# leighghunt/kart

Measured on AMD Instinct MI355X. Metric: feature deltas classified+field-diffed/sec (M/s) at 1/2/4/8 GPUs; % HBM peak, higher is better.
Workload: dtype u8/u64 (integer + fp64 compare); 1 GPU; C3: ONE 100000000-polygon int-PK layer, 10% edits (4% geometry + 4% attribute updates, 1% del, 1% ins), two-commit diff + field diff; features=100000000, delta_order=walk (= key) order, then pk order (kd_delta_pk_order), side_order=git tree (walk) order as listed, no side sort, parallelism=bucket-range shards x1

## Files before the change

include/kartdiff.h:

```cpp
#ifndef KARTDIFF_H
#define KARTDIFF_H

#include <stddef.h>
#include <stdint.h>

#ifdef __cplusplus
extern "C" {
#endif

#define KD_ABI_VERSION 1

#define KD_OK 0
#define KD_EINVAL (-1)
#define KD_EHIP (-2)
#define KD_EUNSUPPORTED (-3)

#define KD_NONE 0xFFFFFFFFu

#define KD_MEM_HOST 0u
#define KD_MEM_DEVICE 1u

#define KD_KEY_INT 0u
#define KD_KEY_HASH 1u

// ... 3 lines not shown
    uint64_t n;
    const uint64_t* key;
    const uint8_t* oid;
    const uint8_t* name;
    const uint64_t* name_off;
    uint32_t mem;
    uint32_t key_mode;
} kd_side;

typedef struct kd_blobs {
    uint64_t n;
    const uint8_t* data;
    const uint64_t* off;
    uint32_t mem;
    uint32_t size_hint;
} kd_blobs;

typedef struct kd_legend_maps {
    int32_t n_keys;
    int32_t words;
    int32_t n_leg_old;
    int32_t n_leg_new;
    const uint8_t* leg_old_hex;
    const int16_t* map_old;
    const uint8_t* leg_new_hex;
    const int16_t* map_new;
    const uint64_t* cmp_mask;
} kd_legend_maps;

typedef struct kd_diff_result {
    uint64_t n_insert, n_update, n_delete, n_delta;
    uint32_t* delta;
    uint32_t* upd;
} kd_diff_result;

typedef struct kd_merge_result {
    uint64_t n_clean;
    uint64_t n_conflict;
    uint64_t n_mdelta;
    uint32_t* conflict;
    uint32_t* mdelta;
} kd_merge_result;

int kd_abi_version(void);
const char* kd_last_error(void);
int kd_init(int device_ordinal, kd_ctx** out);
int kd_fini(kd_ctx* ctx);
int kd_set_stream(kd_ctx* ctx, void* hip_stream);
int kd_set_option(kd_ctx* ctx, const char* name, int64_t value);
int kd_get_option(kd_ctx* ctx, const char* name, int64_t* value);
int kd_sync(kd_ctx* ctx);
int kd_reserve(kd_ctx* ctx, uint64_t max_entries_per_side, uint64_t max_updates);
void kd_free(void* p);

int kd_diff2(kd_ctx* ctx, const kd_side* base, const kd_side* target, uint32_t flags,
             kd_diff_result** out);
#define KD_DIFF_UNORDERED 0x1u

int kd_diff2_device(kd_ctx* ctx, const kd_side* base, const kd_side* target, uint32_t flags,
                    uint32_t* d_delta, uint32_t* d_upd, uint64_t* d_counts, uint32_t* d_err);

int kd_diff2_device_perm(kd_ctx* ctx, const kd_side* base, const kd_side* target, const uint32_t* base_order,
                         const uint32_t* target_order, uint32_t flags, uint32_t* d_delta, uint32_t* d_upd,
                         uint64_t* d_counts, uint32_t* d_err);

int kd_diff2_device_ex(kd_ctx* ctx, const kd_side* base, const kd_side* target, const uint32_t* base_order,
                       const uint32_t* target_order, uint32_t flags, uint32_t* d_delta, uint32_t* d_upd,
                       uint64_t* d_delta_key, uint64_t* d_upd_key, uint64_t* d_counts, uint32_t* d_err);

int kd_fielddiff(kd_ctx* ctx, const kd_blobs* old_blobs, const kd_blobs* new_blobs,
                 const uint32_t* pu, uint64_t n_upd, const uint64_t* d_n_upd, uint32_t pairs_mem,
                 const kd_legend_maps* maps, uint64_t* masks, uint8_t* status, uint32_t out_mem);

int kd_merge3(kd_ctx* ctx, const kd_side* ancestor, const kd_side* ours, const kd_side* theirs,
              uint32_t flags, kd_merge_result** out);
int kd_merge3_device(kd_ctx* ctx, const kd_side* ancestor, const kd_side* ours, const kd_side* theirs,
                     uint32_t flags, uint32_t* d_conflict, uint32_t* d_mdelta, uint64_t* d_counts,
                     uint32_t* d_err);

int kd_merge3_device_perm(kd_ctx* ctx, const kd_side* ancestor, const kd_side* ours, const kd_side* theirs,
                          const uint32_t* ancestor_order, const uint32_t* ours_order, const uint32_t* theirs_order,
                          uint32_t flags, uint32_t* d_conflict, uint32_t* d_mdelta, uint64_t* d_counts,
                          uint32_t* d_err);

int kd_envelopes(kd_ctx* ctx, const kd_blobs* geoms, const double filt_env[4], int bits,
                 uint8_t* match, uint8_t* enc, uint8_t* enc_ok, uint32_t out_mem,
                 uint64_t* n_candidates);
int kd_env_overlap(kd_ctx* ctx, const uint8_t* enc, uint64_t n, int bits, const double q[4],
                   uint8_t* out, uint32_t mem);

typedef struct kd_sf_index kd_sf_index;
int kd_sf_index_build(kd_ctx* ctx, const uint8_t* oid, const uint8_t* env, uint64_t n, int bits, uint32_t mem,
                      kd_sf_index** out);
int kd_sf_filter(kd_ctx* ctx, const kd_sf_index* index, const uint8_t* oid, const uint8_t* is_feature, uint64_t m,
                 const double q[4], uint8_t* result, uint32_t mem);
int kd_sf_index_free(kd_sf_index* index);

#define KD_GF_RECT 0x1u
#define KD_GF_DELTA_HEADS 0x2u
typedef struct kd_geom_cols {
    int32_t n_leg_old, n_leg_new;
    const uint8_t* leg_old_hex;
    const int16_t* gidx_old;
    const uint8_t* leg_new_hex;
    const int16_t* gidx_new;
} kd_geom_cols;
int kd_geom_filter(kd_ctx* ctx, const kd_blobs* old_blobs, const kd_blobs* new_blobs, const uint32_t* pairs,
                   uint64_t n, const uint64_t* d_n, uint32_t pairs_mem, const kd_geom_cols* cols,
                   const double filt_env[4], uint32_t flags, int bits, uint8_t* match, uint32_t* keep,
                   uint64_t* n_keep, uint8_t* enc, uint8_t* enc_ok, uint32_t out_mem);

#define KD_GH_GEOM 0u
#define KD_GH_NULL 2u
#define KD_GH_FALLBACK 3u
typedef struct kd_geom_head {
    uint8_t gpkg[40];
    uint32_t glen;
    uint32_t goff_status;
} kd_geom_head;
int kd_geom_heads(const uint8_t* data, const uint64_t* off, uint64_t n, int n_leg, const uint8_t* leg_hex,
                  const int16_t* gidx, int threads, kd_geom_head* out);
int kd_geom_filter_heads(kd_ctx* ctx, const kd_geom_head* heads_old, uint64_t n_old, const kd_geom_head* heads_new,
                         uint64_t n_new, uint32_t heads_mem, const kd_blobs* old_blobs, const kd_blobs* new_blobs,
                         const uint32_t* pairs, uint64_t n, const uint64_t* d_n, uint32_t pairs_mem,
                         const double filt_env[4], uint32_t flags, int bits, uint8_t* match, uint32_t* keep,
                         uint64_t* n_keep, uint8_t* enc, uint8_t* enc_ok, uint32_t out_mem);

int kd_geom_filter_deltas(kd_ctx* ctx, const kd_geom_head* heads_old, uint64_t n_old, const kd_geom_head* heads_new,
                          uint64_t n_new, const kd_blobs* old_blobs, const kd_blobs* new_blobs, const uint32_t* pairs,
                          uint64_t cap, const uint64_t* d_n, const double filt_env[4], uint32_t flags, int bits,
                          uint8_t* match, uint32_t* keep, uint64_t* n_keep, uint8_t* enc, uint8_t* enc_ok);

#define KD_HEX_BYTES 0u
#define KD_HEX_GPKG_WKB 1u
int kd_hex_encode(kd_ctx* ctx, const kd_blobs* blobs, uint32_t mode, uint8_t* hex, uint32_t* start,
                  uint8_t* status, uint32_t out_mem);

int kd_sort_side(kd_ctx* ctx, uint64_t* d_key, uint8_t* d_oid, uint32_t* d_order, uint64_t n, uint32_t* h_dup);
typedef struct kd_keys_info {
    uint64_t vary;
    uint64_t key0;
    int64_t pk_min, pk_max;
    int32_t ascending;
    int32_t seg_max;
} kd_keys_info;
int kd_keys_scan(const uint64_t* keys, uint64_t n, uint32_t key_mode, kd_keys_info* out);
int kd_sort_side_into(kd_ctx* ctx, const uint64_t* d_key_in, const uint8_t* d_oid_in, uint64_t* d_key_out,
                      uint8_t* d_oid_out, uint32_t* d_order, uint64_t n, uint32_t* d_dup, const kd_keys_info* info);
int kd_sort_segmented_into(kd_ctx* ctx, const uint64_t* d_key_in, uint64_t* d_key_out, uint32_t* d_order,
                           uint64_t n, int seg_bits, int max_seg, uint32_t* d_err);
int kd_delta_pk_order(kd_ctx* ctx, const kd_side* base, const kd_side* target, const uint32_t* d_delta,
                      const uint64_t* d_keys, uint64_t cap, const uint64_t* d_n, int64_t pk_lo, int64_t pk_hi,
                      int64_t* d_pk, uint32_t* d_perm);

#define KD_COPY_H2D 1u
#define KD_COPY_D2H 2u
#define KD_COPY_D2D 3u
int kd_malloc(kd_ctx* ctx, uint64_t bytes, void** dptr);
int kd_mfree(kd_ctx* ctx, void* dptr);
int kd_host_alloc(uint64_t bytes, void** hptr);
int kd_host_free(void* hptr);
int kd_memcpy(kd_ctx* ctx, void* dst, const void* src, uint64_t bytes, uint32_t kind);
int kd_memset(kd_ctx* ctx, void* dst, int value, uint64_t bytes);
int kd_device_sync(kd_ctx* ctx);

#define KD_COMM_ID_BYTES 128
int kd_comm_unique_id(uint8_t id[KD_COMM_ID_BYTES]);
int kd_comm_init(kd_ctx* ctx, int nranks, int rank, const uint8_t id[KD_COMM_ID_BYTES]);
int kd_comm_fini(kd_ctx* ctx);
int kd_comm_info(kd_ctx* ctx, int32_t out[3]);
int kd_allgather_u64(kd_ctx* ctx, const uint64_t* d_send, uint64_t* d_recv, uint64_t n);
int kd_diff2_gather(kd_ctx* ctx, const kd_side* base, const kd_side* target, uint64_t base_off,
                    uint64_t target_off, uint32_t flags, uint32_t* d_delta, uint32_t* d_upd,
                    uint64_t* d_counts, uint32_t* d_err, uint32_t* d_all_delta, uint64_t all_cap,
                    uint64_t* d_all_counts, uint64_t* h_all_counts);
int kd_diff2_gather_begin(kd_ctx* ctx, const kd_side* base, const kd_side* target, uint64_t base_off,
                          uint64_t target_off, uint32_t flags, uint32_t* d_delta, uint32_t* d_upd,
                          uint64_t* d_counts, uint32_t* d_err, uint64_t* d_all_counts);
int kd_diff2_gather_end(kd_ctx* ctx, const uint32_t* d_delta, uint32_t* d_all_delta, uint64_t all_cap,
                        uint64_t* h_all_counts);
int kd_diff2_sharded(kd_ctx** ctxs, int g, const kd_side* base, const kd_side* target, int bucket_bits,
                     uint32_t flags, kd_diff_result** out);
int kd_shard_cuts(const uint64_t* key_a, uint64_t n_a, const uint64_t* key_b, uint64_t n_b, int g, int bucket_bits,
                  uint64_t* cut, uint64_t* a_lo, uint64_t* b_lo);

int64_t kd_pack_int_keys(const uint8_t* names, const uint64_t* name_off, uint64_t n,
                         uint64_t* keys, uint8_t* status);
int64_t kd_pack_hash_keys(const uint8_t* paths, const uint64_t* path_off, uint64_t n, int levels,
                          int hex, uint64_t* keys, uint8_t* status);
int kd_int_keys_to_pks(const uint64_t* keys, uint64_t n, int64_t* pks);

#define KD_ENOTFOUND (-4)
typedef struct kd_odb kd_odb;
int kd_odb_open(const char* gitdir, kd_odb** out);
int kd_odb_set_option(kd_odb* odb, const char* name, int64_t value);
int kd_odb_get_option(kd_odb* odb, const char* name, int64_t* value);
int kd_odb_close(kd_odb* odb);
int kd_odb_read(kd_odb* odb, const uint8_t oid[20], int* type, uint8_t** data, uint64_t* len);
int kd_odb_read_batch(kd_odb* odb, const uint8_t* oids, uint64_t n, int threads, uint8_t** data,
                      uint64_t* off, uint8_t* status);
typedef struct kd_leaves {
    uint64_t n;
    uint64_t* path_off;
    uint32_t* mode;
    uint8_t* oid;
    uint8_t* path;
    int32_t present;
} kd_leaves;
#define KD_WALK_ALL (-1)
int kd_walk(kd_odb* odb, const uint8_t* roots, int k, const char* subpath, int cmp0, int cmp1,
            int threads, kd_leaves** out);

int kd_prof_enable(kd_ctx* ctx, int on);
int kd_prof_select(kd_ctx* ctx, const char* names);
int kd_prof_get(kd_ctx* ctx, const char* name, uint64_t* launches, double* total_ms);
int kd_prof_reset(kd_ctx* ctx);

#ifdef __cplusplus
}
#endif
#endif
```

kart_amd/_native.py:

```python
import ctypes
import os

HERE = os.path.dirname(os.path.abspath(__file__))
LIB_PATH = os.environ.get("KART_AMD_LIB", os.path.join(HERE, "libkartdiff.so"))

KD_OK = 0
KD_EINVAL = -1
KD_EHIP = -2
KD_EUNSUPPORTED = -3
KD_ENOTFOUND = -4
KD_WALK_ALL = -1
KD_NONE = 0xFFFFFFFF
KD_MEM_HOST = 0
KD_MEM_DEVICE = 1
KD_KEY_INT = 0
KD_KEY_HASH = 1
KD_DIFF_UNORDERED = 0x1
KD_HEX_BYTES = 0
KD_HEX_GPKG_WKB = 1
KD_COPY_H2D = 1
KD_COPY_D2H = 2
KD_COPY_D2D = 3
KD_COMM_ID_BYTES = 128
KD_GH_GEOM, KD_GH_NULL, KD_GH_FALLBACK = 0, 2, 3
KD_GF_RECT = 0x1
KD_GF_DELTA_HEADS = 0x2

c_u8p = ctypes.POINTER(ctypes.c_uint8)
c_u32p = ctypes.POINTER(ctypes.c_uint32)
c_u64p = ctypes.POINTER(ctypes.c_uint64)
c_i16p = ctypes.POINTER(ctypes.c_int16)
c_i64p = ctypes.POINTER(ctypes.c_int64)
c_dblp = ctypes.POINTER(ctypes.c_double)


class NativeUnavailable(RuntimeError):
    pass


class KdError(RuntimeError):
    def __init__(self, code, msg):
        super().__init__(f"libkartdiff error {code}: {msg}")
        self.code = code


class Unsupported(KdError):
    """KD_EUNSUPPORTED: this input needs the reference CPU path."""


class NotFound(KdError):
    """KD_ENOTFOUND: a git object is not in the object database."""


class KdLeaves(ctypes.Structure):
    _fields_ = [
        ("n", ctypes.c_uint64),
        ("path_off", c_u64p),
        ("mode", c_u32p),
        ("oid", c_u8p),
        ("path", c_u8p),
        ("present", ctypes.c_int32),
    ]


class KdSide(ctypes.Structure):
    _fields_ = [
        ("n", ctypes.c_uint64),
        ("key", ctypes.c_void_p),
        ("oid", ctypes.c_void_p),
        ("name", ctypes.c_void_p),
        ("name_off", ctypes.c_void_p),
        ("mem", ctypes.c_uint32),
        ("key_mode", ctypes.c_uint32),
    ]


class KdBlobs(ctypes.Structure):
    _fields_ = [
        ("n", ctypes.c_uint64),
        ("data", ctypes.c_void_p),
        ("off", ctypes.c_void_p),
        ("mem", ctypes.c_uint32),
        ("size_hint", ctypes.c_uint32),
    ]


class KdLegendMaps(ctypes.Structure):
    _fields_ = [
        ("n_keys", ctypes.c_int32),
        ("words", ctypes.c_int32),
        ("n_leg_old", ctypes.c_int32),
        ("n_leg_new", ctypes.c_int32),
        ("leg_old_hex", ctypes.c_void_p),
        ("map_old", ctypes.c_void_p),
        ("leg_new_hex", ctypes.c_void_p),
        ("map_new", ctypes.c_void_p),
        ("cmp_mask", ctypes.c_void_p),
    ]


class KdGeomCols(ctypes.Structure):
    _fields_ = [
        ("n_leg_old", ctypes.c_int32),
        ("n_leg_new", ctypes.c_int32),
        ("leg_old_hex", ctypes.c_void_p),
        ("gidx_old", ctypes.c_void_p),
        ("leg_new_hex", ctypes.c_void_p),
        ("gidx_new", ctypes.c_void_p),
    ]


class KdKeysInfo(ctypes.Structure):
    _fields_ = [
        ("vary", ctypes.c_uint64),
        ("key0", ctypes.c_uint64),
        ("pk_min", ctypes.c_int64),
        ("pk_max", ctypes.c_int64),
        ("ascending", ctypes.c_int32),
        ("seg_max", ctypes.c_int32),
    ]


class KdDiffResult(ctypes.Structure):
    _fields_ = [
        ("n_insert", ctypes.c_uint64),
        ("n_update", ctypes.c_uint64),
        ("n_delete", ctypes.c_uint64),
        ("n_delta", ctypes.c_uint64),
        ("delta", c_u32p),
        ("upd", c_u32p),
    ]


class KdMergeResult(ctypes.Structure):
    _fields_ = [
        ("n_clean", ctypes.c_uint64),
        ("n_conflict", ctypes.c_uint64),
        ("n_mdelta", ctypes.c_uint64),
        ("conflict", c_u32p),
        ("mdelta", c_u32p),
    ]


SIGNATURES = {
    "kd_abi_version": (ctypes.c_int, []),
    "kd_last_error": (ctypes.c_char_p, []),
    "kd_init": (ctypes.c_int, [ctypes.c_int, ctypes.POINTER(ctypes.c_void_p)]),
    "kd_fini": (ctypes.c_int, [ctypes.c_void_p]),
    "kd_set_stream": (ctypes.c_int, [ctypes.c_void_p, ctypes.c_void_p]),
    "kd_set_option": (ctypes.c_int, [ctypes.c_void_p, ctypes.c_char_p, ctypes.c_int64]),
    "kd_get_option": (ctypes.c_int, [ctypes.c_void_p, ctypes.c_char_p, ctypes.POINTER(ctypes.c_int64)]),
    "kd_sync": (ctypes.c_int, [ctypes.c_void_p]),
    "kd_reserve": (ctypes.c_int, [ctypes.c_void_p, ctypes.c_uint64, ctypes.c_uint64]),
    "kd_free": (None, [ctypes.c_void_p]),
    "kd_diff2": (
        ctypes.c_int,
        [ctypes.c_void_p, ctypes.POINTER(KdSide), ctypes.POINTER(KdSide), ctypes.c_uint32,
         ctypes.POINTER(ctypes.POINTER(KdDiffResult))],
    ),
    "kd_diff2_device": (
        ctypes.c_int,
        [ctypes.c_void_p, ctypes.POINTER(KdSide), ctypes.POINTER(KdSide), ctypes.c_uint32,
         ctypes.c_void_p, ctypes.c_void_p, ctypes.c_void_p, ctypes.c_void_p],
    ),
    "kd_fielddiff": (
        ctypes.c_int,
        [ctypes.c_void_p, ctypes.POINTER(KdBlobs), ctypes.POINTER(KdBlobs), ctypes.c_void_p,
         ctypes.c_uint64, ctypes.c_void_p, ctypes.c_uint32, ctypes.POINTER(KdLegendMaps),
         ctypes.c_void_p, ctypes.c_void_p, ctypes.c_uint32],
    ),
    "kd_merge3": (
        ctypes.c_int,
        [ctypes.c_void_p, ctypes.POINTER(KdSide), ctypes.POINTER(KdSide), ctypes.POINTER(KdSide),
         ctypes.c_uint32, ctypes.POINTER(ctypes.POINTER(KdMergeResult))],
    ),
    "kd_merge3_device": (
        ctypes.c_int,
        [ctypes.c_void_p, ctypes.POINTER(KdSide), ctypes.POINTER(KdSide), ctypes.POINTER(KdSide),
         ctypes.c_uint32, ctypes.c_void_p, ctypes.c_void_p, ctypes.c_void_p, ctypes.c_void_p],
    ),
    "kd_merge3_device_perm": (
        ctypes.c_int,
        [ctypes.c_void_p, ctypes.POINTER(KdSide), ctypes.POINTER(KdSide), ctypes.POINTER(KdSide), ctypes.c_void_p,
         ctypes.c_void_p, ctypes.c_void_p, ctypes.c_uint32, ctypes.c_void_p, ctypes.c_void_p, ctypes.c_void_p,
         ctypes.c_void_p],
    ),
    "kd_envelopes": (
        ctypes.c_int,
        [ctypes.c_void_p, ctypes.POINTER(KdBlobs), c_dblp, ctypes.c_int, ctypes.c_void_p,
         ctypes.c_void_p, ctypes.c_void_p, ctypes.c_uint32, c_u64p],
    ),
    "kd_env_overlap": (
        ctypes.c_int,
        [ctypes.c_void_p, ctypes.c_void_p, ctypes.c_uint64, ctypes.c_int, c_dblp, ctypes.c_void_p,
         ctypes.c_uint32],
    ),
    "kd_geom_heads": (ctypes.c_int, [ctypes.c_void_p, ctypes.c_void_p, ctypes.c_uint64, ctypes.c_int, ctypes.c_void_p,
                                      ctypes.c_void_p, ctypes.c_int, ctypes.c_void_p]),
    "kd_geom_filter_heads": (
        ctypes.c_int,
        [ctypes.c_void_p, ctypes.c_void_p, ctypes.c_uint64, ctypes.c_void_p, ctypes.c_uint64, ctypes.c_uint32,
         ctypes.c_void_p, ctypes.c_void_p, ctypes.c_void_p, ctypes.c_uint64, ctypes.c_void_p, ctypes.c_uint32, c_dblp,
         ctypes.c_uint32, ctypes.c_int, ctypes.c_void_p, ctypes.c_void_p, c_u64p, ctypes.c_void_p, ctypes.c_void_p,
         ctypes.c_uint32],
    ),
    "kd_geom_filter_deltas": (
        ctypes.c_int,
        [ctypes.c_void_p, ctypes.c_void_p, ctypes.c_uint64, ctypes.c_void_p, ctypes.c_uint64, ctypes.POINTER(KdBlobs),
         ctypes.POINTER(KdBlobs), ctypes.c_void_p, ctypes.c_uint64, ctypes.c_void_p, c_dblp, ctypes.c_uint32, ctypes.c_int,
         ctypes.c_void_p, ctypes.c_void_p, c_u64p, ctypes.c_void_p, ctypes.c_void_p],
    ),
    "kd_shard_cuts": (ctypes.c_int, [ctypes.c_void_p, ctypes.c_uint64, ctypes.c_void_p, ctypes.c_uint64, ctypes.c_int,
                                      ctypes.c_int, ctypes.c_void_p, ctypes.c_void_p, ctypes.c_void_p]),
    "kd_sf_index_build": (ctypes.c_int, [ctypes.c_void_p, ctypes.c_void_p, ctypes.c_void_p, ctypes.c_uint64, ctypes.c_int,
                                          ctypes.c_uint32, ctypes.POINTER(ctypes.c_void_p)]),
    "kd_sf_filter": (ctypes.c_int, [ctypes.c_void_p, ctypes.c_void_p, ctypes.c_void_p, ctypes.c_void_p, ctypes.c_uint64,
                                     c_dblp, ctypes.c_void_p, ctypes.c_uint32]),
    "kd_sf_index_free": (ctypes.c_int, [ctypes.c_void_p]),
    "kd_geom_filter": (
        ctypes.c_int,
        [ctypes.c_void_p, ctypes.POINTER(KdBlobs), ctypes.POINTER(KdBlobs), ctypes.c_void_p, ctypes.c_uint64,
         ctypes.c_void_p, ctypes.c_uint32, ctypes.POINTER(KdGeomCols), c_dblp, ctypes.c_uint32, ctypes.c_int,
         ctypes.c_void_p, ctypes.c_void_p, c_u64p, ctypes.c_void_p, ctypes.c_void_p, ctypes.c_uint32],
    ),
    "kd_hex_encode": (
        ctypes.c_int,
        [ctypes.c_void_p, ctypes.POINTER(KdBlobs), ctypes.c_uint32, ctypes.c_void_p, ctypes.c_void_p,
         ctypes.c_void_p, ctypes.c_uint32],
    ),
    "kd_sort_side": (ctypes.c_int, [ctypes.c_void_p, ctypes.c_void_p, ctypes.c_void_p, ctypes.c_void_p, ctypes.c_uint64,
                                     ctypes.c_void_p]),
    "kd_diff2_device_perm": (ctypes.c_int, [ctypes.c_void_p, ctypes.c_void_p, ctypes.c_void_p, ctypes.c_void_p,
                                             ctypes.c_void_p, ctypes.c_uint32, ctypes.c_void_p, ctypes.c_void_p,
                                             ctypes.c_void_p, ctypes.c_void_p]),
    "kd_sort_side_into": (ctypes.c_int, [ctypes.c_void_p, ctypes.c_void_p, ctypes.c_void_p, ctypes.c_void_p,
                                          ctypes.c_void_p, ctypes.c_void_p, ctypes.c_uint64, ctypes.c_void_p,
                                          ctypes.POINTER(KdKeysInfo)]),
    "kd_keys_scan": (ctypes.c_int, [ctypes.c_void_p, ctypes.c_uint64, ctypes.c_uint32, ctypes.POINTER(KdKeysInfo)]),
    "kd_sort_segmented_into": (ctypes.c_int, [ctypes.c_void_p, ctypes.c_void_p, ctypes.c_void_p, ctypes.c_void_p,
                                               ctypes.c_uint64, ctypes.c_int, ctypes.c_int, ctypes.c_void_p]),
    "kd_delta_pk_order": (ctypes.c_int, [ctypes.c_void_p, ctypes.POINTER(KdSide), ctypes.POINTER(KdSide),
                                          ctypes.c_void_p, ctypes.c_void_p, ctypes.c_uint64, ctypes.c_void_p,
                                          ctypes.c_int64, ctypes.c_int64, ctypes.c_void_p, ctypes.c_void_p]),
    "kd_diff2_device_ex": (ctypes.c_int, [ctypes.c_void_p, ctypes.POINTER(KdSide), ctypes.POINTER(KdSide),
                                           ctypes.c_void_p, ctypes.c_void_p, ctypes.c_uint32, ctypes.c_void_p,
                                           ctypes.c_void_p, ctypes.c_void_p, ctypes.c_void_p, ctypes.c_void_p,
                                           ctypes.c_void_p]),
    "kd_malloc": (ctypes.c_int, [ctypes.c_void_p, ctypes.c_uint64, ctypes.POINTER(ctypes.c_void_p)]),
    "kd_mfree": (ctypes.c_int, [ctypes.c_void_p, ctypes.c_void_p]),
    "kd_host_alloc": (ctypes.c_int, [ctypes.c_uint64, ctypes.POINTER(ctypes.c_void_p)]),
    "kd_host_free": (ctypes.c_int, [ctypes.c_void_p]),
    "kd_memcpy": (ctypes.c_int, [ctypes.c_void_p, ctypes.c_void_p, ctypes.c_void_p, ctypes.c_uint64, ctypes.c_uint32]),
    "kd_memset": (ctypes.c_int, [ctypes.c_void_p, ctypes.c_void_p, ctypes.c_int, ctypes.c_uint64]),
    "kd_device_sync": (ctypes.c_int, [ctypes.c_void_p]),
    "kd_comm_unique_id": (ctypes.c_int, [ctypes.c_void_p]),
    "kd_comm_init": (ctypes.c_int, [ctypes.c_void_p, ctypes.c_int, ctypes.c_int, ctypes.c_void_p]),
    "kd_comm_fini": (ctypes.c_int, [ctypes.c_void_p]),
    "kd_comm_info": (ctypes.c_int, [ctypes.c_void_p, ctypes.c_void_p]),
    "kd_allgather_u64": (ctypes.c_int, [ctypes.c_void_p, ctypes.c_void_p, ctypes.c_void_p, ctypes.c_uint64]),
    "kd_diff2_gather": (
        ctypes.c_int,
        [ctypes.c_void_p, ctypes.POINTER(KdSide), ctypes.POINTER(KdSide), ctypes.c_uint64, ctypes.c_uint64,
         ctypes.c_uint32, ctypes.c_void_p, ctypes.c_void_p, ctypes.c_void_p, ctypes.c_void_p, ctypes.c_void_p,
         ctypes.c_uint64, ctypes.c_void_p, ctypes.c_void_p],
    ),
    "kd_diff2_gather_begin": (
        ctypes.c_int,
        [ctypes.c_void_p, ctypes.POINTER(KdSide), ctypes.POINTER(KdSide), ctypes.c_uint64, ctypes.c_uint64,
         ctypes.c_uint32, ctypes.c_void_p, ctypes.c_void_p, ctypes.c_void_p, ctypes.c_void_p, ctypes.c_void_p],
    ),
    "kd_diff2_gather_end": (
        ctypes.c_int, [ctypes.c_void_p, ctypes.c_void_p, ctypes.c_void_p, ctypes.c_uint64, ctypes.c_void_p],
    ),
    "kd_diff2_sharded": (
        ctypes.c_int,
        [ctypes.POINTER(ctypes.c_void_p), ctypes.c_int, ctypes.POINTER(KdSide), ctypes.POINTER(KdSide), ctypes.c_int,
         ctypes.c_uint32, ctypes.POINTER(ctypes.POINTER(KdDiffResult))],
    ),
    "kd_pack_int_keys": (
        ctypes.c_int64,
        [ctypes.c_void_p, ctypes.c_void_p, ctypes.c_uint64, ctypes.c_void_p, ctypes.c_void_p],
    ),
    "kd_pack_hash_keys": (
        ctypes.c_int64,
        [ctypes.c_void_p, ctypes.c_void_p, ctypes.c_uint64, ctypes.c_int, ctypes.c_int,
         ctypes.c_void_p, ctypes.c_void_p],
    ),
    "kd_int_keys_to_pks": (ctypes.c_int, [ctypes.c_void_p, ctypes.c_uint64, ctypes.c_void_p]),
    "kd_odb_open": (ctypes.c_int, [ctypes.c_char_p, ctypes.POINTER(ctypes.c_void_p)]),
    "kd_odb_close": (ctypes.c_int, [ctypes.c_void_p]),
    "kd_odb_set_option": (ctypes.c_int, [ctypes.c_void_p, ctypes.c_char_p, ctypes.c_int64]),
    "kd_odb_get_option": (ctypes.c_int, [ctypes.c_void_p, ctypes.c_char_p, ctypes.POINTER(ctypes.c_int64)]),
    "kd_odb_read": (
        ctypes.c_int,
        [ctypes.c_void_p, ctypes.c_void_p, ctypes.POINTER(ctypes.c_int), ctypes.POINTER(c_u8p), c_u64p],
    ),
    "kd_odb_read_batch": (
        ctypes.c_int,
        [ctypes.c_void_p, ctypes.c_void_p, ctypes.c_uint64, ctypes.c_int, ctypes.POINTER(c_u8p), ctypes.c_void_p,
         ctypes.c_void_p],
    ),
    "kd_walk": (
        ctypes.c_int,
        [ctypes.c_void_p, ctypes.c_void_p, ctypes.c_int, ctypes.c_char_p, ctypes.c_int, ctypes.c_int, ctypes.c_int,
         ctypes.POINTER(ctypes.POINTER(KdLeaves))],
    ),
    "kd_prof_enable": (ctypes.c_int, [ctypes.c_void_p, ctypes.c_int]),
    "kd_prof_select": (ctypes.c_int, [ctypes.c_void_p, ctypes.c_char_p]),
    "kd_prof_get": (
        ctypes.c_int,
        [ctypes.c_void_p, ctypes.c_char_p, c_u64p, c_dblp],
    ),
    "kd_prof_reset": (ctypes.c_int, [ctypes.c_void_p]),
}

_lib = None


def lib():
    global _lib
    if _lib is None:
        if not os.path.exists(LIB_PATH):
            raise NativeUnavailable(
                f"{LIB_PATH} not built: run `python -c 'import __graft_entry__ as g; g.build()'`"
            )
        try:
            L = ctypes.CDLL(LIB_PATH)
        except OSError as e:
            raise NativeUnavailable(f"cannot load {LIB_PATH}: {e}") from e
        for name, (res, args) in SIGNATURES.items():
            fn = getattr(L, name)
            fn.restype = res
            fn.argtypes = args
        _lib = L
    return _lib


def check(rc, what=""):
    if rc == KD_OK:
        return
    msg = lib().kd_last_error().decode(errors="replace")
    if rc == KD_EUNSUPPORTED:
        raise Unsupported(rc, f"{what}: {msg}")
    if rc == KD_ENOTFOUND:
        raise NotFound(rc, f"{what}: {msg}")
    raise KdError(rc, f"{what}: {msg}")


def ptr(a):
    if a is None:
        return None
    return a.ctypes.data
```

kart_amd/csrc/kd_classify.hip:

```cpp
#include <cstdlib>

#include "kd_join.h"

namespace kd {

#ifndef KD_RS3_PROBE_NOSEARCH
#define KD_RS3_PROBE_NOSEARCH 0
#endif
#ifndef KD_RS3_PROBE_NOOID
#define KD_RS3_PROBE_NOOID 0
#endif
#ifndef KD_RS3_PROBE_NONAMES
#define KD_RS3_PROBE_NONAMES 0
#endif
constexpr int C3_NT = 256;
constexpr int C3_CH = 1024;
#ifndef KD_C3_SAMPLE_BITS
#define KD_C3_SAMPLE_BITS 11
#endif
constexpr int C3_SAMPLE_BITS = KD_C3_SAMPLE_BITS;
constexpr int C3_SAMPLES = 1 << C3_SAMPLE_BITS;

struct Resolve3Args {
    const u64 *A, *O, *T;
// ... 281 lines not shown
    g.A = (const u64*)dz; g.O = (const u64*)ptr(O.key, nO); g.T = (const u64*)ptr(T.key, nT);
    g.oA = (const u32*)ptr(A.oid, nA); g.oO = (const u32*)ptr(O.oid, nO); g.oT = (const u32*)ptr(T.oid, nT);
    g.nA = nA; g.nO = nO;
    g.nmA = (const u8*)ptr(A.name, nA); g.nmO = (const u8*)ptr(O.name, nO); g.nmT = (const u8*)ptr(T.name, nT);
    g.noA = (const u64*)ptr(A.name_off, nA); g.noO = (const u64*)ptr(O.name_off, nO); g.noT = (const u64*)ptr(T.name_off, nT);
    g.hash_mode = A.key_mode == KD_KEY_HASH;
    g.cand = nullptr; g.cand3 = cand3; g.c2 = c2;
    g.pA = (const u32*)ptr(pA, nA); g.pO = (const u32*)ptr(pO, nO); g.pT = (const u32*)ptr(pT, nT);
    g.desc = (u64*)desc; g.nchunk = nchunk; g.aux = (u32*)aux;
    g.out_conf = d_conf; g.out_md = d_md; g.counts = counts; g.err = derr;
    const u64 grid = std::min<u64>((nO + nT) / C3_CH + 1, (u64)ctx->n_cu * (u64)occ_r3a);
    return launch(ctx, "k_resolve3", [&] {
        if (perm) hipLaunchKernelGGL((k_resolve3<C3_NT, true, true>), dim3((unsigned)grid), dim3(C3_NT), 0, ctx->stream, g);
        else hipLaunchKernelGGL((k_resolve3<C3_NT, false, true>), dim3((unsigned)grid), dim3(C3_NT), 0, ctx->stream, g);
    });
}

int kd::stage_side(kd_ctx* ctx, const kd_side* s, const char* tag, kd_side* dev) {
    *dev = *s;
    dev->mem = KD_MEM_DEVICE;
    std::string p(tag);
    int rc;
    if ((rc = stage_in(ctx, (p + ".key").c_str(), s->key, s->n * 8, s->mem, (const void**)&dev->key))) return rc;
    if ((rc = stage_in(ctx, (p + ".oid").c_str(), s->oid, s->n * 20, s->mem, (const void**)&dev->oid))) return rc;
    if (s->key_mode == KD_KEY_HASH && s->n) {
        KD_CHECK(s->name_off && s->name, "KD_KEY_HASH side without filenames");
        u64 nbytes = s->mem == KD_MEM_HOST ? s->name_off[s->n] : 0;
        if (s->mem == KD_MEM_DEVICE) {
            KD_HIP(hipMemcpy(&nbytes, s->name_off + s->n, 8, hipMemcpyDeviceToHost));
        }
        if ((rc = stage_in(ctx, (p + ".noff").c_str(), s->name_off, (s->n + 1) * 8, s->mem, (const void**)&dev->name_off))) return rc;
        if ((rc = stage_in(ctx, (p + ".name").c_str(), s->name, nbytes ? nbytes : 1, s->mem, (const void**)&dev->name))) return rc;
    }
    return KD_OK;
}

int kd::check_side(const kd_side* s, const char* which) {
    KD_CHECK(s, "%s side is NULL", which);
    KD_CHECK(s->n == 0 || (s->key && s->oid), "%s side: key/oid NULL", which);
    KD_CHECK(s->mem == KD_MEM_HOST || s->mem == KD_MEM_DEVICE, "%s side: bad mem", which);
    KD_CHECK(s->key_mode == KD_KEY_INT || s->key_mode == KD_KEY_HASH, "%s side: bad key_mode", which);
    return KD_OK;
}

static int merge3_device(kd_ctx* ctx, const kd_side& A, const kd_side& O, const kd_side& T, u32* d_conf, uint2* d_md,
                         u64* counts, u32* derr, const u32* pA = nullptr, const u32* pO = nullptr,
                         const u32* pT = nullptr) {
    const bool perm = pA || pO || pT;
    int rc;
    const u64 nA = A.n, nO = O.n, nT = T.n;
    if (nO + nT > 0 && ctx->opt.merge3_join)
        return merge3_join_device(ctx, A, O, T, d_conf, d_md, counts, derr, pA, pO, pT);
    const u64 nchunk = (nO + nT) / C3_CH + 2;
    void *cand, *c2, *desc, *aux, *dz;
    if ((rc = ensure(ctx, "c3.cand", (nO + nT + 1) * 8, &cand))) return rc;
    if ((rc = ensure(ctx, "c3.c2", 64, &c2))) return rc;
    if ((rc = ensure(ctx, "c3.desc", 2 * nchunk * 8, &desc))) return rc;
    const bool fresh_aux = ctx->bufs["c3.aux"].p == nullptr;
    if ((rc = ensure(ctx, "c3.aux", 64, &aux))) return rc;
    if (fresh_aux) KD_HIP(hipMemsetAsync(aux, 0, 64, ctx->stream));
    if ((rc = device_zeros(ctx, &dz))) return rc;
    const u64* kA = nA ? A.key : (const u64*)dz;
    rc = launch(ctx, "k_sorted3", [&] {
        const u64 work = std::max<u64>(nA / 2, 2 * nchunk);
        const u64 blocks = std::min<u64>((work + 255) / 256, (u64)ctx->n_cu * 8);
        hipLaunchKernelGGL(k_sorted3, dim3((unsigned)std::max<u64>(blocks, 1)), dim3(256), 0, ctx->stream, kA, nA,
                           (u64*)desc, 2 * nchunk, (u32*)aux, counts);
    });
    if (rc) return rc;
    if ((rc = diff2_device(ctx, &O, &T, 0, (u32*)cand, nullptr, (u64*)c2, derr, perm ? pO : nullptr,
                           perm ? pT : nullptr)))
        return rc;
    ctx->occ_resolve3 = occupancy(ctx, perm ? (const void*)k_resolve3<C3_NT, true, false> : (const void*)k_resolve3<C3_NT, false, false>,
                                  C3_NT, 0);
    auto ptr = [&](const void* p, u64 n) { return n && p ? p : (const void*)dz; };
    Resolve3Args g;
    g.A = kA; g.O = (const u64*)ptr(O.key, nO); g.T = (const u64*)ptr(T.key, nT);
    g.oA = (const u32*)ptr(A.oid, nA); g.oO = (const u32*)ptr(O.oid, nO); g.oT = (const u32*)ptr(T.oid, nT);
    g.nA = nA; g.nO = nO;
    g.nmA = (const u8*)ptr(A.name, nA); g.nmO = (const u8*)ptr(O.name, nO); g.nmT = (const u8*)ptr(T.name, nT);
    g.noA = (const u64*)ptr(A.name_off, nA); g.noO = (const u64*)ptr(O.name_off, nO); g.noT = (const u64*)ptr(T.name_off, nT);
    g.hash_mode = A.key_mode == KD_KEY_HASH;
    g.cand = (const uint2*)cand; g.c2 = (const u64*)c2;
    g.pA = (const u32*)ptr(pA, nA); g.pO = (const u32*)ptr(pO, nO); g.pT = (const u32*)ptr(pT, nT);
    g.desc = (u64*)desc; g.nchunk = nchunk; g.aux = (u32*)aux;
    g.out_conf = d_conf; g.out_md = d_md; g.counts = counts; g.err = derr;
    const u64 grid = std::min<u64>((nO + nT) / C3_CH + 1, (u64)ctx->n_cu * (u64)ctx->occ_resolve3);
    return launch(ctx, "k_resolve3", [&] {
        if (perm) hipLaunchKernelGGL((k_resolve3<C3_NT, true, false>), dim3((unsigned)grid), dim3(C3_NT), 0, ctx->stream, g);
        else hipLaunchKernelGGL((k_resolve3<C3_NT, false, false>), dim3((unsigned)grid), dim3(C3_NT), 0, ctx->stream, g);
    });
}

extern "C" {

int kd_reserve(kd_ctx* ctx, uint64_t max_entries_per_side, uint64_t max_updates) {
    KD_CHECK(ctx, "kd_reserve: ctx NULL");
    KD_HIP(hipSetDevice(ctx->device));
    u64 total = 2 * max_entries_per_side;
    u64 ntiles = (total + C2_TILE - 1) / C2_TILE + 1;
    void* p;
    int rc;
    if ((rc = ensure(ctx, "c2.part", (ntiles + 1) * 8, &p))) return rc;
    if ((rc = ensure(ctx, "c2.tcnt", ntiles * 16, &p))) return rc;
    if ((rc = ensure(ctx, "c2.gsum", 2 * (ntiles / 64 + 1) * 8, &p))) return rc;
    if ((rc = ensure(ctx, "c2.sdel", ntiles * (C2_TILE + 64) * 8, &p))) return rc;
    (void)max_updates;
    return KD_OK;
}

int kd_diff2_device(kd_ctx* ctx, const kd_side* base, const kd_side* target, uint32_t flags, uint32_t* d_delta,
                    uint32_t* d_upd, uint64_t* d_counts, uint32_t* d_err) {
    KD_CHECK(ctx, "kd_diff2_device: ctx NULL");
    int rc;
    if ((rc = check_side(base, "base")) || (rc = check_side(target, "target"))) return rc;
    KD_CHECK(base->mem == KD_MEM_DEVICE && target->mem == KD_MEM_DEVICE, "kd_diff2_device: sides must be device memory");
    KD_CHECK(d_delta && d_counts && d_err, "kd_diff2_device: NULL output");
    KD_HIP(hipSetDevice(ctx->device));
    return diff2_device(ctx, base, target, flags, d_delta, d_upd, d_counts, d_err);
}

int kd_diff2_device_perm(kd_ctx* ctx, const kd_side* base, const kd_side* target, const uint32_t* base_order,
                         const uint32_t* target_order, uint32_t flags, uint32_t* d_delta, uint32_t* d_upd,
                         uint64_t* d_counts, uint32_t* d_err) {
    KD_CHECK(ctx, "kd_diff2_device_perm: ctx NULL");
    int rc;
    if ((rc = check_side(base, "base")) || (rc = check_side(target, "target"))) return rc;
    KD_CHECK(base->mem == KD_MEM_DEVICE && target->mem == KD_MEM_DEVICE, "kd_diff2_device_perm: sides must be device memory");
    KD_CHECK(d_delta && d_counts && d_err, "kd_diff2_device_perm: NULL output");
    KD_CHECK((base->n == 0 || base_order) && (target->n == 0 || target_order), "kd_diff2_device_perm: NULL order");
    KD_HIP(hipSetDevice(ctx->device));
    return diff2_device(ctx, base, target, flags, d_delta, d_upd, d_counts, d_err,
                        base_order ? base_order : (const u32*)nullptr, target_order);
}

int kd_diff2_device_ex(kd_ctx* ctx, const kd_side* base, const kd_side* target, const uint32_t* base_order,
                       const uint32_t* target_order, uint32_t flags, uint32_t* d_delta, uint32_t* d_upd,
                       uint64_t* d_delta_key, uint64_t* d_upd_key, uint64_t* d_counts, uint32_t* d_err) {
    KD_CHECK(ctx, "kd_diff2_device_ex: ctx NULL");
    int rc;
    if ((rc = check_side(base, "base")) || (rc = check_side(target, "target"))) return rc;
    KD_CHECK(base->mem == KD_MEM_DEVICE && target->mem == KD_MEM_DEVICE, "kd_diff2_device_ex: sides must be device memory");
    KD_CHECK(d_delta && d_counts && d_err, "kd_diff2_device_ex: NULL output");
    KD_CHECK(!base_order == !target_order, "kd_diff2_device_ex: both orders or neither");
    KD_CHECK(!d_upd_key || (d_upd && d_delta_key), "kd_diff2_device_ex: update keys need the update list and delta keys");
    KD_HIP(hipSetDevice(ctx->device));
    void* dz = nullptr;
    if (base_order && (rc = device_zeros(ctx, &dz))) return rc;
    const u32* oa = base_order ? (base->n ? base_order : (const u32*)dz) : nullptr;
    const u32* ob = target_order ? (target->n ? target_order : (const u32*)dz) : nullptr;
    return diff2_device(ctx, base, target, flags, d_delta, d_upd, d_counts, d_err, oa, ob, d_delta_key, d_upd_key);
}

int kd_diff2(kd_ctx* ctx, const kd_side* base, const kd_side* target, uint32_t flags, kd_diff_result** out) {
    KD_CHECK(ctx && out, "kd_diff2: NULL");
    int rc;
    if ((rc = check_side(base, "base")) || (rc = check_side(target, "target"))) return rc;
    KD_HIP(hipSetDevice(ctx->device));
    host_mark(ctx, nullptr);
    kd_side A, B;
    if ((rc = stage_side(ctx, base, "in.a", &A)) || (rc = stage_side(ctx, target, "in.b", &B))) return rc;
    host_mark(ctx, "kd_diff2 stage");
    u64 total = base->n + target->n;
    void *dd, *du, *dc;
    if ((rc = ensure(ctx, "out.delta", (total + 1) * 8, &dd))) return rc;
    if ((rc = ensure(ctx, "out.upd", (total + 1) * 8, &du))) return rc;
    if ((rc = ensure(ctx, "out.counts", 64, &dc))) return rc;
    host_mark(ctx, "kd_diff2 ensure");
    u64* counts = (u64*)dc;
    u32* derr = (u32*)(counts + 4);
    if ((rc = diff2_device(ctx, &A, &B, flags, (u32*)dd, (u32*)du, counts, derr))) return rc;
    host_mark(ctx, "kd_diff2 kernels");
    u64 hc[5];
    KD_HIP(hipMemcpyAsync(hc, dc, 40, hipMemcpyDeviceToHost, ctx->stream));
    KD_HIP(hipStreamSynchronize(ctx->stream));
    u32 err = (u32)(hc[4] & 0xFFFFFFFFu);
    if (err) {
        set_error("kd_diff2: %s", (err & 1) ? "side keys not strictly ascending" : "hash key collision between different filenames");
        return KD_EUNSUPPORTED;
    }
    u64 nd = hc[3], nu = hc[1];
    host_mark(ctx, "kd_diff2 counts");
    size_t bytes = sizeof(kd_diff_result) + (nd + nu) * 8 + 16;
    kd_diff_result* r = (kd_diff_result*)std::malloc(bytes);
    KD_CHECK(r, "kd_diff2: out of host memory");
    host_mark(ctx, "kd_diff2 malloc");
    r->n_insert = hc[0]; r->n_update = hc[1]; r->n_delete = hc[2]; r->n_delta = nd;
    r->delta = (u32*)(r + 1);
    r->upd = r->delta + 2 * nd;
    if (nd) {
        if ((rc = stage_d2h(ctx, r->delta, dd, nd * 8)) || (nu && (rc = stage_d2h(ctx, r->upd, du, nu * 8)))) {
            std::free(r);
            return rc;
        }
    }
    host_mark(ctx, "kd_diff2 results");
    prof_flush(ctx);
    *out = r;
    return KD_OK;
}

int kd_merge3(kd_ctx* ctx, const kd_side* anc, const kd_side* ours, const kd_side* theirs, uint32_t flags,
              kd_merge_result** out) {
    (void)flags;
    KD_CHECK(ctx && out, "kd_merge3: NULL");
    int rc;
    if ((rc = check_side(anc, "ancestor")) || (rc = check_side(ours, "ours")) || (rc = check_side(theirs, "theirs"))) return rc;
    KD_CHECK(anc->key_mode == ours->key_mode && ours->key_mode == theirs->key_mode, "kd_merge3: key modes differ");
    KD_CHECK(anc->n < 0xFFFFFFFFull && ours->n < 0xFFFFFFFFull && theirs->n < 0xFFFFFFFFull, "kd_merge3: side too large");
    KD_HIP(hipSetDevice(ctx->device));
    kd_side A, O, T;
    if ((rc = stage_side(ctx, anc, "in.a", &A)) || (rc = stage_side(ctx, ours, "in.b", &O)) ||
        (rc = stage_side(ctx, theirs, "in.c", &T)))
        return rc;
    const u64 nA = A.n, nO = O.n, nT = T.n;
    void *oc, *om, *dc;
    if ((rc = ensure(ctx, "c3.oc", (nA + nO + nT + 1) * 12, &oc))) return rc;
    if ((rc = ensure(ctx, "c3.om", (nO + nT + 1) * 8, &om))) return rc;
    if ((rc = ensure(ctx, "c3.counts", 64, &dc))) return rc;
    u64* counts = (u64*)dc;
    u32* derr = (u32*)(counts + 4);
    if ((rc = merge3_device(ctx, A, O, T, (u32*)oc, (uint2*)om, counts, derr))) return rc;
    u64 hc[5];
    KD_HIP(hipMemcpyAsync(hc, dc, 40, hipMemcpyDeviceToHost, ctx->stream));
    KD_HIP(hipStreamSynchronize(ctx->stream));
    u32 err = (u32)(hc[4] & 0xFFFFFFFFu);
    if (err) {
        set_error("kd_merge3: err=0x%x (%s)", err,
                  (err & 1) ? "keys not strictly ascending" : (err & 2) ? "hash key collision" : "tile overflow");
        return KD_EUNSUPPORTED;
    }
    u64 nc = hc[1], nm = hc[2];
    kd_merge_result* r = (kd_merge_result*)std::malloc(sizeof(kd_merge_result) + nc * 12 + nm * 8 + 16);
    KD_CHECK(r, "kd_merge3: out of host memory");
    r->n_clean = hc[0]; r->n_conflict = nc; r->n_mdelta = nm;
    r->conflict = (u32*)(r + 1);
    r->mdelta = r->conflict + 3 * nc;
    if ((nc && (rc = stage_d2h(ctx, r->conflict, oc, nc * 12))) || (nm && (rc = stage_d2h(ctx, r->mdelta, om, nm * 8)))) {
        std::free(r);
        return rc;
    }
    prof_flush(ctx);
    *out = r;
    return KD_OK;
}

int kd_merge3_device(kd_ctx* ctx, const kd_side* anc, const kd_side* ours, const kd_side* theirs, uint32_t flags,
                     uint32_t* d_conflict, uint32_t* d_mdelta, uint64_t* d_counts, uint32_t* d_err) {
    (void)flags;
    KD_CHECK(ctx && d_conflict && d_mdelta && d_counts && d_err, "kd_merge3_device: NULL");
    int rc;
    if ((rc = check_side(anc, "ancestor")) || (rc = check_side(ours, "ours")) || (rc = check_side(theirs, "theirs"))) return rc;
    KD_CHECK(anc->mem == KD_MEM_DEVICE && ours->mem == KD_MEM_DEVICE && theirs->mem == KD_MEM_DEVICE,
             "kd_merge3_device: sides must be device memory");
    KD_CHECK(anc->key_mode == ours->key_mode && ours->key_mode == theirs->key_mode, "kd_merge3_device: key modes differ");
    KD_CHECK(anc->n < 0xFFFFFFFFull && ours->n < 0xFFFFFFFFull && theirs->n < 0xFFFFFFFFull,
             "kd_merge3_device: side too large");
    KD_HIP(hipSetDevice(ctx->device));
    return merge3_device(ctx, *anc, *ours, *theirs, d_conflict, (uint2*)d_mdelta, d_counts, d_err);
}

int kd_merge3_device_perm(kd_ctx* ctx, const kd_side* anc, const kd_side* ours, const kd_side* theirs,
                          const uint32_t* anc_order, const uint32_t* ours_order, const uint32_t* theirs_order,
                          uint32_t flags, uint32_t* d_conflict, uint32_t* d_mdelta, uint64_t* d_counts, uint32_t* d_err) {
    (void)flags;
    KD_CHECK(ctx && d_conflict && d_mdelta && d_counts && d_err, "kd_merge3_device_perm: NULL");
    int rc;
    if ((rc = check_side(anc, "ancestor")) || (rc = check_side(ours, "ours")) || (rc = check_side(theirs, "theirs"))) return rc;
    KD_CHECK(anc->mem == KD_MEM_DEVICE && ours->mem == KD_MEM_DEVICE && theirs->mem == KD_MEM_DEVICE,
             "kd_merge3_device_perm: sides must be device memory");
    KD_CHECK(anc->key_mode == ours->key_mode && ours->key_mode == theirs->key_mode, "kd_merge3_device_perm: key modes differ");
    KD_CHECK(anc->n < 0xFFFFFFFFull && ours->n < 0xFFFFFFFFull && theirs->n < 0xFFFFFFFFull,
             "kd_merge3_device_perm: side too large");
    KD_CHECK((anc->n == 0 || anc_order) && (ours->n == 0 || ours_order) && (theirs->n == 0 || theirs_order),
             "kd_merge3_device_perm: NULL order");
    KD_HIP(hipSetDevice(ctx->device));
    void* dz;
    if ((rc = device_zeros(ctx, &dz))) return rc;
    auto ord = [&](const uint32_t* p) { return p ? p : (const u32*)dz; };
    return merge3_device(ctx, *anc, *ours, *theirs, d_conflict, (uint2*)d_mdelta, d_counts, d_err, ord(anc_order),
                         ord(ours_order), ord(theirs_order));
}

}
```

kart_amd/csrc/kd_classify2.hip:

```cpp
#include <cstdlib>

#include "kd_join.h"

namespace kd {

constexpr u64 C2_GROUP = 64;
#ifndef KD_C2_STAGE_PAD
#define KD_C2_STAGE_PAD 32
#endif
constexpr u64 C2_STAGE = C2_TILE + KD_C2_STAGE_PAD;
#ifndef KD_J2_NAME_HALO
#define KD_J2_NAME_HALO 64
#endif
constexpr u64 J2_NAME_HALO = KD_J2_NAME_HALO;
#ifndef KD_PLACE_NT
#define KD_PLACE_NT 64
#endif


template <int PW>
__device__ __forceinline__ u64 mp_search(const u64* __restrict__ A, const u64* __restrict__ B, u64 d, u64 lo, u64 hi) {
    const int lane = threadIdx.x & 63, sub = lane % PW, grp = lane / PW;
    while (hi > lo) {
        const u64 step = (hi - lo + PW - 1) / PW;
// ... 1492 lines not shown
        }
        __syncthreads();
        if (cf) {
            u32* o = sc + 3 * (tc + pc + __builtin_amdgcn_mbcnt_hi((u32)(bc >> 32), __builtin_amdgcn_mbcnt_lo((u32)bc, 0)));
            o[0] = ik; o[1] = io; o[2] = itt;
        }
        if (md) sm[tm + pm + __builtin_amdgcn_mbcnt_hi((u32)(bm >> 32), __builtin_amdgcn_mbcnt_lo((u32)bm, 0))] = make_uint2(io, itt);
        tc += nc;
        tm += nm;
    }
    if (ne) err |= 2u;
    static_assert(2 * IPT < 16, "k_join3b: the clean count's ballot slices");
    {
        const u32 wcl = (u32)__popcll(__ballot(clean & 1)) + 2u * (u32)__popcll(__ballot((clean >> 1) & 1)) +
                        4u * (u32)__popcll(__ballot((clean >> 2) & 1)) + 8u * (u32)__popcll(__ballot((clean >> 3) & 1));
        if (lane == 0) s_wave[2 * (NT / 64) + wid] = wcl;
    }
    __syncthreads();
    u32 tcl = 0;
#pragma unroll
    for (int w = 0; w < NT / 64; w++) tcl += s_wave[2 * (NT / 64) + w];
    if (tid == 0) {
        u32* cc = g.tile_cnt + 4 * tile;
        cc[0] = tcl; cc[1] = tm; cc[2] = 0; cc[3] = tc;
        u64* gs = g.gsum + 2 * (tile / C2_GROUP);
        atomicAdd((unsigned long long*)gs, (unsigned long long)(tc | (u64)tm << 32));
        atomicAdd((unsigned long long*)gs + 1, (unsigned long long)tcl);
    }
    if (!more) break;
    tile = tnext;
    nmA0 = xA0; nmA1 = xA1; nmB0 = xB0; nmB1 = xB1;
    }
    if (err) atomicOr(g.err, err);
}

int merge3_join_device(kd_ctx* ctx, const kd_side& K, const kd_side& O, const kd_side& T, u32* d_conf, uint2* d_md,
                       u64* d_counts, u32* d_err, const u32* ordK, const u32* ordO, const u32* ordT) {
    const u64 nK = K.n, nO = O.n, nT = T.n, total = nO + nT;
    const bool hash = K.key_mode == KD_KEY_HASH;
    const bool perm = ordK || ordO || ordT;
    const bool split = ctx->opt.merge3_split == 1;
    const bool j3_ol = ctx->opt.j3_ol == 1;
    const bool v2 = ctx->opt.j3_v != 0 && !(j3_ol && !perm);
    const int TILE = v2 ? J3B_TILE : J3_TILE;
    if (hash) KD_CHECK((nK == 0 || (K.name && K.name_off)) && (nO == 0 || (O.name && O.name_off)) &&
                       (nT == 0 || (T.name && T.name_off)), "merge3: KD_KEY_HASH needs filenames");
    const u64 ntiles = (total + TILE - 1) / TILE;
    const u64 n_zero = 2 * ((ntiles + C2_GROUP - 1) / C2_GROUP);
    void *part, *apart, *tcnt, *gsum, *gpre, *sconf, *smd, *dz;
    int rc;
    if ((rc = ensure(ctx, "c2.part", (ntiles + 1) * sizeof(u64), &part))) return rc;
    if ((rc = ensure(ctx, "c3.apart", (ntiles + 1) * sizeof(u64), &apart))) return rc;
    if ((rc = ensure(ctx, "c2.tcnt", ntiles * 4 * sizeof(u32), &tcnt))) return rc;
    if ((rc = ensure(ctx, "c2.gsum", n_zero * sizeof(u64), &gsum))) return rc;
    if ((rc = ensure(ctx, "c2.gpre", n_zero * sizeof(u64), &gpre))) return rc;
    if ((rc = ensure(ctx, "c3.sconf", ntiles * C2_STAGE * 12, &sconf))) return rc;
    if ((rc = ensure(ctx, "c3.smd", ntiles * C2_STAGE * sizeof(uint2), &smd))) return rc;
    if ((rc = device_zeros(ctx, &dz))) return rc;
    auto P = [&](const void* p, u64 n) { return n && p ? p : (const void*)dz; };
    const u64* kO = (const u64*)P(O.key, nO);
    const u64* kT = (const u64*)P(T.key, nT);
    const u64* kK = (const u64*)P(K.key, nK);
    rc = launch(ctx, "k_partition2", [&] {
        unsigned nb = (unsigned)((ntiles + C2_PG - 1) / C2_PG);
        if (v2) hipLaunchKernelGGL(k_partition2<J3B_TILE>, dim3(nb), dim3(C2_PNT), 0, ctx->stream, kO, nO, kT, nT, ntiles,
                                   (u64*)part, d_counts, d_err, (u64*)gsum, n_zero);
        else hipLaunchKernelGGL(k_partition2<J3_TILE>, dim3(nb), dim3(C2_PNT), 0, ctx->stream, kO, nO, kT, nT, ntiles,
                                (u64*)part, d_counts, d_err, (u64*)gsum, n_zero);
    });
    if (rc) return rc;
    void* nsplit = nullptr;
    if (v2 && hash && (rc = ensure(ctx, "c3.nsplit", 4 * (ntiles + 1) * sizeof(u64), &nsplit))) return rc;
    rc = launch(ctx, "k_apart3", [&] {
        const u64 lanes = 8 * (ntiles + 1);
        if (v2)
            hipLaunchKernelGGL(k_apart3b, dim3((unsigned)((lanes + 255) / 256)), dim3(256), 0, ctx->stream, kO, nO, kT, nT,
                               (const u64*)part, ntiles, TILE, kK, nK, (u64*)apart, (const u64*)P(O.name_off, nO),
                               (const u64*)P(T.name_off, nT), perm ? J3B_HALO : (u64)0, (u64*)nsplit);
        else
            hipLaunchKernelGGL(k_apart3, dim3((unsigned)((lanes + 255) / 256)), dim3(256), 0, ctx->stream, kO, nO, kT, nT,
                               (const u64*)part, ntiles, TILE, kK, nK, (u64*)apart);
    });
    if (rc) return rc;
    Join3Args a;
    Join2Args& g = a.j;
    g.A = kO; g.oidA = (const u8*)P(O.oid, nO); g.nA = nO;
    g.B = kT; g.oidB = (const u8*)P(T.oid, nT); g.nB = nT;
    g.part = (const u64*)part;
    g.nameA = (const u8*)P(O.name, nO); g.nameOffA = (const u64*)P(O.name_off, nO);
    g.nameB = (const u8*)P(T.name, nT); g.nameOffB = (const u64*)P(T.name_off, nT);
    g.hash_mode = hash ? 1 : 0;
    g.dummy = (const u8*)dz;
    g.ordA = (const u32*)P(ordO, nO); g.ordB = (const u32*)P(ordT, nT);
    g.stage_delta = nullptr;
    g.tile_cnt = (u32*)tcnt; g.gsum = (u64*)gsum; g.err = d_err;
    g.out_delta = g.out_upd = nullptr; g.counts = d_counts;
    g.stage_dkey = g.out_dkey = g.out_ukey = nullptr;
    g.ntiles = ntiles;
    a.K = kK; a.oidK = (const u8*)P(K.oid, nK); a.nameK = (const u8*)P(K.name, nK);
    a.nameOffK = (const u64*)P(K.name_off, nK); a.ordK = (const u32*)P(ordK, nK); a.nK = nK;
    a.apart = (const u64*)apart; a.stage_conf = (u32*)sconf; a.stage_md = (uint2*)smd;
    a.nsplit = (const u64*)nsplit;
    void *cand3 = nullptr, *c2 = nullptr;
    if (split) {
        if ((rc = ensure(ctx, "c3.cand3", (total + 1) * 12, &cand3))) return rc;
        if ((rc = ensure(ctx, "c3.c2j", 64, &c2))) return rc;
    }
    auto j3b_grid = [&](const void* kern) {
        if (!J3B_PERSIST) return (unsigned)ntiles;
        return (unsigned)std::max<u64>(1, std::min<u64>(ntiles, (u64)ctx->n_cu * (u64)occupancy(ctx, kern, J3B_NT, 0)));
    };
    rc = launch(ctx, "k_join3", [&] {
#define KD_J3(H, PM, S) hipLaunchKernelGGL((k_join3<C2_NT, J3_IPT, H, PM, S>), dim3((unsigned)ntiles), dim3(C2_NT), 0, ctx->stream, a)
        if (v2) {
#define KD_J3B(H, PM, S) hipLaunchKernelGGL((k_join3b<J3B_NT, J3B_IPT, H, PM, S>), dim3(j3b_grid((const void*)k_join3b<J3B_NT, J3B_IPT, H, PM, S>)), dim3(J3B_NT), 0, ctx->stream, a)
            if (split) {
                if (hash) { if (perm) KD_J3B(true, true, true); else KD_J3B(true, false, true); }
                else { if (perm) KD_J3B(false, true, true); else KD_J3B(false, false, true); }
            } else {
                if (hash) { if (perm) KD_J3B(true, true, false); else KD_J3B(true, false, false); }
                else { if (perm) KD_J3B(false, true, false); else KD_J3B(false, false, false); }
            }
#undef KD_J3B
        } else if (split) {
            if (hash) { if (perm) KD_J3(true, true, true); else KD_J3(true, false, true); }
            else { if (perm) KD_J3(false, true, true); else KD_J3(false, false, true); }
        } else if (j3_ol && !perm) {
            if (hash) hipLaunchKernelGGL((k_join3<C2_NT, J3_IPT, true, false, false, true>), dim3((unsigned)ntiles), dim3(C2_NT), 0, ctx->stream, a);
            else hipLaunchKernelGGL((k_join3<C2_NT, J3_IPT, false, false, false, true>), dim3((unsigned)ntiles), dim3(C2_NT), 0, ctx->stream, a);
        } else {
            if (hash) { if (perm) KD_J3(true, true, false); else KD_J3(true, false, false); }
            else { if (perm) KD_J3(false, true, false); else KD_J3(false, false, false); }
        }
#undef KD_J3
    });
    if (rc) return rc;
    u64* jcounts = split ? (u64*)c2 : d_counts;
    rc = launch(ctx, "k_gscan2", [&] {
        hipLaunchKernelGGL(k_gscan2, dim3(1), dim3(1024), 0, ctx->stream, (const u64*)gsum, (u64)(n_zero / 2),
                           (u64*)gpre, jcounts, 1);
    });
    if (rc) return rc;
    rc = launch(ctx, "k_place3", [&] {
        hipLaunchKernelGGL(k_place3, dim3((unsigned)ntiles), dim3(64), 0, ctx->stream, (const u32*)sconf,
                           (const uint2*)smd, (const u32*)tcnt, (const u64*)gpre, split ? (u32*)cand3 : d_conf, d_md);
    });
    if (rc || !split) return rc;
    return resolve3_have_a(ctx, K, O, T, (const u32*)cand3, (const u64*)c2, d_conf, d_md, d_counts, d_err, ordK, ordO,
                           ordT);
}

int diff2_device(kd_ctx* ctx, const kd_side* A, const kd_side* B, u32 flags, u32* d_delta, u32* d_upd,
                 u64* d_counts, u32* d_err, const u32* ordA, const u32* ordB, u64* d_dkey, u64* d_ukey) {
    const bool unord = (flags & KD_DIFF_UNORDERED) != 0;
    const u64 nA = A->n, nB = B->n, total = nA + nB;
    KD_CHECK(nA < 0xFFFFFFFFull && nB < 0xFFFFFFFFull, "diff2: side too large for uint32 indices");
    const bool hash = A->key_mode == KD_KEY_HASH || B->key_mode == KD_KEY_HASH;
    KD_CHECK(A->key_mode == B->key_mode, "diff2: key modes differ");
    if (hash) KD_CHECK((nA == 0 || (A->name && A->name_off)) && (nB == 0 || (B->name && B->name_off)),
                       "diff2: KD_KEY_HASH needs filenames");
    const u64 ntiles = (total + C2_TILE - 1) / C2_TILE;
    if (ntiles == 0) {
        KD_HIP(hipMemsetAsync(d_err, 0, sizeof(u32), ctx->stream));
        KD_HIP(hipMemsetAsync(d_counts, 0, 4 * sizeof(u64), ctx->stream));
        return KD_OK;
    }
    void *part, *tcnt = nullptr, *sdel = nullptr, *gsum = nullptr, *gpre = nullptr;
    int rc;
    if ((rc = ensure(ctx, "c2.part", (ntiles + 1) * sizeof(u64), &part))) return rc;
    u64* zero = nullptr;
    u64 n_zero = 0;
    if (!unord) {
        n_zero = 2 * ((ntiles + C2_GROUP - 1) / C2_GROUP);
        if ((rc = ensure(ctx, "c2.tcnt", ntiles * 4 * sizeof(u32), &tcnt))) return rc;
        if ((rc = ensure(ctx, "c2.gsum", n_zero * sizeof(u64), &gsum))) return rc;
        if ((rc = ensure(ctx, "c2.gpre", n_zero * sizeof(u64), &gpre))) return rc;
        if ((rc = ensure(ctx, "c2.sdel", ntiles * C2_STAGE * sizeof(uint2), &sdel))) return rc;
        zero = (u64*)gsum;
    }
    void* skd = nullptr;
    if (d_dkey && !unord && (rc = ensure(ctx, "c2.skd", ntiles * C2_STAGE * sizeof(u64), &skd))) return rc;
    void* dz;
    if ((rc = device_zeros(ctx, &dz))) return rc;
    const u64* kA = nA ? A->key : (const u64*)dz;
    const u64* kB = nB ? B->key : (const u64*)dz;
    const u8* empty_oid = (const u8*)dz;
    rc = launch(ctx, "k_partition2", [&] {
        unsigned nb = (unsigned)((ntiles + C2_PG - 1) / C2_PG);
        hipLaunchKernelGGL(k_partition2<C2_TILE>, dim3(nb), dim3(C2_PNT), 0, ctx->stream, kA, nA, kB, nB, ntiles,
                           (u64*)part, d_counts, d_err, zero, n_zero);
    });
    if (rc) return rc;
    Join2Args g;
    g.A = kA; g.oidA = nA ? A->oid : empty_oid; g.nA = nA;
    g.B = kB; g.oidB = nB ? B->oid : empty_oid; g.nB = nB;
    g.part = (const u64*)part;
    g.nameA = nA && A->name ? A->name : (const u8*)dz;
    g.nameOffA = nA && A->name_off ? A->name_off : (const u64*)dz;
    g.nameB = nB && B->name ? B->name : (const u8*)dz;
    g.nameOffB = nB && B->name_off ? B->name_off : (const u64*)dz;
    g.hash_mode = hash ? 1 : 0;
    g.dummy = (const u8*)dz;
    const bool perm = ordA != nullptr || ordB != nullptr;
    const bool oid_lds = nA + nB >= ctx->opt.j2_oidlds_min;
    const bool j2r = ctx->opt.j2r == 1;
    const int j2r_occ = j2r ? occupancy(ctx, (const void*)k_join2r<C2_NT, C2_IPT>, C2_NT, 0) : 1;
    g.ordA = nA && ordA ? ordA : (const u32*)dz;
    g.ordB = nB && ordB ? ordB : (const u32*)dz;
    g.stage_delta = (uint2*)sdel;
    g.tile_cnt = (u32*)tcnt; g.gsum = (u64*)gsum; g.err = d_err;
    g.out_delta = (uint2*)d_delta; g.out_upd = (uint2*)d_upd; g.counts = d_counts;
    g.stage_dkey = (u64*)skd;
    g.out_dkey = d_dkey; g.out_ukey = d_upd ? d_ukey : nullptr;
    g.ntiles = ntiles;
    rc = launch(ctx, "k_join2", [&] {
#define KD_J2(U, H, P) hipLaunchKernelGGL((k_join2<C2_NT, C2_IPT, U, H, P>), dim3((unsigned)ntiles), dim3(C2_NT), 0, ctx->stream, g)
#define KD_J2OL(U) hipLaunchKernelGGL((k_join2<C2_NT, C2_IPT, U, false, false, true>), dim3((unsigned)ntiles), dim3(C2_NT), 0, ctx->stream, g)
#define KD_J2R() hipLaunchKernelGGL((k_join2r<C2_NT, C2_IPT>), dim3((unsigned)std::min<u64>(ntiles, (u64)ctx->n_cu * j2r_occ)), dim3(C2_NT), 0, ctx->stream, g)
        if (perm) {
            if (unord) { if (hash) KD_J2(true, true, true); else KD_J2(true, false, true); }
            else { if (hash) KD_J2(false, true, true); else KD_J2(false, false, true); }
        } else if (!hash && oid_lds) {
            if (unord) KD_J2OL(true);
            else if (j2r) KD_J2R();
            else KD_J2OL(false);
        } else {
            if (unord) { if (hash) KD_J2(true, true, false); else KD_J2(true, false, false); }
            else { if (hash) KD_J2(false, true, false); else KD_J2(false, false, false); }
        }
#undef KD_J2
#undef KD_J2OL
#undef KD_J2R
    });
    if (rc || unord) return rc;
    rc = launch(ctx, "k_gscan2", [&] {
        hipLaunchKernelGGL(k_gscan2, dim3(1), dim3(1024), 0, ctx->stream, (const u64*)gsum, (u64)(n_zero / 2),
                           (u64*)gpre, d_counts, 0);
    });
    if (rc) return rc;
    return launch(ctx, "k_place2", [&] {
        hipLaunchKernelGGL((k_place2<KD_PLACE_NT>), dim3((unsigned)ntiles), dim3(KD_PLACE_NT), 0, ctx->stream,
                           (const uint2*)sdel, (const u32*)tcnt, (const u64*)gpre, (int)C2_STAGE, (uint2*)d_delta,
                           (uint2*)d_upd, (const u64*)skd, d_dkey, d_upd ? d_ukey : nullptr);
    });
}

}
```

kart_amd/csrc/kd_ctx.hip:

```cpp
#include <cstdarg>
#include <cstdio>
#include <cstdlib>
#include <cstring>
#include <algorithm>
#include <chrono>
#include <thread>

#include "kd_internal.h"
#include "kd_walkkey.h"

namespace kd {

static thread_local char g_err[1024] = "";

void set_error(const char* fmt, ...) {
    va_list ap;
    va_start(ap, fmt);
    vsnprintf(g_err, sizeof g_err, fmt, ap);
    va_end(ap);
}

constexpr size_t SLAB_BYTES = (size_t)64 << 20, SLAB_PIECE_MAX = (size_t)8 << 20;

int ensure(kd_ctx* ctx, const char* slot, size_t bytes, void** out) {
    DevBuf& b = ctx->bufs[slot];
    if (bytes == 0) bytes = 16;
    if (b.bytes < bytes) {
        if (b.p) {
            hipError_t e = hipStreamSynchronize(ctx->stream);
            if (e != hipSuccess) { set_error("sync before realloc: %s", hipGetErrorString(e)); return KD_EHIP; }
            if (!b.slab) KD_HIP(hipFree(b.p));
            b.p = nullptr;
            b.bytes = 0;
            b.slab = false;
        }
        const size_t want = (bytes + bytes / 8 + 255) & ~(size_t)255;
        if (want <= SLAB_PIECE_MAX) {
            if (!ctx->slab) {
                void* s = nullptr;
                if (hipMalloc(&s, SLAB_BYTES) == hipSuccess) ctx->slab = (char*)s;
                ctx->slab_used = 0;
            }
            if (ctx->slab && ctx->slab_used + want <= SLAB_BYTES) {
                b.p = ctx->slab + ctx->slab_used;
                ctx->slab_used += want;
                b.bytes = want;
                b.slab = true;
            }
        }
        if (!b.p) {
            KD_HIP(hipMalloc(&b.p, want));
            b.bytes = want;
        }
    }
    *out = b.p;
    return KD_OK;
}

int device_zeros(kd_ctx* ctx, void** out) {
    kd::DevBuf& b = ctx->bufs["zeros"];
    const bool fresh = b.p == nullptr;
    int rc = ensure(ctx, "zeros", 256, out);
    if (rc) return rc;
    if (fresh) KD_HIP(hipMemsetAsync(*out, 0, 256, ctx->stream));
    return KD_OK;
}

int stage_in(kd_ctx* ctx, const char* slot, const void* p, size_t bytes, u32 mem, const void** dev) {
    if (p == nullptr || bytes == 0 || mem == KD_MEM_DEVICE) {
        *dev = p;
        return KD_OK;
    }
    void* d = nullptr;
    int rc = ensure(ctx, slot, bytes, &d);
    if (rc) return rc;
    if ((rc = stage_h2d(ctx, d, p, bytes))) return rc;
    *dev = d;
    return KD_OK;
}

constexpr size_t PIN_CHUNK = (size_t)4 << 20, PIN_MIN = (size_t)64 << 10, PIN_MAX = (size_t)32 << 20;

int stage_h2d(kd_ctx* ctx, void* dst, const void* src, size_t bytes) {
    if (bytes < PIN_MIN || bytes >= PIN_MAX || !ctx->pin[1]) {
        KD_HIP(hipMemcpyAsync(dst, src, bytes, hipMemcpyHostToDevice, ctx->stream));
        return KD_OK;
    }
    for (size_t o = 0; o < bytes; o += PIN_CHUNK) {
        const int j = ctx->pin_next;
        ctx->pin_next ^= 1;
        const size_t c = std::min(PIN_CHUNK, bytes - o);
        KD_HIP(hipEventSynchronize(ctx->pin_ev[j]));
        std::memcpy(ctx->pin[j], (const char*)src + o, c);
        KD_HIP(hipMemcpyAsync((char*)dst + o, ctx->pin[j], c, hipMemcpyHostToDevice, ctx->stream));
        KD_HIP(hipEventRecord(ctx->pin_ev[j], ctx->stream));
    }
    return KD_OK;
}

__global__ __launch_bounds__(256) void k_to_host(const u8* __restrict__ src, u8* __restrict__ dst, u64 bytes) {
    const u64 n16 = bytes / 16;
    for (u64 i = (u64)blockIdx.x * 256 + threadIdx.x; i < n16; i += (u64)gridDim.x * 256)
        ((uint4*)dst)[i] = ((const uint4*)src)[i];
    const u64 t = 16 * n16 + (u64)blockIdx.x * 256 + threadIdx.x;
    if (blockIdx.x == 0 && t < bytes) dst[t] = src[t];
}

int stage_d2h(kd_ctx* ctx, void* dst, const void* src, size_t bytes) {
    if (bytes < PIN_MIN || bytes >= PIN_MAX || !ctx->pin[1]) {
        KD_HIP(hipMemcpyAsync(dst, src, bytes, hipMemcpyDeviceToHost, ctx->stream));
        KD_HIP(hipStreamSynchronize(ctx->stream));
        return KD_OK;
    }
    const size_t n = (bytes + PIN_CHUNK - 1) / PIN_CHUNK;
    const bool aligned = ((uintptr_t)src & 15) == 0 && ctx->pin_dev[1];
    auto issue = [&](size_t i) -> hipError_t {
        const size_t o = i * PIN_CHUNK, c = std::min(PIN_CHUNK, bytes - o);
        hipError_t e;
        if (aligned) {
            const unsigned grid = (unsigned)std::min<size_t>((c / 16 + 255) / 256 + 1, 1024);
            hipLaunchKernelGGL(k_to_host, dim3(grid), dim3(256), 0, ctx->stream, (const u8*)src + o,
                               (u8*)ctx->pin_dev[i & 1], (u64)c);
            e = hipGetLastError();
        } else {
            e = hipMemcpyAsync(ctx->pin[i & 1], (const char*)src + o, c, hipMemcpyDeviceToHost, ctx->stream);
        }
        return e == hipSuccess ? hipEventRecord(ctx->pin_ev[i & 1], ctx->stream) : e;
    };
    KD_HIP(issue(0));
    for (size_t i = 0; i < n; i++) {
        if (i + 1 < n) KD_HIP(issue(i + 1));
        KD_HIP(hipEventSynchronize(ctx->pin_ev[i & 1]));
        host_mark(ctx, "d2h chunk wait");
        const size_t o = i * PIN_CHUNK;
        std::memcpy((char*)dst + o, ctx->pin[i & 1], std::min(PIN_CHUNK, bytes - o));
        host_mark(ctx, "d2h chunk copy-out");
    }
    ctx->pin_next = 0;
    return KD_OK;
}

void host_mark(kd_ctx* ctx, const char* name) {
    static thread_local std::chrono::steady_clock::time_point t0;
    if (!ctx->opt.trace_host) return;
    (void)hipStreamSynchronize(ctx->stream);
    const auto t = std::chrono::steady_clock::now();
    if (name) std::fprintf(stderr, "[kd] %-22s %9.3f ms\n", name, std::chrono::duration<double, std::milli>(t - t0).count());
    t0 = t;
}

void prof_begin(kd_ctx* ctx, const char* name, hipEvent_t* a) {
    (void)name;
    if (ctx->ev_pool.empty()) {
        hipEvent_t e;
        if (hipEventCreateWithFlags(&e, hipEventDisableSystemFence) != hipSuccess) { *a = nullptr; return; }
        ctx->ev_pool.push_back(e);
    }
    *a = ctx->ev_pool.back();
    ctx->ev_pool.pop_back();
    (void)hipEventRecord(*a, ctx->stream);
}

void prof_end(kd_ctx* ctx, const char* name, hipEvent_t a) {
    if (!a) return;
    hipEvent_t b;
    if (ctx->ev_pool.empty()) {
        if (hipEventCreateWithFlags(&b, hipEventDisableSystemFence) != hipSuccess) return;
    } else {
        b = ctx->ev_pool.back();
        ctx->ev_pool.pop_back();
    }
    (void)hipEventRecord(b, ctx->stream);
    ctx->pending.push_back({name, a, b});
}

int prof_flush(kd_ctx* ctx) {
    for (auto& p : ctx->pending) {
        KD_HIP(hipEventSynchronize(p.b));
        float ms = 0;
        KD_HIP(hipEventElapsedTime(&ms, p.a, p.b));
        ProfStat& s = ctx->stats[p.name];
        s.launches++;
        s.ms += ms;
        ctx->ev_pool.push_back(p.a);
        ctx->ev_pool.push_back(p.b);
    }
    ctx->pending.clear();
    return KD_OK;
}

static inline int b64v(u8 c) {
    if (c >= 'A' && c <= 'Z') return c - 'A';
    if (c >= 'a' && c <= 'z') return c - 'a' + 26;
    if (c >= '0' && c <= '9') return c - '0' + 52;
    if (c == '-') return 62;
    if (c == '_') return 63;
    return -1;
}

static inline int int_key(bool neg, u64 mag, u64* key) {
    if (neg ? mag > (1ull << 63) : mag >= (1ull << 63)) return 2;
    *key = wk::int_key(neg ? (i64)(0 - mag) : (i64)mag);
    return 0;
}

static int decode_int_name(const u8* s, int n, u64* key) {
    u8 buf[16];
    int o = 0, acc = 0, bits = 0;
    for (int i = 0; i < n; i++) {
        if (s[i] == '=') break;
        int v = b64v(s[i]);
        if (v < 0) return 1;
        acc = (acc << 6) | v;
        bits += 6;
        if (bits >= 8) {
            bits -= 8;
            if (o >= 16) return 1;
            buf[o++] = (u8)((acc >> bits) & 0xFF);
        }
    }
    if (o < 2 || buf[0] != 0x91) return 1;
    u8 t = buf[1];
    int w = 0;
    bool sgn = false;
    u64 u = 0;
    if (t <= 0x7f) { u = t; }
    else if (t >= 0xe0) { sgn = true; u = (u64)(i64)(int8_t)t; }
    else if (t >= 0xcc && t <= 0xcf) { w = 1 << (t - 0xcc); }
    else if (t >= 0xd0 && t <= 0xd3) { w = 1 << (t - 0xd0); sgn = true; }
    else return 1;
    if (o != 2 + w) return 1;
    if (w) {
        for (int i = 0; i < w; i++) u = (u << 8) | buf[2 + i];
        if (sgn) { int sh = 64 - 8 * w; u = (u64)(((i64)(u << sh)) >> sh); }
    }
    if (sgn) {
        i64 v = (i64)u;
        return int_key(v < 0, v < 0 ? (u64)(-(__int128)v) : (u64)v, key);
    }
    return int_key(false, u, key);
}

template <typename F>
static void par_for(u64 n, F&& f) {
    unsigned nt = std::thread::hardware_concurrency();
    if (nt == 0) nt = 1;
    if (nt > 32) nt = 32;
    if (n < 65536) nt = 1;
    std::vector<std::thread> th;
    u64 chunk = (n + nt - 1) / nt;
    for (unsigned t = 0; t < nt; t++) {
        u64 a = t * chunk, b = std::min<u64>(n, a + chunk);
        if (a >= b) break;
        th.emplace_back([&f, a, b] { for (u64 i = a; i < b; i++) f(i); });
    }
    for (auto& t : th) t.join();
}

static inline u64 fnv1a64(const u8* p, u64 n) {
    u64 h = 1469598103934665603ull;
    for (u64 i = 0; i < n; i++) { h ^= p[i]; h *= 1099511628211ull; }
    return h;
}

}

using namespace kd;

namespace kd {
int occupancy(kd_ctx* ctx, const void* kernel, int block, size_t lds) {
    const auto key = std::make_tuple(kernel, block, lds);
    auto it = ctx->occ.find(key);
    if (it != ctx->occ.end()) return it->second;
    int nb = 0;
    if (hipSetDevice(ctx->device) != hipSuccess ||
        hipOccupancyMaxActiveBlocksPerMultiprocessor(&nb, kernel, block, lds) != hipSuccess || nb <= 0)
        nb = 1;
    ctx->occ[key] = nb;
    return nb;
}
}

extern "C" {

int kd_abi_version(void) { return KD_ABI_VERSION; }

const char* kd_last_error(void) { return kd::g_err; }

__global__ void k_load_probe() {}

namespace {
struct OptDef {
    const char* name;
    const char* env;
    int64_t kd_opts::*i64;
    int kd_opts::*i32;
    uint64_t kd_opts::*u64;
};
const OptDef OPTS[] = {
    {"merge3_join", "KD_MERGE3_JOIN", nullptr, &kd_opts::merge3_join, nullptr},
    {"merge3_split", "KD_MERGE3_SPLIT", nullptr, &kd_opts::merge3_split, nullptr},
    {"j3_ol", "KD_J3_OL", nullptr, &kd_opts::j3_ol, nullptr},
    {"j3_v", "KD_J3_V", nullptr, &kd_opts::j3_v, nullptr},
    {"j2_oidlds_min", "KD_J2_OIDLDS_MIN", nullptr, nullptr, &kd_opts::j2_oidlds_min},
    {"j2r", "KD_J2R", nullptr, &kd_opts::j2r, nullptr},
    {"fd_stream", "KD_FD_STREAM", nullptr, &kd_opts::fd_stream, nullptr},
    {"fd_walk", "KD_FD_WALK", nullptr, &kd_opts::fd_walk, nullptr},
    {"pkm_max_blocks", "KD_PKM_MAX_BLOCKS", nullptr, nullptr, &kd_opts::pkm_max_blocks},
    {"trace_host", "KD_TRACE_HOST", nullptr, &kd_opts::trace_host, nullptr},
};
void opt_set(kd_opts& o, const OptDef& d, int64_t v) {
    if (d.i32) o.*(d.i32) = (int)v;
    else if (d.u64) o.*(d.u64) = (uint64_t)v;
}
}

int kd_set_option(kd_ctx* ctx, const char* name, int64_t value) {
    KD_CHECK(ctx && name, "kd_set_option: NULL");
    for (const OptDef& d : OPTS)
        if (!strcmp(d.name, name)) {
            opt_set(ctx->opt, d, value);
            return KD_OK;
        }
    KD_CHECK(false, "kd_set_option: unknown option '%s'", name);
}

int kd_get_option(kd_ctx* ctx, const char* name, int64_t* value) {
    KD_CHECK(ctx && name && value, "kd_get_option: NULL");
    for (const OptDef& d : OPTS)
        if (!strcmp(d.name, name)) {
            *value = d.i32 ? (int64_t)(ctx->opt.*(d.i32)) : (int64_t)(ctx->opt.*(d.u64));
            return KD_OK;
        }
    KD_CHECK(false, "kd_get_option: unknown option '%s'", name);
}

int kd_init(int device_ordinal, kd_ctx** out) {
    KD_CHECK(out != nullptr, "kd_init: out is NULL");
    int n = 0;
    KD_HIP(hipGetDeviceCount(&n));
    KD_CHECK(device_ordinal >= 0 && device_ordinal < n, "kd_init: device %d of %d", device_ordinal, n);
    KD_HIP(hipSetDevice(device_ordinal));
    kd_ctx* c = new kd_ctx();
    c->device = device_ordinal;
    for (const OptDef& d : OPTS)
        if (const char* v = std::getenv(d.env)) opt_set(c->opt, d, strtoll(v, nullptr, 10));
    hipError_t e = hipStreamCreateWithFlags(&c->own_stream, hipStreamNonBlocking);
    if (e != hipSuccess) {
        delete c;
        set_error("hipStreamCreate: %s", hipGetErrorString(e));
        return KD_EHIP;
    }
    c->stream = c->own_stream;
    int cu = 0;
    if (hipDeviceGetAttribute(&cu, hipDeviceAttributeMultiprocessorCount, device_ordinal) == hipSuccess && cu > 0)
        c->n_cu = cu;
    {
        void* s = nullptr;
        if (hipMalloc(&s, SLAB_BYTES) == hipSuccess) c->slab = (char*)s;
        c->slab_used = 0;
    }
    for (int j = 0; j < 2; j++) {
        void* h = nullptr;
        if (hipHostMalloc(&h, PIN_CHUNK, hipHostMallocMapped) != hipSuccess) break;
        if (hipEventCreateWithFlags(&c->pin_ev[j], hipEventDisableTiming) != hipSuccess) {
            (void)hipHostFree(h);
            break;
        }
        c->pin[j] = (char*)h;
        void* dp = nullptr;
        if (hipHostGetDevicePointer(&dp, h, 0) == hipSuccess) c->pin_dev[j] = dp;
    }
    hipLaunchKernelGGL(k_load_probe, dim3(1), dim3(64), 0, c->stream);
    if (c->slab) {
        (void)hipMemsetAsync(c->slab, 0, 1024, c->stream);
        (void)hipMemcpyAsync(c->slab + 512, c->slab, 256, hipMemcpyDeviceToDevice, c->stream);
        for (int j = 0; j < 2; j++)
            if (c->pin[j]) {
                std::memset(c->pin[j], 0, PIN_CHUNK);
                (void)hipMemcpyAsync(c->slab + 4096, c->pin[j], PIN_CHUNK, hipMemcpyHostToDevice, c->stream);
                if (c->pin_dev[j])
                    hipLaunchKernelGGL(k_to_host, dim3(64), dim3(256), 0, c->stream, (const u8*)(c->slab + 4096),
                                       (u8*)c->pin_dev[j], (u64)PIN_CHUNK);
                (void)hipEventRecord(c->pin_ev[j], c->stream);
                (void)hipEventSynchronize(c->pin_ev[j]);
            }
        kd_side A{};
        A.n = 1;
        A.key = (const u64*)c->slab;
        A.oid = (const u8*)c->slab;
        A.mem = KD_MEM_DEVICE;
        A.key_mode = KD_KEY_INT;
        u32* out = (u32*)(c->slab + 512);
        c->slab_used = (size_t)8 << 20;
        (void)diff2_device(c, &A, &A, 0, out, out + 8, (u64*)(c->slab + 768), (u32*)(c->slab + 800));
        c->slab_used = 0;
        for (auto& kv : c->bufs)
            if (!kv.second.slab && kv.second.p) (void)hipFree(kv.second.p);
        c->bufs.clear();
    }
    if ((e = hipStreamSynchronize(c->stream)) != hipSuccess) {
        if (c->slab) (void)hipFree(c->slab);
        for (int j = 0; j < 2; j++) {
            if (c->pin[j]) (void)hipHostFree(c->pin[j]);
            if (c->pin_ev[j]) (void)hipEventDestroy(c->pin_ev[j]);
        }
        (void)hipStreamDestroy(c->own_stream);
        delete c;
        set_error("kd_init: %s", hipGetErrorString(e));
        return KD_EHIP;
    }
    *out = c;
    return KD_OK;
}

int kd_fini(kd_ctx* ctx) {
    if (!ctx) return KD_OK;
    (void)hipSetDevice(ctx->device);
    (void)hipStreamSynchronize(ctx->stream);
    prof_flush(ctx);
    comm_release(ctx);
    gather_release(ctx);
    for (auto& kv : ctx->bufs)
        if (kv.second.p && !kv.second.slab) (void)hipFree(kv.second.p);
    if (ctx->slab) (void)hipFree(ctx->slab);
    for (int j = 0; j < 2; j++) {
        if (ctx->pin[j]) (void)hipHostFree(ctx->pin[j]);
        if (ctx->pin_ev[j]) (void)hipEventDestroy(ctx->pin_ev[j]);
    }
    for (auto e : ctx->ev_pool) (void)hipEventDestroy(e);
    if (ctx->own_stream) (void)hipStreamDestroy(ctx->own_stream);
    delete ctx;
    return KD_OK;
}

int kd_set_stream(kd_ctx* ctx, void* hip_stream) {
    KD_CHECK(ctx, "kd_set_stream: ctx is NULL");
    ctx->stream = hip_stream ? (hipStream_t)hip_stream : ctx->own_stream;
    return KD_OK;
}

int kd_sync(kd_ctx* ctx) {
    KD_CHECK(ctx, "kd_sync: ctx is NULL");
    KD_HIP(hipSetDevice(ctx->device));
    KD_HIP(hipStreamSynchronize(ctx->stream));
    return prof_flush(ctx);
}

void kd_free(void* p) {
    if (!p) return;
    std::free(p);
}

int kd_prof_enable(kd_ctx* ctx, int on) {
    KD_CHECK(ctx, "kd_prof_enable: ctx is NULL");
    ctx->prof = on != 0;
    return KD_OK;
}

int kd_prof_select(kd_ctx* ctx, const char* names) {
    KD_CHECK(ctx, "kd_prof_select: ctx is NULL");
    ctx->prof_only = names && *names ? "," + std::string(names) + "," : std::string();
    return KD_OK;
}

int kd_prof_get(kd_ctx* ctx, const char* name, uint64_t* launches, double* total_ms) {
    KD_CHECK(ctx && name, "kd_prof_get: bad args");
    int rc = prof_flush(ctx);
    if (rc) return rc;
    auto it = ctx->stats.find(name);
    if (launches) *launches = it == ctx->stats.end() ? 0 : it->second.launches;
    if (total_ms) *total_ms = it == ctx->stats.end() ? 0 : it->second.ms;
    return KD_OK;
}

int kd_prof_reset(kd_ctx* ctx) {
    KD_CHECK(ctx, "kd_prof_reset: ctx is NULL");
    int rc = prof_flush(ctx);
    ctx->stats.clear();
    return rc;
}


int64_t kd_pack_int_keys(const uint8_t* names, const uint64_t* name_off, uint64_t n, uint64_t* keys,
                         uint8_t* status) {
    if (!names || !name_off || !keys || !status) { set_error("kd_pack_int_keys: NULL"); return KD_EINVAL; }
    std::vector<u64> badc(1, 0);
    std::mutex m;
    u64 bad = 0;
    par_for(n, [&](u64 i) {
        u64 a = name_off[i], b = name_off[i + 1];
        for (u64 j = b; j > a; j--)
            if (names[j - 1] == '/') { a = j; break; }
        u64 k = 0;
        int st = (b - a > 24) ? 1 : decode_int_name(names + a, (int)(b - a), &k);
        keys[i] = k;
        status[i] = (u8)st;
        if (st) { std::lock_guard<std::mutex> g(m); bad++; }
    });
    return (int64_t)bad;
}

int64_t kd_pack_hash_keys(const uint8_t* paths, const uint64_t* path_off, uint64_t n, int levels, int hex,
                          uint64_t* keys, uint8_t* status) {
    if (!paths || !path_off || !keys || !status || levels <= 0) { set_error("kd_pack_hash_keys: bad args"); return KD_EINVAL; }
    std::mutex m;
    u64 bad = 0;
    par_for(n, [&](u64 i) {
        const u8* s = paths + path_off[i];
        u64 len = path_off[i + 1] - path_off[i];
        u64 bucket = 0, pos = 0;
        int bits = 0, st = 0;
        for (int l = 0; l < levels && !st; l++) {
            int seg = hex ? 2 : 1;
            for (int c = 0; c < seg && !st; c++) {
                if (pos >= len) { st = 1; break; }
                u8 ch = s[pos++];
                int v;
                if (hex) {
                    v = (ch >= '0' && ch <= '9') ? ch - '0' : (ch >= 'a' && ch <= 'f') ? ch - 'a' + 10 : -1;
                    if (v < 0) { st = 1; break; }
                    bucket = (bucket << 4) | (u64)v; bits += 4;
                } else {
                    v = b64v(ch);
                    if (v < 0) { st = 1; break; }
                    bucket = (bucket << 6) | (u64)wk::T.rank[v]; bits += 6;
                }
            }
            if (!st && (pos >= len || s[pos] != '/')) st = 1;
            pos++;
        }
        u64 k = 0;
        if (!st) {
            int low = 64 - bits;
            u64 h = fnv1a64(s + pos, len - pos);
            k = (bucket << low) | (h >> (64 - low));
        }
        keys[i] = k;
        status[i] = (u8)st;
        if (st) { std::lock_guard<std::mutex> g(m); bad++; }
    });
    return (int64_t)bad;
}

int kd_keys_scan(const uint64_t* keys, uint64_t n, uint32_t key_mode, kd_keys_info* out) {
    KD_CHECK(out && (n == 0 || keys), "kd_keys_scan: NULL");
    KD_CHECK(key_mode == KD_KEY_INT || key_mode == KD_KEY_HASH, "kd_keys_scan: bad key_mode");
    *out = kd_keys_info{};
    out->ascending = 1;
    if (n == 0) return KD_OK;
    const u64 k0 = keys[0];
    unsigned nt = std::thread::hardware_concurrency();
    nt = nt == 0 ? 1 : nt > 32 ? 32 : nt;
    if (n < 65536) nt = 1;
    struct Part {
        u64 vary = 0;
        i64 lo = INT64_MAX, hi = INT64_MIN;
        bool asc = true, basc = true;
        u64 b0 = 0, b1 = 0, pre = 0, suf = 0, mx = 0, len = 0;
    };
    std::vector<Part> part(nt);
    std::vector<std::thread> th;
    const u64 chunk = (n + nt - 1) / nt;
    for (unsigned t = 0; t < nt; t++) {
        const u64 a = t * chunk, b = std::min<u64>(n, a + chunk);
        if (a >= b) break;
        th.emplace_back([&, t, a, b] {
            Part p;
            p.len = b - a;
            p.b0 = keys[a] >> 40;
            u64 run = 0, prev = p.b0;
            bool first = true;
            for (u64 i = a; i < b; i++) {
                const u64 k = keys[i];
                p.vary |= k ^ k0;
// ... 66 lines not shown
```

kart_amd/csrc/kd_internal.h:

```cpp
#pragma once
#include <hip/hip_runtime.h>

#include <cstdint>
#include <cstring>
#include <map>
#include <utility>
#include <mutex>
#include <string>
#include <tuple>
#include <vector>

#include "kartdiff.h"

typedef uint8_t u8;
typedef uint16_t u16;
typedef uint32_t u32;
typedef uint64_t u64;
typedef int64_t i64;
typedef int16_t i16;
typedef int8_t i8;
typedef unsigned u32x4 __attribute__((ext_vector_type(4)));
typedef uint64_t u64x2 __attribute__((ext_vector_type(2)));

namespace kd {

void set_error(const char* fmt, ...);

#define KD_HIP(call)                                                                        \
    do {                                                                                    \
        hipError_t e_ = (call);                                                             \
        if (e_ != hipSuccess) {                                                             \
            ::kd::set_error("%s:%d %s: %s", __FILE__, __LINE__, #call, hipGetErrorString(e_)); \
            return KD_EHIP;                                                                 \
        }                                                                                   \
    } while (0)

#define KD_CHECK(cond, ...)            \
    do {                               \
        if (!(cond)) {                 \
            ::kd::set_error(__VA_ARGS__); \
            return KD_EINVAL;          \
        }                              \
    } while (0)

struct DevBuf {
    void* p = nullptr;
    size_t bytes = 0;
    bool slab = false;
};

struct ProfStat {
    u64 launches = 0;
    double ms = 0;
};

struct PendingEv {
    std::string name;
    hipEvent_t a, b;
};

}

struct kd_opts {
    int merge3_join = 1;
    int merge3_split = 0;
    int j3_ol = 0;
    int j3_v = 1;
    uint64_t j2_oidlds_min = 1ull << 26;
    int j2r = 0;
    int fd_stream = -1;
    int fd_walk = -1;
    uint64_t pkm_max_blocks = 1ull << 26;
    int trace_host = 0;
};

struct kd_ctx {
    int device = 0;
    kd_opts opt;
    hipStream_t own_stream = nullptr;
    hipStream_t stream = nullptr;
    std::map<std::string, kd::DevBuf> bufs;
    bool prof = false;
    std::string prof_only;
    std::vector<hipEvent_t> ev_pool;
    std::vector<kd::PendingEv> pending;
    std::map<std::string, kd::ProfStat> stats;
    std::vector<uint8_t> fd_tab;
    int n_cu = 256;
    void* comm = nullptr;
    int nranks = 1, rank = 0;
    std::vector<int> group_devs;
    std::vector<void*> group_comms;
    hipStream_t comm_stream = nullptr;
    hipEvent_t ev_counts = nullptr, ev_gathered = nullptr;
    uint64_t* h_counts_pin = nullptr;
    int h_counts_ranks = 0;
    uint64_t gather_send_cap = 0;
    int occ_resolve3 = 0;
    std::map<std::tuple<const void*, int, size_t>, int> occ;
    uint32_t rs_epoch = 0;
    int pkm_cur = 0;
    void* pkm_zero_ptr[2] = {nullptr, nullptr};
    uint64_t pkm_zero_nb[2] = {0, 0};
    char* slab = nullptr;
    size_t slab_used = 0;
    char* pin[2] = {nullptr, nullptr};
    void* pin_dev[2] = {nullptr, nullptr};
    hipEvent_t pin_ev[2] = {nullptr, nullptr};
    int pin_next = 0;
};

namespace kd {

void gather_release(kd_ctx* ctx);
int ensure(kd_ctx* ctx, const char* slot, size_t bytes, void** out);
int stage_h2d(kd_ctx* ctx, void* dst, const void* src, size_t bytes);
void host_mark(kd_ctx* ctx, const char* name);
int stage_d2h(kd_ctx* ctx, void* dst, const void* src, size_t bytes);

int device_zeros(kd_ctx* ctx, void** out);

int occupancy(kd_ctx* ctx, const void* kernel, int block, size_t lds);

void prof_begin(kd_ctx* ctx, const char* name, hipEvent_t* a);
void prof_end(kd_ctx* ctx, const char* name, hipEvent_t a);
int prof_flush(kd_ctx* ctx);

inline bool prof_on(const kd_ctx* ctx, const char* name) {
    return ctx->prof && (ctx->prof_only.empty() || ctx->prof_only.find("," + std::string(name) + ",") != std::string::npos);
}

template <typename F>
inline int launch(kd_ctx* ctx, const char* name, F&& f) {
    hipEvent_t a = nullptr;
    const bool prof = prof_on(ctx, name);
    if (prof) prof_begin(ctx, name, &a);
    f();
    hipError_t e = hipGetLastError();
    if (prof) prof_end(ctx, name, a);
    if (e != hipSuccess) {
        set_error("launch %s: %s", name, hipGetErrorString(e));
        return KD_EHIP;
    }
    return KD_OK;
}

int stage_in(kd_ctx* ctx, const char* slot, const void* p, size_t bytes, u32 mem, const void** dev);
int stage_side(kd_ctx* ctx, const kd_side* s, const char* tag, kd_side* dev);
int check_side(const kd_side* s, const char* which);
void comm_release(kd_ctx* ctx);

int resolve3_have_a(kd_ctx* ctx, const kd_side& K, const kd_side& O, const kd_side& T, const u32* cand3, const u64* c2,
                    u32* d_conf, uint2* d_md, u64* d_counts, u32* d_err, const u32* ordK, const u32* ordO,
                    const u32* ordT);
int merge3_join_device(kd_ctx* ctx, const kd_side& K, const kd_side& O, const kd_side& T, u32* d_conf, uint2* d_md,
                       u64* d_counts, u32* d_err, const u32* ordK = nullptr, const u32* ordO = nullptr,
                       const u32* ordT = nullptr);
int diff2_device(kd_ctx* ctx, const kd_side* A, const kd_side* B, u32 flags, u32* d_delta,
                 u32* d_upd, u64* d_counts, u32* d_err, const u32* ordA = nullptr, const u32* ordB = nullptr,
                 u64* d_dkey = nullptr, u64* d_ukey = nullptr);
#ifndef KD_C2_NT
#define KD_C2_NT 256
#endif
constexpr int C2_NT = KD_C2_NT;
#ifndef KD_C2_IPT
#define KD_C2_IPT 4
#endif
constexpr int C2_IPT = KD_C2_IPT;
constexpr int C2_TILE = C2_NT * C2_IPT;

}
```

kart_amd/csrc/kd_sort.hip:

```cpp
#include "kd_internal.h"
#include "kd_walkkey.h"

namespace kd {

#ifndef KD_RS_RB
#define KD_RS_RB 9
#endif
constexpr int RS_RB = KD_RS_RB;
constexpr int RS_RD = 1 << RS_RB;
constexpr int RS_MAXRUNS = 4;
constexpr int RS_HIST_NT = 256, RS_HIST_IPT = 16;
#ifndef KD_RS_NT
#define KD_RS_NT 512
#endif
#ifndef KD_RS_IPT32
#define KD_RS_IPT32 16
#endif
#ifndef KD_RS_IPT64
#define KD_RS_IPT64 8
#endif
constexpr int RS_NT = KD_RS_NT;

struct SortPlan {
    u64 kconst;
// ... 244 lines not shown
        u32 x[CPT], s = 0;
#pragma unroll
        for (int j = 0; j < CPT; j++) {
            const u32 L = (u32)(tid * CPT + j);
            x[j] = s_cnt[rs_ci<NW>(L / NW, L % NW)];
            s += x[j];
        }
        u32 inc = s;
#pragma unroll
        for (int o = 1; o < 64; o <<= 1) {
            const u32 y = __shfl_up(inc, o, 64);
            if (lane >= o) inc += y;
        }
        if (lane == 63) s_wsum[wv] = inc;
        __syncthreads();
        u32 ex = inc - s;
#pragma unroll
        for (int w = 0; w < NW; w++)
            if (w < wv) ex += s_wsum[w];
#pragma unroll
        for (int j = 0; j < CPT; j++) {
            const u32 L = (u32)(tid * CPT + j);
            s_cnt[rs_ci<NW>(L / NW, L % NW)] = (u16)ex;
            ex += x[j];
        }
    }
    __syncthreads();
    const u32 dstart = tid < RS_RD ? (u32)s_cnt[rs_ci<NW>(tid, 0)] : 0;
#pragma unroll
    for (int i = 0; i < IPT; i++) {
        if (wbase + (u64)i * 64 < n) {
            const u32 d = (u32)(c[i] >> shift) & dmask;
            const u32 p = s_cnt[rs_ci<NW>(d, wv)] + rk[i];
            s_key[p] = c[i];
            s_val[p] = v[i];
        }
    }
    if (tid < RS_RD) {
        u64 ex = 0;
#ifdef KD_RS_PROBE_NOLB
        if (false) {
#else
        if (tile > 0) {
#endif
            i64 t = (i64)tile - 1;
            while (true) {
                u64 w[RS_LBW];
#pragma unroll
                for (int k = 0; k < RS_LBW; k++) w[k] = t - k >= 0 ? rs_load(status + (u64)(t - k) * RS_RD + tid) : RS_INC;
                int used = 0;
                bool done = false;
#pragma unroll
                for (int k = 0; k < RS_LBW; k++) {
                    if (done || used < k) continue;
                    const u64 x = w[k];
                    const bool ready = (x >> 62) != 0 && ((u32)((x >> 40) & (RS_EPOCHS - 1)) == epoch || t - k < 0);
                    if (!ready) continue;
                    ex += x & RS_CNT;
                    used = k + 1;
                    done = (x >> 62) == 2;
                }
                if (done) break;
                t -= used;
                if (used < RS_LBW) __builtin_amdgcn_s_sleep(1);
            }
            rs_store(st, RS_INC | ((u64)epoch << 40) | (ex + dcnt));
        }
        s_goff[tid] = gbase[tid] + (u32)ex - dstart;
    }
    __syncthreads();
    for (u32 j = tid; j < valid; j += NT) {
        const CK k = s_key[j];
        const u32 x = s_val[j];
        const u32 dst = s_goff[(u32)(k >> shift) & dmask] + j;
        if (LAST) ((u64*)kout)[dst] = rs_expand((u64)k, plan) ^ plan.out_xor;
        else ((CK*)kout)[dst] = k;
        vout[dst] = x;
    }
    __syncthreads();
    }
}

__global__ __launch_bounds__(256) void k_gather_oid(const u8* __restrict__ in, const u32* __restrict__ order, u64 n,
                                                    u8* __restrict__ out) {
    typedef const __attribute__((address_space(1))) u32* gp32;
    __shared__ __attribute__((aligned(16))) u32 s_rows[4][64 * 5];
    const int lane = threadIdx.x & 63, wv = threadIdx.x >> 6;
    u32* R = s_rows[wv];
    const bool al16 = ((uintptr_t)out & 15) == 0;
    for (u64 r0 = ((u64)blockIdx.x * 4 + wv) * 64; r0 < n; r0 += (u64)gridDim.x * 256) {
        const u64 k = r0 + lane;
        const u32 m = (u32)min<u64>(64, n - r0);
        if (k < n) {
            const gp32 s = (gp32)(in + 20ull * order[k]);
            const u32 a = s[0], b = s[1], c = s[2], e = s[3], f = s[4];
            R[5 * lane] = a; R[5 * lane + 1] = b; R[5 * lane + 2] = c; R[5 * lane + 3] = e; R[5 * lane + 4] = f;
        }
        __builtin_amdgcn_wave_barrier();
        u32* d = (u32*)(out + 20ull * r0);
        if (m == 64 && al16) {
            const u32x4* S = (const u32x4*)R;
            ((u32x4*)d)[lane] = S[lane];
            if (lane < 16) ((u32x4*)d)[64 + lane] = S[64 + lane];
        } else {
            for (u32 j = lane; j < 5 * m; j += 64) d[j] = R[j];
        }
        __builtin_amdgcn_wave_barrier();
    }
}

__global__ __launch_bounds__(256) void k_iota_u32(u32* __restrict__ out, u64 n) {
    for (u64 i = (u64)blockIdx.x * 256 + threadIdx.x; i < n; i += (u64)gridDim.x * 256) out[i] = (u32)i;
}

__global__ __launch_bounds__(256) void k_check_sorted(const u64* __restrict__ key, u64 n, u32* __restrict__ dup) {
    bool bad = false;
    for (u64 i = (u64)blockIdx.x * 256 + threadIdx.x + 1; i < n; i += (u64)gridDim.x * 256) bad |= key[i - 1] >= key[i];
    if (__ballot(bad) && (threadIdx.x & 63) == 0) atomicOr(dup, 1u);
}

template <typename CK>
__global__ __launch_bounds__(RS_HIST_NT) void k_dpk_keys(const uint2* __restrict__ rec, u64 ncap, const u64* __restrict__ dn,
                                                          const u64* __restrict__ kA, const u64* __restrict__ kB,
                                                          const u64* __restrict__ rkey,
                                                          int npass, int width, SortPlan plan, CK* __restrict__ out,
                                                          u32* __restrict__ hist) {
    __shared__ u32 s_h[8 * RS_RD];
    const int tid = threadIdx.x;
    for (int i = tid; i < npass * RS_RD; i += RS_HIST_NT) s_h[i] = 0;
    __syncthreads();
    const u64 n = min(*dn, ncap);
    const u32 dmask = (1u << width) - 1;
    for (u64 r = (u64)blockIdx.x * RS_HIST_NT + tid; r < n; r += (u64)gridDim.x * RS_HIST_NT) {
        u64 key;
        if (rkey) key = rkey[r];
        else {
            const uint2 d = rec[r];
            key = d.x != KD_NONE ? kA[d.x] : kB[d.y];
        }
        const u64 sk = (u64)wk::int_key_pk(key) ^ (1ull << 63);
        const CK c = rs_compact<CK>(sk, plan);
        out[r] = c;
        for (int p = 0; p < npass; p++) atomicAdd(&s_h[p * RS_RD + ((u32)(c >> (p * width)) & dmask)], 1u);
    }
    __syncthreads();
    for (int i = tid; i < npass * RS_RD; i += RS_HIST_NT)
        if (s_h[i]) atomicAdd(&hist[i], s_h[i]);
}

#ifndef KD_PKM_IPT
#define KD_PKM_IPT 16
#endif
constexpr int PKM_NT = 256, PKM_IPT = KD_PKM_IPT, PKM_CH = PKM_NT * PKM_IPT;

__global__ __launch_bounds__(PKM_NT) void k_pkm_mark(const uint2* __restrict__ rec, u64 ncap, const u64* __restrict__ dn,
                                                     const u64* __restrict__ kA, const u64* __restrict__ kB,
                                                     const u64* __restrict__ rkey, i64 lo_block, u64 nb,
                                                     u64* __restrict__ masks, i64* __restrict__ pk_out) {
    const u64 n = min(*dn, ncap);
    const int lane = threadIdx.x & 63;
    const u64 stride = (u64)gridDim.x * PKM_NT;
    for (u64 base = (u64)blockIdx.x * PKM_NT + (threadIdx.x & ~63); base < n; base += stride) {
        const u64 r = base + lane;
        const bool ok = r < n;
        i64 pk = 0;
        if (ok) {
            u64 key;
            if (rkey) key = rkey[r];
            else {
                const uint2 d = rec[r];
                key = d.x != KD_NONE ? kA[d.x] : kB[d.y];
            }
            pk = wk::int_key_pk(key);
            if (!rkey) pk_out[r] = pk;
        }
        const u64 b = (u64)((pk >> 6) - lo_block);
        const bool inb = ok && b < nb;
        u64 bit = inb ? 1ull << (pk & 63) : 0;
        const u64 bprev = __shfl_up(b, 1, 64);
        const bool head = inb && (lane == 0 || bprev != b);
        const u64 heads = __ballot(head);
        const u64 later = lane == 63 ? 0 : heads & (~0ull << (lane + 1));
        const int seg_end = later ? __ffsll((long long)later) - 1 : 64;
#pragma unroll
        for (int o = 1; o < 64; o <<= 1) {
            const u64 v = __shfl_down(bit, o, 64);
            if (lane + o < seg_end) bit |= v;
        }
        if (head) atomicOr((unsigned long long*)(masks + b), (unsigned long long)bit);
    }
}

static_assert(PKM_IPT % 4 == 0, "k_pkm_scan: 16-B loads and stores");
__global__ __launch_bounds__(PKM_NT) void k_pkm_scan(const u64* __restrict__ masks, u64 nb, u32* __restrict__ local,
                                                     u32* __restrict__ chunk_tot, u64* __restrict__ zero) {
    __shared__ u32 s_wave[PKM_NT / 64];
    const int tid = threadIdx.x;
    const u64 c0 = (u64)blockIdx.x * PKM_CH + (u64)tid * PKM_IPT;
    u32 cnt[PKM_IPT], sum = 0;
    if (c0 + PKM_IPT <= nb) {
        const u32x4* m4 = (const u32x4*)(masks + c0);
#pragma unroll
        for (int j = 0; j < PKM_IPT / 2; j++) {
            const u32x4 v = m4[j];
            cnt[2 * j] = (u32)__popc(v.x) + (u32)__popc(v.y);
            cnt[2 * j + 1] = (u32)__popc(v.z) + (u32)__popc(v.w);
        }
        u32x4* z4 = (u32x4*)(zero + c0);
#pragma unroll
        for (int j = 0; j < PKM_IPT / 2; j++) z4[j] = u32x4{0u, 0u, 0u, 0u};
    } else {
#pragma unroll
        for (int j = 0; j < PKM_IPT; j++) {
            cnt[j] = c0 + j < nb ? (u32)__popcll(masks[c0 + j]) : 0u;
            if (c0 + j < nb) zero[c0 + j] = 0;
        }
    }
#pragma unroll
    for (int j = 0; j < PKM_IPT; j++) sum += cnt[j];
    u32 tot;
    u32 ex = block_scan_u32<PKM_NT>(sum, s_wave, &tot);
    if (c0 + PKM_IPT <= nb) {
        u32x4* l4 = (u32x4*)(local + c0);
#pragma unroll
        for (int j = 0; j < PKM_IPT / 4; j++) {
            u32x4 o;
            o.x = ex; ex += cnt[4 * j];
            o.y = ex; ex += cnt[4 * j + 1];
            o.z = ex; ex += cnt[4 * j + 2];
            o.w = ex; ex += cnt[4 * j + 3];
            l4[j] = o;
        }
    } else {
#pragma unroll
        for (int j = 0; j < PKM_IPT; j++) {
            if (c0 + j < nb) local[c0 + j] = ex;
            ex += cnt[j];
        }
    }
    if (tid == 0) chunk_tot[blockIdx.x] = tot;
}

constexpr int PKC_PT = 8;
__global__ __launch_bounds__(1024) void k_pkm_cscan(const u32* __restrict__ chunk_tot, u32 nch, u32* __restrict__ chunk_pre) {
    __shared__ u32 s_wave[1024 / 64];
    const int tid = threadIdx.x;
    u32 carry = 0;
    for (u32 base = 0; base < nch; base += 1024 * PKC_PT) {
        const u32 k0 = base + (u32)tid * PKC_PT;
        u32 v[PKC_PT], sum = 0;
#pragma unroll
        for (int j = 0; j < PKC_PT; j++) {
            v[j] = k0 + j < nch ? chunk_tot[k0 + j] : 0u;
            sum += v[j];
        }
        u32 t2;
        u32 e = block_scan_u32<1024>(sum, s_wave, &t2);
#pragma unroll
        for (int j = 0; j < PKC_PT; j++) {
            if (k0 + j < nch) chunk_pre[k0 + j] = carry + e;
            e += v[j];
        }
        carry += t2;
        __syncthreads();
    }
}

__global__ __launch_bounds__(PKM_NT) void k_pkm_place(const i64* __restrict__ pks, const u64* __restrict__ rkey, u64 ncap,
                                                      const u64* __restrict__ dn, i64 lo_block, u64 nb,
                                                      const u64* __restrict__ masks, const u32* __restrict__ local,
                                                      const u32* __restrict__ chunk_pre, i64* __restrict__ out_pk,
                                                      u32* __restrict__ out_perm) {
    const u64 n = min(*dn, ncap);
    for (u64 r = (u64)blockIdx.x * PKM_NT + threadIdx.x; r < n; r += (u64)gridDim.x * PKM_NT) {
        const i64 pk = rkey ? wk::int_key_pk(rkey[r]) : pks[r];
        const u64 b = (u64)((pk >> 6) - lo_block);
        if (b >= nb) continue;
        const u64 below = masks[b] & ((1ull << (pk & 63)) - 1);
        const u32 pos = chunk_pre[b / PKM_CH] + local[b] + (u32)__popcll(below);
        out_pk[pos] = pk;
        out_perm[pos] = (u32)r;
    }
}

constexpr int RS_SEG_MAX = 512;
#ifndef KD_SEG_IPT
#define KD_SEG_IPT 8
#endif
constexpr int SEG_NT = 256, SEG_IPT = KD_SEG_IPT, SEG_T = SEG_NT * SEG_IPT, SEG_HS = 128;

template <bool MAX>
__device__ __forceinline__ u32 seg_block_scan(u32 v, u32* s_w, bool reverse) {
    const int lane = threadIdx.x & 63, wv = threadIdx.x >> 6;
    constexpr int NW = SEG_NT / 64;
    u32 x = v;
#pragma unroll
    for (int o = 1; o < 64; o <<= 1) {
        const u32 y = reverse ? __shfl_down(x, o, 64) : __shfl_up(x, o, 64);
        const bool in = reverse ? lane + o < 64 : lane >= o;
        if (in) x = MAX ? (y > x ? y : x) : (y < x ? y : x);
    }
    if (lane == (reverse ? 0 : 63)) s_w[wv] = x;
    __syncthreads();
#pragma unroll
    for (int w = 0; w < NW; w++) {
        const u32 y = s_w[w];
        if (reverse ? w > wv : w < wv) x = MAX ? (y > x ? y : x) : (y < x ? y : x);
    }
    __syncthreads();
    return x;
}

template <int SEG_H, bool BM>
__global__ __launch_bounds__(SEG_NT) void k_seg_sort(const u64* __restrict__ key, u64 n, int shift, u64* __restrict__ kout,
                                                     u32* __restrict__ order, u32* __restrict__ err) {
    constexpr int SEG_E = SEG_T + 2 * SEG_H, SEG_EPT = SEG_E / SEG_NT;
    static_assert(SEG_E % SEG_NT == 0 && SEG_E < 65536, "segmented-sort tile shape");
    __shared__ u64 s_k[SEG_E];
    __shared__ u64 s_bm[BM ? SEG_E / 2 : 1];
    __shared__ u16 s_st[SEG_E];
    __shared__ u16 s_en[SEG_E];
    __shared__ u32 s_w[SEG_NT / 64];
    __shared__ u32 s_inc[SEG_NT];
    const int tid = threadIdx.x;
    const u64 ntiles = (n + SEG_T - 1) / SEG_T;
    auto geo = [&](u64 t, i64& g0, int& vlo, int& vhi) {
        g0 = (i64)(t * SEG_T) - SEG_H;
        vlo = g0 < 0 ? (int)(-g0) : 0;
        vhi = (int)min<i64>((i64)SEG_E, (i64)n - g0);
    };
    u64 v[SEG_EPT];
    auto fetch = [&](u64 t) {
        i64 g0;
        int vlo, vhi;
        geo(t, g0, vlo, vhi);
        const char* kt = (const char*)(key + g0);
#pragma unroll
        for (int j = 0; j < SEG_EPT; j++) {
            const int x = tid + j * SEG_NT;
            const u32 xc = (u32)(x < vlo ? vlo : (x >= vhi ? vhi - 1 : x));
            v[j] = *(const u64*)(kt + 8u * xc);
        }
    };
    u64 tile = blockIdx.x;
    if (tile < ntiles) fetch(tile);
    u32 bad = 0;
    for (; tile < ntiles; tile += gridDim.x) {
        i64 g0;
        int vlo, vhi;
        geo(tile, g0, vlo, vhi);
#pragma unroll
        for (int j = 0; j < SEG_EPT; j++) {
            const int x = tid + j * SEG_NT;
            s_k[x] = (x >= vlo && x < vhi) ? v[j] : 0;
        }
        __syncthreads();
        if (tile + gridDim.x < ntiles) fetch(tile + gridDim.x);
        static_assert(SEG_EPT <= 32, "head bits");
        const int x0 = tid * SEG_EPT;
        u64 kk[SEG_EPT + 1];
        kk[0] = x0 > 0 ? s_k[x0 - 1] : 0;
#pragma unroll
        for (int j = 0; j < SEG_EPT; j++) kk[j + 1] = s_k[x0 + j];
        u32 hm = 0;
#pragma unroll
        for (int j = 0; j < SEG_EPT; j++) {
            const int x = x0 + j;
            const bool valid = x >= vlo && x < vhi;
            const bool head = !valid || x == vlo || ((kk[j + 1] ^ kk[j]) >> shift) != 0;
            hm |= head ? 1u << j : 0u;
            if (head && valid && x > vlo && x >= SEG_H && x < SEG_H + SEG_T && (kk[j + 1] >> shift) < (kk[j] >> shift))
                bad |= 1u;
        }
        u32 st_loc[SEG_EPT], en_loc[SEG_EPT];
        u32 runp1 = 0;
#pragma unroll
        for (int j = 0; j < SEG_EPT; j++) {
            if ((hm >> j) & 1u) runp1 = (u32)(x0 + j) + 1;
            st_loc[j] = runp1;
        }
        u32 nxt = SEG_E;
#pragma unroll
        for (int j = SEG_EPT - 1; j >= 0; j--) {
            en_loc[j] = nxt;
            if ((hm >> j) & 1u) nxt = (u32)(x0 + j);
        }
        const u32 fwd = seg_block_scan<true>(runp1, s_w, false);
        s_inc[tid] = fwd;
        __syncthreads();
        const u32 before = tid ? s_inc[tid - 1] : 0u;
        __syncthreads();
        const u32 bwd = seg_block_scan<false>(nxt, s_w, true);
        s_inc[tid] = bwd;
        __syncthreads();
        const u32 after = tid + 1 < SEG_NT ? s_inc[tid + 1] : (u32)SEG_E;
#pragma unroll
        for (int j = 0; j < SEG_EPT; j++) {
            s_st[x0 + j] = (u16)((st_loc[j] ? st_loc[j] : before) - 1);
            s_en[x0 + j] = (u16)(en_loc[j] != (u32)SEG_E ? en_loc[j] : after);
        }
        __syncthreads();
        if (BM) {
#pragma unroll
            for (int j = 0; j < SEG_EPT; j++) {
                const int x = x0 + j;
                const u32 s0 = s_st[x], len = s_en[x] - s0;
                if (x >= vlo && x < vhi && (u32)x == s0 && len >= 2 && len <= 64) s_bm[x >> 1] = 0;
            }
            __syncthreads();
            u64 acc = 0;
            u32 cur = 0;
#pragma unroll
            for (int j = 0; j < SEG_EPT; j++) {
                const int x = x0 + j;
                const u32 s0 = s_st[x], len = s_en[x] - s0;
                if (s0 != cur) {
                    if (acc) atomicOr((unsigned long long*)&s_bm[cur >> 1], acc);
                    acc = 0;
                    cur = s0;
                }
                if (x >= vlo && x < vhi && len >= 2 && len <= 64) {
                    const u64 k = s_k[x], hk = s_k[s0];
                    if (((k ^ hk) >> 6) == 0) acc |= 1ull << (k & 63);
                }
            }
            if (acc) atomicOr((unsigned long long*)&s_bm[cur >> 1], acc);
            __syncthreads();
        }
        char* const ko = (char*)(kout + g0);
        char* const oo = (char*)(order + g0);
        const u32 og = (u32)g0;
        const bool lo_open = g0 > 0, hi_open = g0 + SEG_E < (i64)n;
// ... 184 lines not shown
    } else {
        void* bits;
        if ((rc = ensure(ctx, "rs.bits", 16, &bits))) return rc;
        KD_HIP(hipMemsetAsync(bits, 0, 16, ctx->stream));
        rc = launch(ctx, "k_rs_bits", [&] {
            hipLaunchKernelGGL(k_rs_bits, dim3(gs), dim3(256), 0, ctx->stream, key_in, n, (u64*)bits);
        });
        if (rc) return rc;
        u64 hv[2] = {0, 0};
        KD_HIP(hipMemcpyAsync(hv, bits, 8, hipMemcpyDeviceToHost, ctx->stream));
        KD_HIP(hipMemcpyAsync(hv + 1, key_in, 8, hipMemcpyDeviceToHost, ctx->stream));
        KD_HIP(hipStreamSynchronize(ctx->stream));
        vary = hv[0];
        k0 = hv[1];
    }
    if (vary == 0) {
        if (key_out != key_in) KD_HIP(hipMemcpyAsync(key_out, key_in, n * 8, hipMemcpyDeviceToDevice, ctx->stream));
        return launch(ctx, "k_iota", [&] {
            hipLaunchKernelGGL(k_iota_u32, dim3(gs), dim3(256), 0, ctx->stream, order, n);
        });
    }
    const SortPlan plan = make_plan(vary, k0);
    int npass, width;
    plan_passes(plan, &npass, &width);
    if (inplace && npass == 1) {
        void* tmp;
        if ((rc = ensure(ctx, "rs.kin", n * 8, &tmp))) return rc;
        KD_HIP(hipMemcpyAsync(tmp, key_in, n * 8, hipMemcpyDeviceToDevice, ctx->stream));
        key_in = (const u64*)tmp;
    }
    SortState S;
    if ((rc = rs_state(ctx, npass, S))) return rc;
    const bool narrow = plan.bits <= 32;
    constexpr u64 HCH = (u64)RS_HIST_NT * RS_HIST_IPT;
    const unsigned hg = (unsigned)std::max<u64>(1, std::min<u64>((n + HCH - 1) / HCH, (u64)ctx->n_cu * 2));
    rc = launch(ctx, "k_sort_hist", [&] {
        if (narrow)
            hipLaunchKernelGGL(k_sort_hist<u32>, dim3(hg), dim3(RS_HIST_NT), 0, ctx->stream, key_in, n, (const u64*)nullptr,
                               npass, width, plan, S.hist);
        else
            hipLaunchKernelGGL(k_sort_hist<u64>, dim3(hg), dim3(RS_HIST_NT), 0, ctx->stream, key_in, n, (const u64*)nullptr,
                               npass, width, plan, S.hist);
    });
    if (rc) return rc;
    rc = launch(ctx, "k_sort_scan", [&] {
        hipLaunchKernelGGL(k_sort_scan, dim3(1), dim3(RS_RD), 0, ctx->stream, (const u32*)S.hist, npass, S.gbase);
    });
    if (rc) return rc;
    return narrow ? rs_passes<u32>(ctx, S, key_in, true, key_out, order, n, nullptr, npass, width, plan)
                  : rs_passes<u64>(ctx, S, key_in, true, key_out, order, n, nullptr, npass, width, plan);
}

static int gather_and_check(kd_ctx* ctx, const u8* oid_in, u8* oid_out, const u32* order, const u64* key_sorted, u64 n,
                            u32* d_dup) {
    const unsigned gs = (unsigned)std::max<u64>(1, std::min<u64>((n + 255) / 256, (u64)ctx->n_cu * 8));
    int rc;
    if (oid_in) {
        if ((rc = launch(ctx, "k_gather_oid", [&] {
                 hipLaunchKernelGGL(k_gather_oid, dim3(gs), dim3(256), 0, ctx->stream, oid_in, order, n, oid_out);
             })))
            return rc;
    }
    if (d_dup) {
        KD_HIP(hipMemsetAsync(d_dup, 0, 4, ctx->stream));
        if ((rc = launch(ctx, "k_check_sorted", [&] {
                 hipLaunchKernelGGL(k_check_sorted, dim3(gs), dim3(256), 0, ctx->stream, key_sorted, n, d_dup);
             })))
            return rc;
    }
    return KD_OK;
}

static SortPlan pk_plan(i64 lo, i64 hi) {
    const u64 a = (u64)lo ^ (1ull << 63), b = (u64)hi ^ (1ull << 63);
    const u64 d = a ^ b;
    const u64 vary = d ? (d >> 63 ? ~0ull : ((1ull << (64 - __builtin_clzll(d))) - 1)) : 0;
    SortPlan p = make_plan(vary, a);
    p.out_xor = 1ull << 63;
    return p;
}

}

using namespace kd;

extern "C" int kd_sort_side_into(kd_ctx* ctx, const uint64_t* d_key_in, const uint8_t* d_oid_in, uint64_t* d_key_out,
                                 uint8_t* d_oid_out, uint32_t* d_order, uint64_t n, uint32_t* d_dup,
                                 const kd_keys_info* info) {
    KD_CHECK(ctx && (n == 0 || (d_key_in && d_key_out && d_order)), "kd_sort_side_into: NULL");
    KD_CHECK(!d_oid_in == !d_oid_out, "kd_sort_side_into: OID input and output go together");
    KD_CHECK(n < 0xFFFFFFFFull, "kd_sort_side_into: side too large for uint32 indices");
    KD_CHECK(n == 0 || ((const void*)d_key_in != (const void*)d_key_out &&
                        (!d_oid_in || (const void*)d_oid_in != (const void*)d_oid_out)),
             "kd_sort_side_into: outputs must not alias the inputs (kd_sort_side sorts in place)");
    KD_HIP(hipSetDevice(ctx->device));
    if (n == 0) {
        if (d_dup) KD_HIP(hipMemsetAsync(d_dup, 0, 4, ctx->stream));
        return KD_OK;
    }
    int rc = sort_keys(ctx, d_key_in, d_key_out, d_order, n, false, info);
    if (rc) return rc;
    return gather_and_check(ctx, d_oid_in, d_oid_out, d_order, d_key_out, n, d_dup);
}

extern "C" int kd_sort_side(kd_ctx* ctx, uint64_t* d_key, uint8_t* d_oid, uint32_t* d_order, uint64_t n,
                            uint32_t* h_dup) {
    KD_CHECK(ctx && (n == 0 || (d_key && d_order)), "kd_sort_side: NULL");
    KD_CHECK(n < 0xFFFFFFFFull, "kd_sort_side: side too large for uint32 indices");
    KD_HIP(hipSetDevice(ctx->device));
    if (h_dup) *h_dup = 0;
    if (n == 0) return KD_OK;
    int rc = sort_keys(ctx, d_key, d_key, d_order, n, true, nullptr);
    if (rc) return rc;
    void *o2 = nullptr, *dup = nullptr;
    if (d_oid && (rc = ensure(ctx, "rs.oid", n * 20, &o2))) return rc;
    if (h_dup && (rc = ensure(ctx, "rs.dup", 16, &dup))) return rc;
    if ((rc = gather_and_check(ctx, d_oid, (u8*)o2, d_order, d_key, n, (u32*)dup))) return rc;
    if (d_oid) KD_HIP(hipMemcpyAsync(d_oid, o2, n * 20, hipMemcpyDeviceToDevice, ctx->stream));
    if (h_dup) {
        KD_HIP(hipMemcpyAsync(h_dup, dup, 4, hipMemcpyDeviceToHost, ctx->stream));
        KD_HIP(hipStreamSynchronize(ctx->stream));
    }
    return KD_OK;
}

extern "C" int kd_sort_segmented_into(kd_ctx* ctx, const uint64_t* d_key_in, uint64_t* d_key_out, uint32_t* d_order,
                                      uint64_t n, int seg_bits, int max_seg, uint32_t* d_err) {
    KD_CHECK(ctx && d_err && (n == 0 || (d_key_in && d_key_out && d_order)), "kd_sort_segmented_into: NULL");
    KD_CHECK(n < 0xFFFFFFFFull, "kd_sort_segmented_into: side too large for uint32 indices");
    KD_CHECK(seg_bits > 0 && seg_bits < 64, "kd_sort_segmented_into: seg_bits %d", seg_bits);
    KD_CHECK(n == 0 || (const void*)d_key_in != (const void*)d_key_out, "kd_sort_segmented_into: output aliases input");
    KD_HIP(hipSetDevice(ctx->device));
    if (n == 0) return KD_OK;
    const u64 ntiles = (n + SEG_T - 1) / SEG_T;
    const bool small = max_seg > 0 && max_seg <= SEG_HS;
    const bool bm = small && max_seg > 16;
    const unsigned grid = (unsigned)ntiles;
    return launch(ctx, "k_seg_sort", [&] {
        if (small && bm)
            hipLaunchKernelGGL((k_seg_sort<SEG_HS, true>), dim3(grid), dim3(SEG_NT), 0, ctx->stream, d_key_in, n,
                               64 - seg_bits, d_key_out, d_order, d_err);
        else if (small)
            hipLaunchKernelGGL((k_seg_sort<SEG_HS, false>), dim3(grid), dim3(SEG_NT), 0, ctx->stream, d_key_in, n,
                               64 - seg_bits, d_key_out, d_order, d_err);
        else
            hipLaunchKernelGGL((k_seg_sort<RS_SEG_MAX, false>), dim3(grid), dim3(SEG_NT), 0, ctx->stream, d_key_in, n,
                               64 - seg_bits, d_key_out, d_order, d_err);
    });
}

extern "C" int kd_delta_pk_order(kd_ctx* ctx, const kd_side* base, const kd_side* target, const uint32_t* d_delta,
                                 const uint64_t* d_keys, uint64_t cap, const uint64_t* d_n, int64_t pk_lo, int64_t pk_hi,
                                 int64_t* d_pk, uint32_t* d_perm) {
    KD_CHECK(ctx && base && target && d_n && d_pk && d_perm && (cap == 0 || d_delta || d_keys), "kd_delta_pk_order: NULL");
    KD_CHECK(base->key_mode == KD_KEY_INT && target->key_mode == KD_KEY_INT, "kd_delta_pk_order: KD_KEY_INT sides only");
    KD_CHECK(base->mem == KD_MEM_DEVICE && target->mem == KD_MEM_DEVICE, "kd_delta_pk_order: sides must be device memory");
    KD_CHECK(pk_lo <= pk_hi, "kd_delta_pk_order: pk_lo > pk_hi");
    KD_CHECK(cap < 0xFFFFFFFFull, "kd_delta_pk_order: too many deltas for uint32 indices");
    KD_HIP(hipSetDevice(ctx->device));
    if (cap == 0) return KD_OK;
    int rc;
    void* dz;
    if ((rc = device_zeros(ctx, &dz))) return rc;
    const u64* kA = base->n ? base->key : (const u64*)dz;
    const u64* kB = target->n ? target->key : (const u64*)dz;
    const i64 lo_block = pk_lo >> 6, hi_block = pk_hi >> 6;
    const u64 nb = (u64)hi_block - (u64)lo_block + 1;
    const u64 pkm_max = ctx->opt.pkm_max_blocks;
    if (nb <= pkm_max && nb / PKM_CH < 0xFFFFFFFFull) {
        void *mbuf[2], *local, *ctot, *cpre, *tpk;
        const u64 nch = (nb + PKM_CH - 1) / PKM_CH;
        if ((rc = ensure(ctx, "pkm.masks0", nb * 8, &mbuf[0]))) return rc;
        if ((rc = ensure(ctx, "pkm.masks1", nb * 8, &mbuf[1]))) return rc;
        const int cur = ctx->pkm_cur & 1;
        void* const masks = mbuf[cur];
        void* const other = mbuf[cur ^ 1];
        if ((rc = ensure(ctx, "pkm.local", nb * 4, &local))) return rc;
        if ((rc = ensure(ctx, "pkm.ctot", nch * 4, &ctot))) return rc;
        if ((rc = ensure(ctx, "pkm.cpre", nch * 4, &cpre))) return rc;
        if ((rc = ensure(ctx, "pkm.pk", cap * 8, &tpk))) return rc;
        ctx->pkm_zero_nb[cur ^ 1] = 0;
        if (ctx->pkm_zero_ptr[cur] != masks || ctx->pkm_zero_nb[cur] < nb) {
            ctx->pkm_zero_nb[cur] = 0;
            KD_HIP(hipMemsetAsync(masks, 0, nb * 8, ctx->stream));
        }
        ctx->pkm_zero_nb[cur] = 0;
        const unsigned g1 = (unsigned)std::max<u64>(1, std::min<u64>((cap + PKM_NT - 1) / PKM_NT, (u64)ctx->n_cu * 8));
        rc = launch(ctx, "k_pkm_mark", [&] {
            hipLaunchKernelGGL(k_pkm_mark, dim3(g1), dim3(PKM_NT), 0, ctx->stream, (const uint2*)d_delta, cap, d_n, kA,
                               kB, d_keys, lo_block, nb, (u64*)masks, (i64*)tpk);
        });
        if (rc) return rc;
        rc = launch(ctx, "k_pkm_scan", [&] {
            hipLaunchKernelGGL(k_pkm_scan, dim3((unsigned)nch), dim3(PKM_NT), 0, ctx->stream, (const u64*)masks, nb,
                               (u32*)local, (u32*)ctot, (u64*)other);
        });
        if (rc) return rc;
        ctx->pkm_zero_ptr[cur ^ 1] = other;
        ctx->pkm_zero_nb[cur ^ 1] = nb;
        ctx->pkm_cur = cur ^ 1;
        rc = launch(ctx, "k_pkm_cscan", [&] {
            hipLaunchKernelGGL(k_pkm_cscan, dim3(1), dim3(1024), 0, ctx->stream, (const u32*)ctot, (u32)nch, (u32*)cpre);
        });
        if (rc) return rc;
        return launch(ctx, "k_pkm_place", [&] {
            hipLaunchKernelGGL(k_pkm_place, dim3(g1), dim3(PKM_NT), 0, ctx->stream, (const i64*)tpk, d_keys, cap, d_n,
                               lo_block, nb, (const u64*)masks, (const u32*)local, (const u32*)cpre, d_pk, d_perm);
        });
    }
    SortPlan plan = pk_plan(pk_lo, pk_hi);
    int npass, width;
    plan_passes(plan, &npass, &width);
    if (npass == 0) {
        plan.nruns = 1; plan.mask[0] = 1; plan.lo[0] = 0; plan.pos[0] = 0; plan.bits = 1;
        plan.kconst = ((u64)pk_lo ^ (1ull << 63)) & ~1ull;
        npass = width = 1;
    }
    const bool narrow = plan.bits <= 32;
    void* ck;
    if ((rc = ensure(ctx, "dpk.keys", cap * (narrow ? 4 : 8), &ck))) return rc;
    SortState S;
    if ((rc = rs_state(ctx, npass, S))) return rc;
    const unsigned hg = (unsigned)std::max<u64>(1, std::min<u64>((cap + RS_HIST_NT - 1) / RS_HIST_NT, (u64)ctx->n_cu * 4));
    rc = launch(ctx, "k_dpk_keys", [&] {
        if (narrow)
            hipLaunchKernelGGL(k_dpk_keys<u32>, dim3(hg), dim3(RS_HIST_NT), 0, ctx->stream, (const uint2*)d_delta, cap, d_n,
                               kA, kB, d_keys, npass, width, plan, (u32*)ck, S.hist);
        else
            hipLaunchKernelGGL(k_dpk_keys<u64>, dim3(hg), dim3(RS_HIST_NT), 0, ctx->stream, (const uint2*)d_delta, cap, d_n,
                               kA, kB, d_keys, npass, width, plan, (u64*)ck, S.hist);
    });
    if (rc) return rc;
    rc = launch(ctx, "k_sort_scan", [&] {
        hipLaunchKernelGGL(k_sort_scan, dim3(1), dim3(RS_RD), 0, ctx->stream, (const u32*)S.hist, npass, S.gbase);
    });
    if (rc) return rc;
    return narrow ? rs_passes<u32>(ctx, S, ck, false, (u64*)d_pk, d_perm, cap, d_n, npass, width, plan)
                  : rs_passes<u64>(ctx, S, ck, false, (u64*)d_pk, d_perm, cap, d_n, npass, width, plan);
}
```

kart_amd/device.py:

```python
import ctypes

import numpy as np

from . import _native as N


class DevBuf:

    def __init__(self, engine, nbytes):
        self.eng = engine
        self.nbytes = int(nbytes)
        p = ctypes.c_void_p()
        N.check(engine.L.kd_malloc(engine.ctx, max(self.nbytes, 16), ctypes.byref(p)), "kd_malloc")
        self.ptr = p.value

    @classmethod
    def from_numpy(cls, engine, a):
        a = np.ascontiguousarray(a)
        b = cls(engine, a.nbytes)
        b.upload(a)
        return b

    def upload(self, a, offset=0, sync=True):
        a = np.ascontiguousarray(a)
# ... 19 lines not shown

    def free(self):
        if self.ptr and self.eng.ctx:
            self.eng.L.kd_mfree(self.eng.ctx, self.ptr)
        self.ptr = None

    def __del__(self):
        try:
            self.free()
        except Exception:
            pass


def _nonempty(a, dtype, width=1):
    return a if a is not None and a.size else np.zeros(width, dtype)


class DevSide:

    def __init__(self, engine, side, keys_only=False):
        if keys_only:
            self.n, self.key_mode = side.n, side.key_mode
            self.key = DevBuf.from_numpy(engine, _nonempty(side.key, np.uint64))
            self.oid = DevBuf.from_numpy(engine, np.zeros(20, np.uint8))
            self.name = self.name_off = None
            return
        if getattr(side, "walk_rows", False):
            raise ValueError("DevSide needs a key-ordered side; a late-materialised side joins through its order "
                             "(side.materialised() gives the sorted form)")
        self.n = side.n
        self.key_mode = side.key_mode
        self.key = DevBuf.from_numpy(engine, _nonempty(side.key, np.uint64))
        self.oid = DevBuf.from_numpy(engine, _nonempty(side.oid.reshape(-1) if side.n else None, np.uint8, 20))
        self.name = self.name_off = None
        if side.name is not None:
            self.name = DevBuf.from_numpy(engine, _nonempty(side.name, np.uint8))
            self.name_off = DevBuf.from_numpy(engine, side.name_off)

    def kd_side(self):
        s = N.KdSide()
        s.n = self.n
        s.key = self.key.ptr
        s.oid = self.oid.ptr
        s.name = self.name.ptr if self.name is not None else None
        s.name_off = self.name_off.ptr if self.name_off is not None else None
        s.mem = N.KD_MEM_DEVICE
        s.key_mode = self.key_mode
        return s


class DevPermSide:

    def __init__(self, engine, n, key_mode, key, oid, order, name=None, name_off=None):
        self.n, self.key_mode = int(n), key_mode
        self.key, self.oid, self.order, self.name, self.name_off = key, oid, order, name, name_off

    def kd_side(self):
        s = N.KdSide()
        s.n = self.n
        s.key, s.oid = self.key.ptr, self.oid.ptr
        s.name = self.name.ptr if self.name is not None else None
        s.name_off = self.name_off.ptr if self.name_off is not None else None
        s.mem = N.KD_MEM_DEVICE
        s.key_mode = self.key_mode
        return s


def perm_dev(engine, side):
    if side.dperm is not None:
        return side.dperm.kd_side(), side.dperm.order, side.dperm
    ds = DevSide(engine, side)
    order = DevBuf.from_numpy(engine, np.arange(max(side.n, 1), dtype=np.uint32))
    return ds.kd_side(), order, (ds, order)


class _WalkSide:

    def __init__(self, side, perm):
        self.key, self.oid = np.ascontiguousarray(side.key[perm]), np.ascontiguousarray(side.oid[perm])
        self.n = int(side.n)
        self.key_mode = side.key_mode
        self.name = self.name_off = None
        if side.name is not None:
            lens = (side.name_off[1:] - side.name_off[:-1])[perm]
            off = np.zeros(self.n + 1, np.uint64)
            np.cumsum(lens, out=off[1:])
            src = side.name_off[:-1][perm].astype(np.int64)
            idx = np.arange(int(off[-1]), dtype=np.int64) + np.repeat(src - off[:-1].astype(np.int64), lens.astype(np.int64))
            self.name, self.name_off = np.ascontiguousarray(side.name[idx]), off


class DevBlobs:

    def __init__(self, engine, data, off):
        self.n = int(off.shape[0]) - 1
        self.data = DevBuf.from_numpy(engine, _nonempty(data, np.uint8))
        self.off = DevBuf.from_numpy(engine, off)
        self.nbytes = int(data.size)
        nz = int(np.count_nonzero(off[1:] != off[:-1])) if self.n else 0
        self.mean_len = int((int(off[-1]) - int(off[0]) + nz - 1) // nz) if nz else 0

    def kd_blobs(self):
        b = N.KdBlobs()
        b.n = self.n
        b.data = self.data.ptr
        b.off = self.off.ptr
        b.mem = N.KD_MEM_DEVICE
        b.size_hint = min(self.mean_len, 0xFFFFFFFF)
        return b


class DiffPipeline:

    def __init__(self, engine, base, target, base_blobs, target_blobs, maps, ordered=True, gather=None, unsorted=None,
                 late=True, pk_order=True, radix=False):
        from . import packing

        self.eng = engine
        self.flags = 0 if ordered else N.KD_DIFF_UNORDERED
        self.A = DevSide(engine, base)
        self.B = DevSide(engine, target)
        self.walk = None
        self.late = bool(late) and gather is None
        self.seg_err = None
        if unsorted is not None:
            self.walk = []
            for side, perm in zip((base, target), unsorted):
                w = _WalkSide(side, perm)
                info = packing.keys_scan(w.key, side.key_mode)
                self.walk.append((DevSide(engine, w), DevBuf(engine, 4 * max(side.n, 1)), side.n, info))
            self.segmented = self.late and not radix and all(0 < x[3].seg_max <= packing.SEG_SORT_MAX for x in self.walk)
            if self.segmented:
                self.seg_err = DevBuf(engine, 8)
                self.seg_err.zero()
        self.OB = DevBlobs(engine, *base_blobs)
        self.NB = DevBlobs(engine, *target_blobs)
        self.OB_off_host, self.NB_off_host = base_blobs[1], target_blobs[1]
        self.OB_data_host, self.NB_data_host = base_blobs[0], target_blobs[0]
        self._ob_u = None
        self.maps = maps
        cap = base.n + target.n + 1
        self.cap = cap
        self.cap_upd = min(base.n, target.n)
        self.delta = DevBuf(engine, 8 * cap)
        self.upd = DevBuf(engine, 8 * cap)
        self.counts = DevBuf(engine, 64)
        self.counts.zero()
        self.masks = DevBuf(engine, 8 * cap * maps.words)
        self.status = DevBuf(engine, cap)
        self._sa, self._sb = self.A.kd_side(), self.B.kd_side()
        self._ob, self._nb = self.OB.kd_blobs(), self.NB.kd_blobs()
        self._km = maps.kd_maps()
        self._perm_sides = None
        self.pk_order = bool(pk_order) and base.key_mode == N.KD_KEY_INT and gather is None
        if self.pk_order:
            lo, hi = [], []
            for side in (base, target):
                info = side.info if side.info is not None else packing.keys_scan(side.key, side.key_mode)
                if side.n:
                    lo.append(int(info.pk_min))
                    hi.append(int(info.pk_max))
            self.pk_range = (min(lo), max(hi)) if lo else (0, 0)
            self.d_pk = DevBuf(engine, 8 * cap)
            self.d_perm = DevBuf(engine, 4 * cap)
            self.dkey = DevBuf(engine, 8 * cap)
            self.ukey = DevBuf(engine, 8 * cap)
            self.u_pk = DevBuf(engine, 8 * max(self.cap_upd, 1))
            self.u_perm = DevBuf(engine, 4 * max(self.cap_upd, 1))
        self.gather = gather
        if gather is not None:
            self.world = engine.nranks
            self.all_counts = DevBuf(engine, 64 * self.world)
            self.h_counts = np.zeros(8 * self.world, np.uint64)
            self.all_cap = cap * self.world
            self.all_delta = DevBuf(engine, 8 * self.all_cap)
        engine.reserve(max(base.n, target.n))
        engine.sync()

    def use_update_arenas(self, upd):
        m = int(upd.shape[0])
        self._u_arenas = []
        blobs = []
        for side, off_h, dev in ((0, self.OB_off_host, self.OB), (1, self.NB_off_host, self.NB)):
            idx = np.asarray(upd[:, side], np.int64)
            start = off_h[idx]
            lens = off_h[idx + 1] - start
            off = np.zeros(m + 1, np.uint64)
            np.cumsum(lens, out=off[1:])
            if m == 0 or np.array_equal(start, start[0] + off[:-1]):
                u = DevBuf.from_numpy(self.eng, off + (np.uint64(start[0]) if m else np.uint64(0)))
                self._u_arenas.append(u)
                b = dev.kd_blobs()
                b.n, b.off = m, u.ptr
            else:
                data = (self.OB_data_host, self.NB_data_host)[side]
                pos = np.repeat(start.astype(np.int64) - off[:-1].astype(np.int64), lens.astype(np.int64)) + \
                    np.arange(int(off[-1]), dtype=np.int64)
                arena = DevBlobs(self.eng, np.ascontiguousarray(data[pos]), off)
                self._u_arenas.append(arena)
                b = arena.kd_blobs()
            blobs.append(b)
        self._ob_u, self._nb_u = blobs

    def reserve_gather(self, max_deltas_per_rank):
        self.all_delta.free()
        self.all_cap = max(int(max_deltas_per_rank), 1) * self.world
        self.all_delta = DevBuf(self.eng, 8 * self.all_cap)

    def sort_step(self):
        L, ctx = self.eng.L, self.eng.ctx
        for (w, order, n, info), S in zip(self.walk, (self.A, self.B)):
            if self.segmented:
                N.check(L.kd_sort_segmented_into(ctx, w.key.ptr, S.key.ptr, order.ptr, n, 24, info.seg_max, self.seg_err.ptr),
                        "kd_sort_segmented_into")
            elif self.late:
                N.check(L.kd_sort_side_into(ctx, w.key.ptr, None, S.key.ptr, None, order.ptr, n, None,
                                            ctypes.byref(info)), "kd_sort_side_into")
            else:
                N.check(L.kd_sort_side_into(ctx, w.key.ptr, w.oid.ptr, S.key.ptr, S.oid.ptr, order.ptr, n, None,
                                            ctypes.byref(info)), "kd_sort_side_into")

    def orders(self):
        return [order.download(np.uint32, n) for _, order, n, _ in self.walk]

    def step(self):
        if self.walk is not None:
            self.sort_step()
        self._diff(self.walk is not None and self.late)

    def diff_step(self):
        self._diff(False)

    def _diff(self, perm):
        L, ctx = self.eng.L, self.eng.ctx
        keys = self.pk_order and self.flags == 0
        if perm:
            if self._perm_sides is None:
                self._perm_sides = []
                for S, (w, _, _, _) in zip((self.A, self.B), self.walk):
                    k = S.kd_side()
                    k.oid = w.oid.ptr
                    if w.name is not None:
                        k.name, k.name_off = w.name.ptr, w.name_off.ptr
                    self._perm_sides.append(k)
            N.check(L.kd_diff2_device_ex(ctx, ctypes.byref(self._perm_sides[0]), ctypes.byref(self._perm_sides[1]),
                                         self.walk[0][1].ptr, self.walk[1][1].ptr, self.flags, self.delta.ptr,
                                         self.upd.ptr, self.dkey.ptr if keys else None, self.ukey.ptr if keys else None,
                                         self.counts.ptr, self.counts.ptr + 32), "kd_diff2_device_ex")
        elif self.gather is None:
            N.check(L.kd_diff2_device_ex(ctx, ctypes.byref(self._sa), ctypes.byref(self._sb), None, None, self.flags,
                                         self.delta.ptr, self.upd.ptr, self.dkey.ptr if keys else None,
                                         self.ukey.ptr if keys else None, self.counts.ptr, self.counts.ptr + 32),
                    "kd_diff2_device_ex")
        else:
            N.check(L.kd_diff2_gather_begin(ctx, ctypes.byref(self._sa), ctypes.byref(self._sb), self.gather[0],
                                            self.gather[1], self.flags, self.delta.ptr, self.upd.ptr, self.counts.ptr,
                                            self.counts.ptr + 32, self.all_counts.ptr), "kd_diff2_gather_begin")
        if self._ob_u is not None:
            N.check(L.kd_fielddiff(ctx, ctypes.byref(self._ob_u), ctypes.byref(self._nb_u), None, self.cap_upd,
                                   ctypes.cast(self.counts.ptr + 8, N.c_u64p), N.KD_MEM_DEVICE,
                                   ctypes.byref(self._km), self.masks.ptr, self.status.ptr, N.KD_MEM_DEVICE),
                    "kd_fielddiff")
        else:
            N.check(L.kd_fielddiff(ctx, ctypes.byref(self._ob), ctypes.byref(self._nb), self.upd.ptr, self.cap_upd,
                               ctypes.cast(self.counts.ptr + 8, N.c_u64p), N.KD_MEM_DEVICE,
                                   ctypes.byref(self._km), self.masks.ptr, self.status.ptr, N.KD_MEM_DEVICE),
                    "kd_fielddiff")
        if keys:
            lo, hi = self.pk_range
            N.check(L.kd_delta_pk_order(ctx, ctypes.byref(self._sa), ctypes.byref(self._sb), self.delta.ptr,
                                        self.dkey.ptr, self.cap, self.counts.ptr + 24, lo, hi, self.d_pk.ptr,
                                        self.d_perm.ptr), "kd_delta_pk_order")
            N.check(L.kd_delta_pk_order(ctx, ctypes.byref(self._sa), ctypes.byref(self._sb), self.upd.ptr,
                                        self.ukey.ptr, max(self.cap_upd, 1), self.counts.ptr + 8, lo, hi, self.u_pk.ptr,
                                        self.u_perm.ptr), "kd_delta_pk_order")
        if self.gather is not None:
            N.check(L.kd_diff2_gather_end(ctx, self.delta.ptr, self.all_delta.ptr, self.all_cap,
                                          self.h_counts.ctypes.data), "kd_diff2_gather_end")

    def results(self):
        c = self.counts.download(np.uint64, 8)
        if c[4]:
            raise N.Unsupported(N.KD_EUNSUPPORTED, f"device error flag {int(c[4])}")
        if self.seg_err is not None and int(self.seg_err.download(np.uint32, 1)[0]):
            raise N.Unsupported(N.KD_EUNSUPPORTED, "per-leaf-tree sort flagged a long or descending leaf tree")
        nd, nu = int(c[3]), int(c[1])
        delta = self.delta.download(np.uint32, 2 * nd).reshape(nd, 2)
        upd = self.upd.download(np.uint32, 2 * nu).reshape(nu, 2)
        masks = self.masks.download(np.uint64, nu * self.maps.words).reshape(nu, self.maps.words)
        status = self.status.download(np.uint8, nu)
        return {"inserts": int(c[0]), "updates": nu, "deletes": int(c[2]), "deltas": nd}, delta, upd, masks, status

    def pk_results(self):
        c = self.counts.download(np.uint64, 8)
        nd, nu = int(c[3]), int(c[1])
        return (self.d_pk.download(np.int64, nd), self.d_perm.download(np.uint32, nd),
                self.u_pk.download(np.int64, nu), self.u_perm.download(np.uint32, nu))

    def gathered(self):
        stride = int(self.h_counts.reshape(self.world, 8)[:, 3].max())
        rec = self.all_delta.download(np.uint32, 2 * stride * self.world)
        return assemble_gathered(self.h_counts, rec, self.world)


def assemble_gathered(h_counts, records, world):
    c = np.asarray(h_counts, np.uint64).reshape(world, 8)
    if c[:, 4].any():
        raise N.Unsupported(N.KD_EUNSUPPORTED, f"device error flags {c[:, 4].tolist()}")
    stride = int(c[:, 3].max())
    rec = np.asarray(records, np.uint32)[:2 * stride * world].reshape(world, stride, 2)
    delta = np.concatenate([rec[r, :int(c[r, 3])] for r in range(world)]) if stride else np.zeros((0, 2), np.uint32)
    return {"inserts": int(c[:, 0].sum()), "updates": int(c[:, 1].sum()), "deletes": int(c[:, 2].sum()),
            "deltas": int(c[:, 3].sum())}, delta


class FilterPipeline:

    def __init__(self, engine, base, target, base_blobs, target_blobs, geom_cols, filt_env, rectangle=False, bits=20,
                 heads=False, delta_order=False, gather=False):
        import ctypes as _c

        self.eng = engine
        self.A, self.B = DevSide(engine, base), DevSide(engine, target)
        self.OB, self.NB = DevBlobs(engine, *base_blobs), DevBlobs(engine, *target_blobs)
        cap = base.n + target.n + 1
        self.cap = cap
        self.bits = bits
        self.delta = DevBuf(engine, 8 * cap)
        self.upd = DevBuf(engine, 8 * cap)
        self.counts = DevBuf(engine, 64)
        self.counts.zero()
        self.match = DevBuf(engine, 2 * cap)
        self.keep = DevBuf(engine, 4 * cap)
        self.n_keep = DevBuf(engine, 8)
        self.enc = DevBuf(engine, cap * max(bits // 2, 1)) if bits else None
        self.enc_ok = DevBuf(engine, cap) if bits else None
        self._sa, self._sb = self.A.kd_side(), self.B.kd_side()
        self._ob, self._nb = self.OB.kd_blobs(), self.NB.kd_blobs()
        self.cols = geom_cols
        self._kc = geom_cols.kd_cols()
        self._fe = (_c.c_double * 4)(*[float(x) for x in filt_env])
        self.flags = N.KD_GF_RECT if rectangle else 0
        self.heads = None
        self.heads_s = None
        self.heads_host = None
        self.delta_order = bool(delta_order) and heads
        self.gather = bool(gather) and self.delta_order
        self.dheads = None
        self.delta_heads_s = None
        if heads:
            import time

            from .spatial import geom_heads

            t0 = time.perf_counter()
            hs = [geom_heads(*base_blobs, geom_cols.old_hex, geom_cols.old_gidx, len(geom_cols.old_map)),
                  geom_heads(*target_blobs, geom_cols.new_hex, geom_cols.new_gidx, len(geom_cols.new_map))]
            self.heads_s = time.perf_counter() - t0
            self.heads_host = hs
            self.heads = [(DevBuf.from_numpy(engine, h.view(np.uint8).reshape(-1)) if h.size else DevBuf(engine, 48), h.size)
                          for h in hs]
        engine.reserve(max(base.n, target.n))
        engine.sync()
        if self.delta_order and not self.gather:
            self._build_delta_heads()

    def _classify(self):
        L, ctx = self.eng.L, self.eng.ctx
        N.check(L.kd_diff2_device(ctx, ctypes.byref(self._sa), ctypes.byref(self._sb), 0, self.delta.ptr, self.upd.ptr,
                                  self.counts.ptr, self.counts.ptr + 32), "kd_diff2_device")

    def _build_delta_heads(self):
        import time

        self._classify()
        c = self.counts.download(np.uint64, 8)
        nd = int(c[3])
        delta = self.delta.download(np.uint32, 2 * nd).reshape(nd, 2)
        t0 = time.perf_counter()
        slots = max((self.cap + 63) // 64 * 64, 64)
        self.dheads = []
        for s in range(2):
            col = delta[:, s]
            pres = np.nonzero(col != N.KD_NONE)[0]
            h = np.zeros(slots, self.heads_host[s].dtype)
            h[pres] = self.heads_host[s][col[pres].astype(np.int64)]
            self.dheads.append((DevBuf.from_numpy(self.eng, h.view(np.uint8).reshape(-1)), slots))
        self.delta_heads_s = time.perf_counter() - t0
        self.eng.sync()

    def step(self):
        L, ctx = self.eng.L, self.eng.ctx
        self._classify()
        if self.delta_order:
            if self.gather:
                (ho, no), (hn, nn) = self.heads
                flags = self.flags
            else:
                (ho, no), (hn, nn) = self.dheads
                flags = self.flags | N.KD_GF_DELTA_HEADS
            N.check(L.kd_geom_filter_deltas(ctx, ho.ptr, no, hn.ptr, nn, ctypes.byref(self._ob), ctypes.byref(self._nb),
                                            self.delta.ptr, self.cap, ctypes.cast(self.counts.ptr + 24, N.c_u64p),
                                            self._fe, flags, self.bits, self.match.ptr, self.keep.ptr,
                                            ctypes.cast(self.n_keep.ptr, N.c_u64p), self.enc.ptr if self.enc else None,
                                            self.enc_ok.ptr if self.enc_ok else None), "kd_geom_filter_deltas")
            return
        if self.heads is not None:
            (ho, no), (hn, nn) = self.heads
            N.check(L.kd_geom_filter_heads(ctx, ho.ptr, no, hn.ptr, nn, N.KD_MEM_DEVICE, ctypes.byref(self._ob),
                                           ctypes.byref(self._nb), self.delta.ptr, self.cap,
                                           ctypes.cast(self.counts.ptr + 24, N.c_u64p), N.KD_MEM_DEVICE, self._fe,
                                           self.flags, self.bits, self.match.ptr, self.keep.ptr,
                                           ctypes.cast(self.n_keep.ptr, N.c_u64p), self.enc.ptr if self.enc else None,
                                           self.enc_ok.ptr if self.enc_ok else None, N.KD_MEM_DEVICE),
                    "kd_geom_filter_heads")
            return
        N.check(L.kd_geom_filter(ctx, ctypes.byref(self._ob), ctypes.byref(self._nb), self.delta.ptr, self.cap,
                                 ctypes.cast(self.counts.ptr + 24, N.c_u64p), N.KD_MEM_DEVICE, ctypes.byref(self._kc),
                                 self._fe, self.flags, self.bits, self.match.ptr, self.keep.ptr,
                                 ctypes.cast(self.n_keep.ptr, N.c_u64p), self.enc.ptr if self.enc else None,
                                 self.enc_ok.ptr if self.enc_ok else None, N.KD_MEM_DEVICE), "kd_geom_filter")

    def results(self):
        c = self.counts.download(np.uint64, 8)
        if c[4]:
            raise N.Unsupported(N.KD_EUNSUPPORTED, f"device error flag {int(c[4])}")
        nd = int(c[3])
        k = int(self.n_keep.download(np.uint64, 1)[0])
        nb = self.bits // 2
        return ({"inserts": int(c[0]), "updates": int(c[1]), "deletes": int(c[2]), "deltas": nd, "kept": k},
                self.delta.download(np.uint32, 2 * nd).reshape(nd, 2), self.match.download(np.uint8, 2 * nd).reshape(nd, 2),
# ... 62 lines not shown
```

Baseline: 34370 M feature-pairs/s.

## Add fused diff2 step API overlapping field diff with placement and pk ordering on side stream

Introduces a single kd_diff2_step entry point that runs the classify front-end and then forks the placement kernel and pk-order passes onto a second stream while the field diff runs on the main stream, joined with events. The Python side caches the step argument struct per form, cutting per-call ctypes overhead and several separate library calls. It also adds wave-level (LDS-free) variants of the pk scan and chunk-scan kernels for use when sharing the GPU concurrently. This adds stream and event management, a sync on the side stream before buffer reallocation, and relies on the scratch buffers not being shared between the two concurrent branches.

```diff
diff --git a/include/kartdiff.h b/include/kartdiff.h
--- a/include/kartdiff.h
+++ b/include/kartdiff.h
@@ -179,6 +179,36 @@
 int kd_delta_pk_order(kd_ctx* ctx, const kd_side* base, const kd_side* target, const uint32_t* d_delta,
                       const uint64_t* d_keys, uint64_t cap, const uint64_t* d_n, int64_t pk_lo, int64_t pk_hi,
                       int64_t* d_pk, uint32_t* d_perm);
+
+typedef struct kd_step {
+    const kd_side* base;
+    const kd_side* target;
+    const uint32_t* base_order;
+    const uint32_t* target_order;
+    uint32_t flags;
+    uint32_t reserved;
+    uint32_t* d_delta;
+    uint32_t* d_upd;
+    uint64_t* d_delta_key;
+    uint64_t* d_upd_key;
+    uint64_t* d_counts;
+    uint32_t* d_err;
+    const kd_blobs* old_blobs;
+    const kd_blobs* new_blobs;
+    const uint32_t* d_pairs;
+    uint64_t upd_cap;
+    const kd_legend_maps* maps;
+    uint64_t* d_masks;
+    uint8_t* d_status;
+    int64_t pk_lo;
+    int64_t pk_hi;
+    uint64_t delta_cap;
+    int64_t* d_delta_pk;
+    uint32_t* d_delta_perm;
+    int64_t* d_upd_pk;
+    uint32_t* d_upd_perm;
+} kd_step;
+int kd_diff2_step(kd_ctx* ctx, const kd_step* step);
 
 #define KD_COPY_H2D 1u
 #define KD_COPY_D2H 2u
diff --git a/kart_amd/_native.py b/kart_amd/_native.py
--- a/kart_amd/_native.py
+++ b/kart_amd/_native.py
@@ -99,6 +99,37 @@
     ]
 
 
+class KdStep(ctypes.Structure):
+    _fields_ = [
+        ("base", ctypes.POINTER(KdSide)),
+        ("target", ctypes.POINTER(KdSide)),
+        ("base_order", ctypes.c_void_p),
+        ("target_order", ctypes.c_void_p),
+        ("flags", ctypes.c_uint32),
+        ("reserved", ctypes.c_uint32),
+        ("d_delta", ctypes.c_void_p),
+        ("d_upd", ctypes.c_void_p),
+        ("d_delta_key", ctypes.c_void_p),
+        ("d_upd_key", ctypes.c_void_p),
+        ("d_counts", ctypes.c_void_p),
+        ("d_err", ctypes.c_void_p),
+        ("old_blobs", ctypes.POINTER(KdBlobs)),
+        ("new_blobs", ctypes.POINTER(KdBlobs)),
+        ("d_pairs", ctypes.c_void_p),
+        ("upd_cap", ctypes.c_uint64),
+        ("maps", ctypes.POINTER(KdLegendMaps)),
+        ("d_masks", ctypes.c_void_p),
+        ("d_status", ctypes.c_void_p),
+        ("pk_lo", ctypes.c_int64),
+        ("pk_hi", ctypes.c_int64),
+        ("delta_cap", ctypes.c_uint64),
+        ("d_delta_pk", ctypes.c_void_p),
+        ("d_delta_perm", ctypes.c_void_p),
+        ("d_upd_pk", ctypes.c_void_p),
+        ("d_upd_perm", ctypes.c_void_p),
+    ]
+
+
 class KdGeomCols(ctypes.Structure):
     _fields_ = [
         ("n_leg_old", ctypes.c_int32),
@@ -246,6 +277,7 @@
                                            ctypes.c_void_p, ctypes.c_void_p, ctypes.c_uint32, ctypes.c_void_p,
                                            ctypes.c_void_p, ctypes.c_void_p, ctypes.c_void_p, ctypes.c_void_p,
                                            ctypes.c_void_p]),
+    "kd_diff2_step": (ctypes.c_int, [ctypes.c_void_p, ctypes.POINTER(KdStep)]),
     "kd_malloc": (ctypes.c_int, [ctypes.c_void_p, ctypes.c_uint64, ctypes.POINTER(ctypes.c_void_p)]),
     "kd_mfree": (ctypes.c_int, [ctypes.c_void_p, ctypes.c_void_p]),
     "kd_host_alloc": (ctypes.c_int, [ctypes.c_uint64, ctypes.POINTER(ctypes.c_void_p)]),
diff --git a/kart_amd/csrc/kd_classify.hip b/kart_amd/csrc/kd_classify.hip
--- a/kart_amd/csrc/kd_classify.hip
+++ b/kart_amd/csrc/kd_classify.hip
@@ -457,6 +457,86 @@
     return diff2_device(ctx, base, target, flags, d_delta, d_upd, d_counts, d_err, oa, ob, d_delta_key, d_upd_key);
 }
 
+int kd_diff2_step(kd_ctx* ctx, const kd_step* s) {
+    KD_CHECK(ctx && s, "kd_diff2_step: NULL");
+    int rc;
+    if ((rc = check_side(s->base, "base")) || (rc = check_side(s->target, "target"))) return rc;
+    KD_CHECK(s->base->mem == KD_MEM_DEVICE && s->target->mem == KD_MEM_DEVICE, "kd_diff2_step: sides must be device memory");
+    KD_CHECK(s->d_delta && s->d_counts && s->d_err, "kd_diff2_step: NULL output");
+    KD_CHECK(!s->base_order == !s->target_order, "kd_diff2_step: both orders or neither");
+    KD_CHECK(!s->d_upd_key || (s->d_upd && s->d_delta_key), "kd_diff2_step: update keys need the update list and delta keys");
+    const bool have_fd = s->old_blobs != nullptr;
+    KD_CHECK(!have_fd || (s->new_blobs && s->maps && s->d_masks && s->d_status), "kd_diff2_step: field diff: NULL argument");
+    const bool have_dpk = s->d_delta_pk != nullptr, have_upk = s->d_upd_pk != nullptr;
+    KD_CHECK(!have_dpk || s->d_delta_perm, "kd_diff2_step: d_delta_pk without d_delta_perm");
+    KD_CHECK(!have_upk || (s->d_upd_perm && s->d_upd), "kd_diff2_step: d_upd_pk needs d_upd_perm and the update list");
+    KD_HIP(hipSetDevice(ctx->device));
+    void* dz = nullptr;
+    if ((rc = device_zeros(ctx, &dz))) return rc;
+    const u32* oa = s->base_order ? (s->base->n ? s->base_order : (const u32*)dz) : nullptr;
+    const u32* ob = s->target_order ? (s->target->n ? s->target_order : (const u32*)dz) : nullptr;
+    Diff2Place pl;
+    if ((rc = diff2_front(ctx, s->base, s->target, s->flags, s->d_delta, s->d_upd, s->d_counts, s->d_err, oa, ob,
+                          s->d_delta_key, s->d_upd_key, &pl)))
+        return rc;
+    const int ov = ctx->opt.step_overlap;
+    auto field_diff = [&]() -> int {
+        return have_fd ? kd_fielddiff(ctx, s->old_blobs, s->new_blobs, s->d_pairs, s->upd_cap, s->d_counts + 1,
+                                      KD_MEM_DEVICE, s->maps, s->d_masks, s->d_status, KD_MEM_DEVICE)
+                       : KD_OK;
+    };
+    auto pk_orders = [&](bool lds_free) -> int {
+        int r = KD_OK;
+        if (have_dpk)
+            r = delta_pk_order(ctx, s->base, s->target, s->d_delta, s->d_delta_key, s->delta_cap, s->d_counts + 3,
+                               s->pk_lo, s->pk_hi, s->d_delta_pk, s->d_delta_perm, lds_free);
+        if (!r && have_upk)
+            r = delta_pk_order(ctx, s->base, s->target, s->d_upd, s->d_upd_key, s->upd_cap, s->d_counts + 1, s->pk_lo,
+                               s->pk_hi, s->d_upd_pk, s->d_upd_perm, lds_free);
+        return r;
+    };
+    const bool place_aside = !(have_fd && s->d_pairs);
+    const bool overlap = ov > 0 && have_fd && pl.needed && (place_aside || have_dpk || have_upk) &&
+                         s->base->n + s->target->n >= ctx->opt.step_overlap_min;
+    const int wave = ctx->opt.pkm_wave;
+    if (!overlap) {
+        if ((rc = diff2_place(ctx, pl)) || (rc = field_diff())) return rc;
+        return pk_orders(wave > 0);
+    }
+    if (!ctx->side_stream) {
+        KD_HIP(hipStreamCreateWithFlags(&ctx->side_stream, hipStreamNonBlocking));
+        KD_HIP(hipEventCreateWithFlags(&ctx->ev_fork, hipEventDisableTiming));
+        KD_HIP(hipEventCreateWithFlags(&ctx->ev_join, hipEventDisableTiming));
+    }
+    const hipStream_t main = ctx->stream, side = ctx->side_stream;
+    if (!place_aside && (rc = diff2_place(ctx, pl))) return rc;
+    KD_HIP(hipEventRecord(ctx->ev_fork, main));
+    auto side_work = [&]() -> int {
+        StreamScope scope(ctx, side);
+        KD_HIP(hipStreamWaitEvent(side, ctx->ev_fork, 0));
+        int r = place_aside ? diff2_place(ctx, pl) : KD_OK;
+        return r ? r : pk_orders(wave != 0);
+    };
+    int rc_fd, rc_side = KD_OK;
+    if (ov == 2) {
+        rc_side = side_work();
+        rc_fd = field_diff();
+    } else {
+        rc_fd = field_diff();
+        if (!rc_fd) rc_side = side_work();
+    }
+    hipError_t e = hipEventRecord(ctx->ev_join, side);
+    if (e == hipSuccess) e = hipStreamWaitEvent(main, ctx->ev_join, 0);
+    if (e != hipSuccess) {
+        const hipError_t e2 = hipStreamSynchronize(side);
+        if (!rc_fd && !rc_side) {
+            set_error("kd_diff2_step: join: %s", hipGetErrorString(e2 != hipSuccess ? e2 : e));
+            return KD_EHIP;
+        }
+    }
+    return rc_fd ? rc_fd : rc_side;
+}
+
 int kd_diff2(kd_ctx* ctx, const kd_side* base, const kd_side* target, uint32_t flags, kd_diff_result** out) {
     KD_CHECK(ctx && out, "kd_diff2: NULL");
     int rc;
diff --git a/kart_amd/csrc/kd_classify2.hip b/kart_amd/csrc/kd_classify2.hip
--- a/kart_amd/csrc/kd_classify2.hip
+++ b/kart_amd/csrc/kd_classify2.hip
@@ -1668,6 +1668,14 @@
 
 int diff2_device(kd_ctx* ctx, const kd_side* A, const kd_side* B, u32 flags, u32* d_delta, u32* d_upd,
                  u64* d_counts, u32* d_err, const u32* ordA, const u32* ordB, u64* d_dkey, u64* d_ukey) {
+    Diff2Place pl;
+    int rc = diff2_front(ctx, A, B, flags, d_delta, d_upd, d_counts, d_err, ordA, ordB, d_dkey, d_ukey, &pl);
+    return rc ? rc : diff2_place(ctx, pl);
+}
+
+int diff2_front(kd_ctx* ctx, const kd_side* A, const kd_side* B, u32 flags, u32* d_delta, u32* d_upd, u64* d_counts,
+                u32* d_err, const u32* ordA, const u32* ordB, u64* d_dkey, u64* d_ukey, Diff2Place* pl) {
+    *pl = Diff2Place{};
     const bool unord = (flags & KD_DIFF_UNORDERED) != 0;
     const u64 nA = A->n, nB = B->n, total = nA + nB;
     KD_CHECK(nA < 0xFFFFFFFFull && nB < 0xFFFFFFFFull, "diff2: side too large for uint32 indices");
@@ -1754,10 +1762,20 @@
                            (u64*)gpre, d_counts, 0);
     });
     if (rc) return rc;
+    pl->needed = true;
+    pl->ntiles = ntiles;
+    pl->sdel = sdel; pl->tcnt = tcnt; pl->gpre = gpre; pl->skd = skd;
+    pl->d_delta = d_delta; pl->d_upd = d_upd;
+    pl->d_dkey = d_dkey; pl->d_ukey = d_upd ? d_ukey : nullptr;
+    return KD_OK;
+}
+
+int diff2_place(kd_ctx* ctx, const Diff2Place& pl) {
+    if (!pl.needed) return KD_OK;
     return launch(ctx, "k_place2", [&] {
-        hipLaunchKernelGGL((k_place2<KD_PLACE_NT>), dim3((unsigned)ntiles), dim3(KD_PLACE_NT), 0, ctx->stream,
-                           (const uint2*)sdel, (const u32*)tcnt, (const u64*)gpre, (int)C2_STAGE, (uint2*)d_delta,
-                           (uint2*)d_upd, (const u64*)skd, d_dkey, d_upd ? d_ukey : nullptr);
+        hipLaunchKernelGGL((k_place2<KD_PLACE_NT>), dim3((unsigned)pl.ntiles), dim3(KD_PLACE_NT), 0, ctx->stream,
+                           (const uint2*)pl.sdel, (const u32*)pl.tcnt, (const u64*)pl.gpre, (int)C2_STAGE,
+                           (uint2*)pl.d_delta, (uint2*)pl.d_upd, (const u64*)pl.skd, pl.d_dkey, pl.d_ukey);
     });
 }
 
diff --git a/kart_amd/csrc/kd_ctx.hip b/kart_amd/csrc/kd_ctx.hip
--- a/kart_amd/csrc/kd_ctx.hip
+++ b/kart_amd/csrc/kd_ctx.hip
@@ -28,6 +28,7 @@
     if (b.bytes < bytes) {
         if (b.p) {
             hipError_t e = hipStreamSynchronize(ctx->stream);
+            if (e == hipSuccess && ctx->step_main) e = hipStreamSynchronize(ctx->step_main);
             if (e != hipSuccess) { set_error("sync before realloc: %s", hipGetErrorString(e)); return KD_EHIP; }
             if (!b.slab) KD_HIP(hipFree(b.p));
             b.p = nullptr;
@@ -308,6 +309,9 @@
     {"fd_walk", "KD_FD_WALK", nullptr, &kd_opts::fd_walk, nullptr},
     {"pkm_max_blocks", "KD_PKM_MAX_BLOCKS", nullptr, nullptr, &kd_opts::pkm_max_blocks},
     {"trace_host", "KD_TRACE_HOST", nullptr, &kd_opts::trace_host, nullptr},
+    {"step_overlap", "KD_STEP_OVERLAP", nullptr, &kd_opts::step_overlap, nullptr},
+    {"step_overlap_min", "KD_STEP_OVERLAP_MIN", nullptr, nullptr, &kd_opts::step_overlap_min},
+    {"pkm_wave", "KD_PKM_WAVE", nullptr, &kd_opts::pkm_wave, nullptr},
 };
 void opt_set(kd_opts& o, const OptDef& d, int64_t v) {
     if (d.i32) o.*(d.i32) = (int)v;
@@ -421,6 +425,12 @@
     prof_flush(ctx);
     comm_release(ctx);
     gather_release(ctx);
+    if (ctx->side_stream) {
+        (void)hipStreamSynchronize(ctx->side_stream);
+        (void)hipStreamDestroy(ctx->side_stream);
+    }
+    if (ctx->ev_fork) (void)hipEventDestroy(ctx->ev_fork);
+    if (ctx->ev_join) (void)hipEventDestroy(ctx->ev_join);
     for (auto& kv : ctx->bufs)
         if (kv.second.p && !kv.second.slab) (void)hipFree(kv.second.p);
     if (ctx->slab) (void)hipFree(ctx->slab);
diff --git a/kart_amd/csrc/kd_internal.h b/kart_amd/csrc/kd_internal.h
--- a/kart_amd/csrc/kd_internal.h
+++ b/kart_amd/csrc/kd_internal.h
@@ -72,6 +72,9 @@
     int fd_walk = -1;
     uint64_t pkm_max_blocks = 1ull << 26;
     int trace_host = 0;
+    int step_overlap = 1;
+    uint64_t step_overlap_min = 1ull << 26;
+    int pkm_wave = -1;
 };
 
 struct kd_ctx {
@@ -80,6 +83,9 @@
     hipStream_t own_stream = nullptr;
     hipStream_t stream = nullptr;
     std::map<std::string, kd::DevBuf> bufs;
+    hipStream_t side_stream = nullptr;
+    hipEvent_t ev_fork = nullptr, ev_join = nullptr;
+    hipStream_t step_main = nullptr;
     bool prof = false;
     std::string prof_only;
     std::vector<hipEvent_t> ev_pool;
@@ -122,6 +128,21 @@
 
 int occupancy(kd_ctx* ctx, const void* kernel, int block, size_t lds);
 
+struct StreamScope {
+    kd_ctx* ctx;
+    hipStream_t saved;
+    StreamScope(kd_ctx* c, hipStream_t s) : ctx(c), saved(c->stream) {
+        c->step_main = saved;
+        c->stream = s;
+    }
+    ~StreamScope() {
+        ctx->stream = saved;
+        ctx->step_main = nullptr;
+    }
+    StreamScope(const StreamScope&) = delete;
+    StreamScope& operator=(const StreamScope&) = delete;
+};
+
 void prof_begin(kd_ctx* ctx, const char* name, hipEvent_t* a);
 void prof_end(kd_ctx* ctx, const char* name, hipEvent_t a);
 int prof_flush(kd_ctx* ctx);
@@ -159,6 +180,18 @@
 int diff2_device(kd_ctx* ctx, const kd_side* A, const kd_side* B, u32 flags, u32* d_delta,
                  u32* d_upd, u64* d_counts, u32* d_err, const u32* ordA = nullptr, const u32* ordB = nullptr,
                  u64* d_dkey = nullptr, u64* d_ukey = nullptr);
+struct Diff2Place {
+    bool needed = false;
+    u64 ntiles = 0;
+    const void *sdel = nullptr, *tcnt = nullptr, *gpre = nullptr, *skd = nullptr;
+    u32 *d_delta = nullptr, *d_upd = nullptr;
+    u64 *d_dkey = nullptr, *d_ukey = nullptr;
+};
+int diff2_front(kd_ctx* ctx, const kd_side* A, const kd_side* B, u32 flags, u32* d_delta, u32* d_upd, u64* d_counts,
+                u32* d_err, const u32* ordA, const u32* ordB, u64* d_dkey, u64* d_ukey, Diff2Place* pl);
+int diff2_place(kd_ctx* ctx, const Diff2Place& pl);
+int delta_pk_order(kd_ctx* ctx, const kd_side* base, const kd_side* target, const u32* d_delta, const u64* d_keys,
+                   u64 cap, const u64* d_n, i64 pk_lo, i64 pk_hi, i64* d_pk, u32* d_perm, bool lds_free);
 #ifndef KD_C2_NT
 #define KD_C2_NT 256
 #endif
diff --git a/kart_amd/csrc/kd_sort.hip b/kart_amd/csrc/kd_sort.hip
--- a/kart_amd/csrc/kd_sort.hip
+++ b/kart_amd/csrc/kd_sort.hip
@@ -420,6 +420,7 @@
 #define KD_PKM_IPT 16
 #endif
 constexpr int PKM_NT = 256, PKM_IPT = KD_PKM_IPT, PKM_CH = PKM_NT * PKM_IPT;
+constexpr int PKM_CHW = 64 * PKM_IPT;
 
 __global__ __launch_bounds__(PKM_NT) void k_pkm_mark(const uint2* __restrict__ rec, u64 ncap, const u64* __restrict__ dn,
                                                      const u64* __restrict__ kA, const u64* __restrict__ kB,
@@ -460,9 +461,9 @@
 }
 
 static_assert(PKM_IPT % 4 == 0, "k_pkm_scan: 16-B loads and stores");
+template <bool WAVE>
 __global__ __launch_bounds__(PKM_NT) void k_pkm_scan(const u64* __restrict__ masks, u64 nb, u32* __restrict__ local,
-                                                     u32* __restrict__ chunk_tot, u64* __restrict__ zero) {
-    __shared__ u32 s_wave[PKM_NT / 64];
+                                                     u32* __restrict__ chunk_tot, u64* __restrict__ zero, u64 nch) {
     const int tid = threadIdx.x;
     const u64 c0 = (u64)blockIdx.x * PKM_CH + (u64)tid * PKM_IPT;
     u32 cnt[PKM_IPT], sum = 0;
@@ -486,8 +487,21 @@
     }
 #pragma unroll
     for (int j = 0; j < PKM_IPT; j++) sum += cnt[j];
-    u32 tot;
-    u32 ex = block_scan_u32<PKM_NT>(sum, s_wave, &tot);
+    u32 tot, ex;
+    if constexpr (WAVE) {
+        const int lane = tid & 63;
+        u32 x = sum;
+#pragma unroll
+        for (int o = 1; o < 64; o <<= 1) {
+            const u32 y = __shfl_up(x, o, 64);
+            if (lane >= o) x += y;
+        }
+        tot = __shfl(x, 63, 64);
+        ex = x - sum;
+    } else {
+        __shared__ u32 s_wave[PKM_NT / 64];
+        ex = block_scan_u32<PKM_NT>(sum, s_wave, &tot);
+    }
     if (c0 + PKM_IPT <= nb) {
         u32x4* l4 = (u32x4*)(local + c0);
 #pragma unroll
@@ -506,7 +520,12 @@
             ex += cnt[j];
         }
     }
-    if (tid == 0) chunk_tot[blockIdx.x] = tot;
+    if constexpr (WAVE) {
+        const u64 ch = (u64)blockIdx.x * (PKM_NT / 64) + (u64)(tid >> 6);
+        if ((tid & 63) == 0 && ch < nch) chunk_tot[ch] = tot;
+    } else {
+        if (tid == 0) chunk_tot[blockIdx.x] = tot;
+    }
 }
 
 constexpr int PKC_PT = 8;
@@ -534,6 +553,35 @@
     }
 }
 
+constexpr int PKC_WPT = 32;
+__global__ __launch_bounds__(64) void k_pkm_cscan_w(const u32* __restrict__ chunk_tot, u32 nch, u32* __restrict__ chunk_pre) {
+    const int lane = threadIdx.x;
+    u32 carry = 0;
+    for (u32 base = 0; base < nch; base += 64 * PKC_WPT) {
+        const u32 k0 = base + (u32)lane * PKC_WPT;
+        u32 v[PKC_WPT], sum = 0;
+#pragma unroll
+        for (int j = 0; j < PKC_WPT; j++) {
+            v[j] = k0 + j < nch ? chunk_tot[k0 + j] : 0u;
+            sum += v[j];
+        }
+        u32 x = sum;
+#pragma unroll
+        for (int o = 1; o < 64; o <<= 1) {
+            const u32 y = __shfl_up(x, o, 64);
+            if (lane >= o) x += y;
+        }
+        u32 e = carry + x - sum;
+#pragma unroll
+        for (int j = 0; j < PKC_WPT; j++) {
+            if (k0 + j < nch) chunk_pre[k0 + j] = e;
+            e += v[j];
+        }
+        carry += __shfl(x, 63, 64);
+    }
+}
+
+template <int CH>
 __global__ __launch_bounds__(PKM_NT) void k_pkm_place(const i64* __restrict__ pks, const u64* __restrict__ rkey, u64 ncap,
                                                       const u64* __restrict__ dn, i64 lo_block, u64 nb,
                                                       const u64* __restrict__ masks, const u32* __restrict__ local,
@@ -545,7 +593,7 @@
         const u64 b = (u64)((pk >> 6) - lo_block);
         if (b >= nb) continue;
         const u64 below = masks[b] & ((1ull << (pk & 63)) - 1);
-        const u32 pos = chunk_pre[b / PKM_CH] + local[b] + (u32)__popcll(below);
+        const u32 pos = chunk_pre[b / CH] + local[b] + (u32)__popcll(below);
         out_pk[pos] = pk;
         out_perm[pos] = (u32)r;
     }
@@ -1036,6 +1084,12 @@
 extern "C" int kd_delta_pk_order(kd_ctx* ctx, const kd_side* base, const kd_side* target, const uint32_t* d_delta,
                                  const uint64_t* d_keys, uint64_t cap, const uint64_t* d_n, int64_t pk_lo, int64_t pk_hi,
                                  int64_t* d_pk, uint32_t* d_perm) {
+    KD_CHECK(ctx, "kd_delta_pk_order: NULL");
+    return delta_pk_order(ctx, base, target, d_delta, d_keys, cap, d_n, pk_lo, pk_hi, d_pk, d_perm, false);
+}
+
+int kd::delta_pk_order(kd_ctx* ctx, const kd_side* base, const kd_side* target, const u32* d_delta, const u64* d_keys,
+                       u64 cap, const u64* d_n, i64 pk_lo, i64 pk_hi, i64* d_pk, u32* d_perm, bool lds_free) {
     KD_CHECK(ctx && base && target && d_n && d_pk && d_perm && (cap == 0 || d_delta || d_keys), "kd_delta_pk_order: NULL");
     KD_CHECK(base->key_mode == KD_KEY_INT && target->key_mode == KD_KEY_INT, "kd_delta_pk_order: KD_KEY_INT sides only");
     KD_CHECK(base->mem == KD_MEM_DEVICE && target->mem == KD_MEM_DEVICE, "kd_delta_pk_order: sides must be device memory");
@@ -1051,9 +1105,10 @@
     const i64 lo_block = pk_lo >> 6, hi_block = pk_hi >> 6;
     const u64 nb = (u64)hi_block - (u64)lo_block + 1;
     const u64 pkm_max = ctx->opt.pkm_max_blocks;
-    if (nb <= pkm_max && nb / PKM_CH < 0xFFFFFFFFull) {
+    if (nb <= pkm_max && nb / PKM_CHW < 0xFFFFFFFFull) {
         void *mbuf[2], *local, *ctot, *cpre, *tpk;
-        const u64 nch = (nb + PKM_CH - 1) / PKM_CH;
+        const u64 chunk = lds_free ? PKM_CHW : PKM_CH;
+        const u64 nch = (nb + chunk - 1) / chunk;
         if ((rc = ensure(ctx, "pkm.masks0", nb * 8, &mbuf[0]))) return rc;
         if ((rc = ensure(ctx, "pkm.masks1", nb * 8, &mbuf[1]))) return rc;
         const int cur = ctx->pkm_cur & 1;
@@ -1076,20 +1131,31 @@
         });
         if (rc) return rc;
         rc = launch(ctx, "k_pkm_scan", [&] {
-            hipLaunchKernelGGL(k_pkm_scan, dim3((unsigned)nch), dim3(PKM_NT), 0, ctx->stream, (const u64*)masks, nb,
-                               (u32*)local, (u32*)ctot, (u64*)other);
+            if (lds_free)
+                hipLaunchKernelGGL(k_pkm_scan<true>, dim3((unsigned)((nch + PKM_NT / 64 - 1) / (PKM_NT / 64))), dim3(PKM_NT),
+                                   0, ctx->stream, (const u64*)masks, nb, (u32*)local, (u32*)ctot, (u64*)other, nch);
+            else
+                hipLaunchKernelGGL(k_pkm_scan<false>, dim3((unsigned)nch), dim3(PKM_NT), 0, ctx->stream, (const u64*)masks,
+                                   nb, (u32*)local, (u32*)ctot, (u64*)other, nch);
         });
         if (rc) return rc;
         ctx->pkm_zero_ptr[cur ^ 1] = other;
         ctx->pkm_zero_nb[cur ^ 1] = nb;
         ctx->pkm_cur = cur ^ 1;
         rc = launch(ctx, "k_pkm_cscan", [&] {
-            hipLaunchKernelGGL(k_pkm_cscan, dim3(1), dim3(1024), 0, ctx->stream, (const u32*)ctot, (u32)nch, (u32*)cpre);
+            if (lds_free)
+                hipLaunchKernelGGL(k_pkm_cscan_w, dim3(1), dim3(64), 0, ctx->stream, (const u32*)ctot, (u32)nch, (u32*)cpre);
+            else
+                hipLaunchKernelGGL(k_pkm_cscan, dim3(1), dim3(1024), 0, ctx->stream, (const u32*)ctot, (u32)nch, (u32*)cpre);
         });
         if (rc) return rc;
         return launch(ctx, "k_pkm_place", [&] {
-            hipLaunchKernelGGL(k_pkm_place, dim3(g1), dim3(PKM_NT), 0, ctx->stream, (const i64*)tpk, d_keys, cap, d_n,
-                               lo_block, nb, (const u64*)masks, (const u32*)local, (const u32*)cpre, d_pk, d_perm);
+            if (lds_free)
+                hipLaunchKernelGGL(k_pkm_place<PKM_CHW>, dim3(g1), dim3(PKM_NT), 0, ctx->stream, (const i64*)tpk, d_keys, cap,
+                                   d_n, lo_block, nb, (const u64*)masks, (const u32*)local, (const u32*)cpre, d_pk, d_perm);
+            else
+                hipLaunchKernelGGL(k_pkm_place<PKM_CH>, dim3(g1), dim3(PKM_NT), 0, ctx->stream, (const i64*)tpk, d_keys, cap,
+                                   d_n, lo_block, nb, (const u64*)masks, (const u32*)local, (const u32*)cpre, d_pk, d_perm);
         });
     }
     SortPlan plan = pk_plan(pk_lo, pk_hi);
diff --git a/kart_amd/device.py b/kart_amd/device.py
--- a/kart_amd/device.py
+++ b/kart_amd/device.py
@@ -195,6 +195,7 @@
         self._ob, self._nb = self.OB.kd_blobs(), self.NB.kd_blobs()
         self._km = maps.kd_maps()
         self._perm_sides = None
+        self._steps = {}
         self.pk_order = bool(pk_order) and base.key_mode == N.KD_KEY_INT and gather is None
         if self.pk_order:
             lo, hi = [], []
@@ -244,6 +245,7 @@
                 b = arena.kd_blobs()
             blobs.append(b)
         self._ob_u, self._nb_u = blobs
+        self._steps = {}
 
     def reserve_gather(self, max_deltas_per_rank):
         self.all_delta.free()
@@ -277,6 +279,31 @@
     def _diff(self, perm):
         L, ctx = self.eng.L, self.eng.ctx
         keys = self.pk_order and self.flags == 0
+        if self.gather is None:
+            N.check(L.kd_diff2_step(ctx, ctypes.byref(self._step_args(perm, keys))), "kd_diff2_step")
+            return
+        N.check(L.kd_diff2_gather_begin(ctx, ctypes.byref(self._sa), ctypes.byref(self._sb), self.gather[0],
+                                        self.gather[1], self.flags, self.delta.ptr, self.upd.ptr, self.counts.ptr,
+                                        self.counts.ptr + 32, self.all_counts.ptr), "kd_diff2_gather_begin")
+        if self._ob_u is not None:
+            N.check(L.kd_fielddiff(ctx, ctypes.byref(self._ob_u), ctypes.byref(self._nb_u), None, self.cap_upd,
+                                   ctypes.cast(self.counts.ptr + 8, N.c_u64p), N.KD_MEM_DEVICE,
+                                   ctypes.byref(self._km), self.masks.ptr, self.status.ptr, N.KD_MEM_DEVICE),
+                    "kd_fielddiff")
+        else:
+            N.check(L.kd_fielddiff(ctx, ctypes.byref(self._ob), ctypes.byref(self._nb), self.upd.ptr, self.cap_upd,
+                                   ctypes.cast(self.counts.ptr + 8, N.c_u64p), N.KD_MEM_DEVICE,
+                                   ctypes.byref(self._km), self.masks.ptr, self.status.ptr, N.KD_MEM_DEVICE),
+                    "kd_fielddiff")
+        N.check(L.kd_diff2_gather_end(ctx, self.delta.ptr, self.all_delta.ptr, self.all_cap,
+                                      self.h_counts.ctypes.data), "kd_diff2_gather_end")
+
+    def _step_args(self, perm, keys):
+        form = (bool(perm), bool(keys), self._ob_u is not None)
+        st = self._steps.get(form)
+        if st is not None:
+            return st
+        st = N.KdStep()
         if perm:
             if self._perm_sides is None:
                 self._perm_sides = []
@@ -286,40 +313,29 @@
                     if w.name is not None:
                         k.name, k.name_off = w.name.ptr, w.name_off.ptr
                     self._perm_sides.append(k)
-            N.check(L.kd_diff2_device_ex(ctx, ctypes.byref(self._perm_sides[0]), ctypes.byref(self._perm_sides[1]),
-                                         self.walk[0][1].ptr, self.walk[1][1].ptr, self.flags, self.delta.ptr,
-                                         self.upd.ptr, self.dkey.ptr if keys else None, self.ukey.ptr if keys else None,
-                                         self.counts.ptr, self.counts.ptr + 32), "kd_diff2_device_ex")
-        elif self.gather is None:
-            N.check(L.kd_diff2_device_ex(ctx, ctypes.byref(self._sa), ctypes.byref(self._sb), None, None, self.flags,
-                                         self.delta.ptr, self.upd.ptr, self.dkey.ptr if keys else None,
-                                         self.ukey.ptr if keys else None, self.counts.ptr, self.counts.ptr + 32),
-                    "kd_diff2_device_ex")
+            st.base, st.target = ctypes.pointer(self._perm_sides[0]), ctypes.pointer(self._perm_sides[1])
+            st.base_order, st.target_order = self.walk[0][1].ptr, self.walk[1][1].ptr
         else:
-            N.check(L.kd_diff2_gather_begin(ctx, ctypes.byref(self._sa), ctypes.byref(self._sb), self.gather[0],
-                                            self.gather[1], self.flags, self.delta.ptr, self.upd.ptr, self.counts.ptr,
-                                            self.counts.ptr + 32, self.all_counts.ptr), "kd_diff2_gather_begin")
+            st.base, st.target = ctypes.pointer(self._sa), ctypes.pointer(self._sb)
+        st.flags = self.flags
+        st.d_delta, st.d_upd = self.delta.ptr, self.upd.ptr
+        st.d_counts, st.d_err = self.counts.ptr, self.counts.ptr + 32
         if self._ob_u is not None:
-            N.check(L.kd_fielddiff(ctx, ctypes.byref(self._ob_u), ctypes.byref(self._nb_u), None, self.cap_upd,
-                                   ctypes.cast(self.counts.ptr + 8, N.c_u64p), N.KD_MEM_DEVICE,
-                                   ctypes.byref(self._km), self.masks.ptr, self.status.ptr, N.KD_MEM_DEVICE),
-                    "kd_fielddiff")
+            st.old_blobs, st.new_blobs = ctypes.pointer(self._ob_u), ctypes.pointer(self._nb_u)
         else:
-            N.check(L.kd_fielddiff(ctx, ctypes.byref(self._ob), ctypes.byref(self._nb), self.upd.ptr, self.cap_upd,
-                               ctypes.cast(self.counts.ptr + 8, N.c_u64p), N.KD_MEM_DEVICE,
-                                   ctypes.byref(self._km), self.masks.ptr, self.status.ptr, N.KD_MEM_DEVICE),
-                    "kd_fielddiff")
+            st.old_blobs, st.new_blobs = ctypes.pointer(self._ob), ctypes.pointer(self._nb)
+            st.d_pairs = self.upd.ptr
+        st.upd_cap = self.cap_upd
+        st.maps = ctypes.pointer(self._km)
+        st.d_masks, st.d_status = self.masks.ptr, self.status.ptr
         if keys:
-            lo, hi = self.pk_range
-            N.check(L.kd_delta_pk_order(ctx, ctypes.byref(self._sa), ctypes.byref(self._sb), self.delta.ptr,
-                                        self.dkey.ptr, self.cap, self.counts.ptr + 24, lo, hi, self.d_pk.ptr,
-                                        self.d_perm.ptr), "kd_delta_pk_order")
-            N.check(L.kd_delta_pk_order(ctx, ctypes.byref(self._sa), ctypes.byref(self._sb), self.upd.ptr,
-                                        self.ukey.ptr, max(self.cap_upd, 1), self.counts.ptr + 8, lo, hi, self.u_pk.ptr,
-                                        self.u_perm.ptr), "kd_delta_pk_order")
-        if self.gather is not None:
-            N.check(L.kd_diff2_gather_end(ctx, self.delta.ptr, self.all_delta.ptr, self.all_cap,
-                                          self.h_counts.ctypes.data), "kd_diff2_gather_end")
+            st.d_delta_key, st.d_upd_key = self.dkey.ptr, self.ukey.ptr
+            st.pk_lo, st.pk_hi = self.pk_range
+            st.delta_cap = self.cap
+            st.d_delta_pk, st.d_delta_perm = self.d_pk.ptr, self.d_perm.ptr
+            st.d_upd_pk, st.d_upd_perm = self.u_pk.ptr, self.u_perm.ptr
+        self._steps[form] = st
+        return st
 
     def results(self):
         c = self.counts.download(np.uint64, 8)
```

Measured after the change: 35770 M feature-pairs/s (median of 6 runs). 4.1% higher.
